# guanjq/targetdiff

Hardware: AMD Instinct MI355X
Metric: ligands/sec (1000-step sampling, 100 samples/pocket) at 1/2/4/8 MI355X (higher is better)
Workload: dtype f32

## Files before the change

targetdiff_amd/capi.py:

```python
from __future__ import annotations

import ctypes
import os
from ctypes import POINTER, c_char_p, c_float, c_int32, c_int64, c_size_t, c_void_p

import numpy as np
import torch

_HERE = os.path.dirname(os.path.abspath(__file__))
LIB_PATH = os.path.join(_HERE, 'lib', 'libtargetdiff_hip.so')

TD_OK = 0
HIDDEN = 128
KNN = 32


class TdConfig(ctypes.Structure):
    _fields_ = [('hidden_dim', c_int32), ('n_heads', c_int32), ('knn', c_int32), ('num_layers', c_int32),
                ('num_r_gaussian', c_int32), ('edge_feat_dim', c_int32), ('protein_feat_dim', c_int32),
                ('ligand_num_classes', c_int32), ('num_timesteps', c_int32), ('cutoff_mode', c_int32), ('radius', c_float),
                ('max_num_neighbors', c_int32), ('model_mean_type', c_int32), ('num_blocks', c_int32), ('ew_net_type', c_int32),
                ('x2h_out_fc', c_int32), ('sync_twoup', c_int32), ('num_x2h', c_int32), ('num_h2x', c_int32), ('reserved', c_int32 * 1)]


# ... 554 lines not shown
        io.d_step = _ptr(step_index, torch.int32, 'step_index').value
        io.d_t_all = _ptr(t_all, torch.int32, 't_all').value
        io.num_steps, io.pos_only = S, int(bool(pos_only))
        io.d_ligand_pos = _ptr(ligand_pos, torch.float32, 'ligand_pos').value
        io.d_ligand_v = _ptr(ligand_v, torch.int64, 'ligand_v').value
        io.d_noise = _ptr(noise, torch.float32, 'noise').value
        io.d_uniform = _ptr(uniform, torch.float32, 'uniform').value
        io.d_pos_traj = _ptr(pos_traj, torch.float32, 'pos_traj').value
        io.d_v_traj = _ptr(v_traj, torch.int64, 'v_traj').value
        io.d_v0_traj = _ptr(v0_traj, torch.float32, 'v0_traj').value if v0_traj is not None and v0_traj.numel() else None
        io.d_vt_traj = _ptr(vt_traj, torch.float32, 'vt_traj').value if vt_traj is not None and vt_traj.numel() else None
        gb = _graph_bias_ptr(ligand_graph_bias, int(t_all.shape[1]))
        io.d_ligand_graph_bias = gb.value if gb is not None else None
        fm, fp, fv = _fixed_ptrs(fixed_mask, fixed_pos, fixed_v, self.Nl)
        if fm is not None:
            io.d_fixed_mask, io.d_fixed_pos, io.d_fixed_v = fm.value, fp.value, fv.value
        return io

    def set_program(self, table, kinds):
        if table is None:
            self._prog_table = None
            with _on(self.device):
                _check(self.lib.td_session_set_program(self.handle, None, None, 0), 'td_session_set_program')
            return
        kinds = [int(k) for k in kinds]
        if table.dtype != torch.float32 or tuple(table.shape) != (len(kinds), PROG_ROW) or not table.is_contiguous():
            raise ValueError(f'the program table must be contiguous fp32 [{len(kinds)}, {PROG_ROW}]')
        arr = (c_int32 * len(kinds))(*kinds)
        self._prog_table = table
        with _on(self.device):
            _check(self.lib.td_session_set_program(self.handle, _ptr(table, torch.float32, 'table'), arr, len(kinds)),
                   'td_session_set_program')

    def step(self, io: StepIO, use_graph=True):
        with _on(self.device):
            _check(self.lib.td_session_step(self.handle, ctypes.byref(io), int(bool(use_graph)), _stream(self.device)),
                   'td_session_step')

    def last_step_was_graph(self) -> bool:
        return bool(self.lib.td_session_step_graph(self.handle))

    def row_counts(self):
        n = self._counts()
        return int(n[0]), int(n[1]), [int(v) for v in n[2:6] if v >= 0]

    def forward_reach_rows(self):
        v = int(self._counts()[6])
        return v if v >= 0 else None

    def shared_static_tables(self):
        n = self._counts()
        return (int(n[7]), int(n[8])) if n[7] >= 0 else None

    @_device_bound
    def _counts(self):
        n = (c_int32 * 10)()
        _check(self.lib.td_session_row_counts(self.handle, n, 10, _stream(self.device)), 'td_session_row_counts')
        return n

    def dirty_rows(self) -> int:
        return self.row_counts()[1]


EGNN_LAYER_KEYS = ('edge_mlp.net.0.weight', 'edge_mlp.net.0.bias', 'edge_mlp.net.2.weight', 'edge_mlp.net.2.bias',
                   'edge_inf.0.weight', 'edge_inf.0.bias', 'x_mlp.0.weight', 'x_mlp.0.bias', 'x_mlp.2.weight',
                   'node_mlp.net.0.weight', 'node_mlp.net.0.bias', 'node_mlp.net.2.weight', 'node_mlp.net.2.bias')


def egnn_flat_key_order(num_layers: int):
    return [f'net.{l}.{k}' for l in range(num_layers) for k in EGNN_LAYER_KEYS]


def graph_ptr(batch: torch.Tensor, B: int) -> torch.Tensor:
    lib = load_library()
    ptr = torch.empty(B + 1, dtype=torch.int32, device=batch.device)
    with _on(batch.device):
        _check(lib.td_graph_ptr(_ptr(batch, torch.int64, 'batch'), batch.numel(), B, _ptr(ptr), _stream(batch.device)),
               'td_graph_ptr')
    return ptr


def protein_centroids(protein_pos: torch.Tensor, protein_ptr: torch.Tensor) -> torch.Tensor:
    lib = load_library()
    B = protein_ptr.numel() - 1
    scratch = protein_pos.detach().clone().contiguous().float()
    offset = torch.empty(B, 3, dtype=torch.float32, device=protein_pos.device)
    with _on(protein_pos.device):
        _check(lib.td_center_pos(_ptr(scratch), _ptr(protein_ptr, torch.int32, 'protein_ptr'), None,
                                 _ptr(protein_ptr, torch.int32, 'protein_ptr'), B, _ptr(offset), 1, -1,
                                 _stream(protein_pos.device)), 'td_center_pos')
    return offset


class NativeEgnn:

    def __init__(self, num_layers: int, state_dict, hidden_dim=HIDDEN, edge_feat_dim=4, k=KNN, device=None, prefix=''):
        self.lib = load_library()
        self.device = _canonical_device(device)
        self.num_layers = int(num_layers)
        blob = np.ascontiguousarray(np.concatenate(
            [state_dict[prefix + key].detach().cpu().numpy().astype(np.float32).reshape(-1)
             for key in egnn_flat_key_order(self.num_layers)]))
        handle = c_void_p()
        with torch.cuda.device(self.device):
            _check(self.lib.td_egnn_create(self.num_layers, hidden_dim, edge_feat_dim, k, blob.ctypes.data_as(POINTER(c_float)),
                                           blob.size, ctypes.byref(handle)), 'td_egnn_create')
# ... 147 lines not shown
```

targetdiff_amd/csrc/edge16.hip:

```cpp
#include <type_traits>

#include "td_device.h"
#include "td_internal.h"

typedef float floatx4_t __attribute__((ext_vector_type(4)));

__device__ __forceinline__ floatx4_t td_mfma16(float a, float b, floatx4_t c) {
    return __builtin_amdgcn_mfma_f32_16x16x4f32(a, b, c, 0, 0, 0);
}

#ifndef TD_ZPLAIN_OFF
#define TD_ZPLAIN_OFF 0
#endif
#ifndef TD_ABL
#define TD_ABL 0
#endif
typedef _Float16 half8_16 __attribute__((ext_vector_type(8)));
__device__ __forceinline__ floatx4_t td_mfma16h(uint4 a, uint4 b, floatx4_t c) {
    return __builtin_amdgcn_mfma_f32_16x16x32_f16(__builtin_bit_cast(half8_16, a), __builtin_bit_cast(half8_16, b), c, 0, 0, 0);
}
__device__ __forceinline__ void td_split_h2(float x, float y, unsigned &h1, unsigned &h2) {
    h1 = __builtin_bit_cast(unsigned, __builtin_amdgcn_cvt_pkrtz(x, y));
    asm("v_fma_mixlo_f16 %0, %1, -1.0, %2 op_sel_hi:[1,0,0]\n\t"
        "v_fma_mixhi_f16 %0, %1, -1.0, %3 op_sel:[1,0,0] op_sel_hi:[1,0,0]"
// ... 41 lines not shown
#if TD_SPLIT_X4
#pragma unroll
    for (int m = 0; m < 4; ++m) h1[m] = __builtin_bit_cast(unsigned, __builtin_amdgcn_cvt_pkrtz(x[m], y[m]));
    asm("v_fma_mixlo_f16 %0, %4, -1.0, %8 op_sel_hi:[1,0,0]\n\t"
        "v_fma_mixlo_f16 %1, %5, -1.0, %9 op_sel_hi:[1,0,0]\n\t"
        "v_fma_mixlo_f16 %2, %6, -1.0, %10 op_sel_hi:[1,0,0]\n\t"
        "v_fma_mixlo_f16 %3, %7, -1.0, %11 op_sel_hi:[1,0,0]\n\t"
        "v_fma_mixhi_f16 %0, %4, -1.0, %12 op_sel:[1,0,0] op_sel_hi:[1,0,0]\n\t"
        "v_fma_mixhi_f16 %1, %5, -1.0, %13 op_sel:[1,0,0] op_sel_hi:[1,0,0]\n\t"
        "v_fma_mixhi_f16 %2, %6, -1.0, %14 op_sel:[1,0,0] op_sel_hi:[1,0,0]\n\t"
        "v_fma_mixhi_f16 %3, %7, -1.0, %15 op_sel:[1,0,0] op_sel_hi:[1,0,0]"
        : "=&v"(h2[0]), "=&v"(h2[1]), "=&v"(h2[2]), "=&v"(h2[3])
        : "v"(h1[0]), "v"(h1[1]), "v"(h1[2]), "v"(h1[3]), "v"(x[0]), "v"(x[1]), "v"(x[2]), "v"(x[3]), "v"(y[0]), "v"(y[1]), "v"(y[2]), "v"(y[3]));
#else
#pragma unroll
    for (int m = 0; m < 4; ++m) td_split_h2(x[m], y[m], h1[m], h2[m]);
#endif
}

constexpr float TD_ATT_SCALE_16 = 0.35355339059327373f;
constexpr float TD_LOG2E = 1.4426950408889634f;
constexpr float TD_FAR_CENTRE = 1.0e4f;
constexpr int E16_STEPS = TD_SLOTK / 4;
constexpr int E16_R_FLOATS = 2 * 2 * E16_STEPS * 64 * 8;
constexpr int E16_WQ_FLOATS = 8 * 4 * 2 * 64 * 4;

struct Args16 {
    const float4 *x4;
    const int32_t *nbr;
    const float *ew;
    const float *P;
    const float *q;
    const int32_t *rows;
    const int32_t *count_ptr;
    float *h;
    const float *gate_m;
    float *out;
    float *alpha;
    float4 *x4_out;
    int64_t count;
    TdEdgeMlp mlp;
    const float *offsets;
    float coeff;
    int p_off;
    const int32_t *chunk_node;
    const int32_t *cptr;
    const int32_t *lig_rows;
    int64_t lig_count;
    int cpn_p;
    int64_t lig_chunks;
    const int32_t *mixed_count;
    int deal;
    unsigned long long *trace;
};

__device__ __forceinline__ void td_trace_wave_end(unsigned long long *trace, int lane) {
    if (lane == 0) {
        const unsigned long long t = __builtin_amdgcn_s_memrealtime();
        atomicMin(trace + 8 * blockIdx.x + 2, t);
        atomicAdd(trace + 8 * blockIdx.x + 3, t);
    }
}

__device__ __forceinline__ void td_node_range16(int64_t count, const int32_t *count_ptr, int64_t &begin, int64_t &end, int G = gridDim.x,
                                                int b = blockIdx.x) {
    if (count_ptr) count = *count_ptr;
    const int x = b & 7, r = G & 7;
    const int chunk = x * (G >> 3) + (x < r ? x : r) + (b >> 3);
    const int64_t per = (count + G - 1) / G;
    begin = (int64_t)chunk * per;
    end = begin + per < count ? begin + per : count;
}

__device__ __forceinline__ void td_deal16(int64_t count, int U, int64_t &first, int64_t &end, int64_t &stride, int G = gridDim.x,
                                          int b = blockIdx.x) {
    const int x = b & 7, r = G & 7, w = b >> 3;
    const int c0 = x * (G >> 3) + (x < r ? x : r), nx = (G >> 3) + (x < r ? 1 : 0);
    const int64_t xb = count * c0 / G;
    end = count * (c0 + nx) / G;
    first = xb + (int64_t)w * U;
    stride = (int64_t)nx * U;
}

__device__ __forceinline__ float td_sum_groups(float v) { return td_sum_halves(td_sum_rows16(v)); }

__device__ __forceinline__ float td_sum16(float v) {
    v += td_dpp<DPP_QUAD_XOR1>(v);
    v += td_dpp<DPP_QUAD_XOR2>(v);
    v += td_dpp<DPP_ROW_HALF_MIRROR>(v);
    v += td_dpp<DPP_ROW_MIRROR>(v);
    return v;
}
__device__ __forceinline__ float td_max16(float v) {
    v = fmaxf(v, td_dpp<DPP_QUAD_XOR1>(v));
    v = fmaxf(v, td_dpp<DPP_QUAD_XOR2>(v));
    v = fmaxf(v, td_dpp<DPP_ROW_HALF_MIRROR>(v));
    v = fmaxf(v, td_dpp<DPP_ROW_MIRROR>(v));
    return v;
}

#define TD_DPP4(op, ctrl)                                            \
    op " %0, %0, %0 " ctrl " row_mask:0xf bank_mask:0xf\n\t"         \
    op " %1, %1, %1 " ctrl " row_mask:0xf bank_mask:0xf\n\t"         \
    op " %2, %2, %2 " ctrl " row_mask:0xf bank_mask:0xf\n\t"         \
    op " %3, %3, %3 " ctrl " row_mask:0xf bank_mask:0xf\n\t"
__device__ __forceinline__ void td_max16x4(float (&v)[4]) {
// ... 370 lines not shown
                for (int h2 = 0; h2 < 2; ++h2)
#pragma unroll
                    for (int eb = 0; eb < NEB; ++eb)
                        acc[eb][2 * hp + h2] = td_mfma16b(aq[h2], bq[eb][tb], acc[eb][2 * hp + h2]);
            }
        }
    }
}

template <int NEB>
__device__ __forceinline__ void td_h2_bquads(const float (&m)[NEB][5], const unsigned (&ct)[NEB], uint4 (&bq)[NEB][2]) {
    if constexpr (NEB == 2) {
        const float x[4] = {m[0][0], m[0][2], m[1][0], m[1][2]}, y[4] = {m[0][1], m[0][3], m[1][1], m[1][3]};
        unsigned a1[4], a2[4], u1, u2;
        td_split_h2_x4(x, y, a1, a2);
        td_split_h2(m[0][4], m[1][4], u1, u2);
        bq[0][0] = make_uint4(a1[0], a1[1], a1[0], a1[1]);
        bq[1][0] = make_uint4(a1[2], a1[3], a1[2], a1[3]);
        bq[0][1] = make_uint4(a2[0], a2[1], __builtin_amdgcn_perm(u2, u1, 0x05040100u), __builtin_amdgcn_perm(ct[0], u1, 0x07060100u));
        bq[1][1] = make_uint4(a2[2], a2[3], __builtin_amdgcn_perm(u2, u1, 0x07060302u), __builtin_amdgcn_perm(ct[1], u1, 0x07060302u));
    } else {
        unsigned a1[2], a2[2], u1, u2;
        td_split_h2(m[0][0], m[0][1], a1[0], a2[0]);
        td_split_h2(m[0][2], m[0][3], a1[1], a2[1]);
        td_split_h2(m[0][4], 0.f, u1, u2);
        bq[0][0] = make_uint4(a1[0], a1[1], a1[0], a1[1]);
        bq[0][1] = make_uint4(a2[0], a2[1], __builtin_amdgcn_perm(u2, u1, 0x05040100u), __builtin_amdgcn_perm(ct[0], u1, 0x07060100u));
    }
}
template <bool AHEAD, int NEB>
__device__ __forceinline__ void td_h2_tiles(const uint4 *__restrict__ Rs, const uint4 (&bq)[NEB][2], floatx4_t (&acc)[2][8]) {
    auto quad = [&](int st) -> uint4 { return Rs[((st & 1) ? 0 : 512) + (st >> 1) * 64]; };
    if constexpr (AHEAD) {
        uint4 cur = quad(0);
#pragma unroll
        for (int st = 0; st < 16; ++st) {
            uint4 nxt = cur;
            if (st + 1 < 16) nxt = quad(st + 1);
            __builtin_amdgcn_sched_barrier(0);
#pragma unroll
            for (int eb = 0; eb < NEB; ++eb) acc[eb][st >> 1] = td_mfma16h(cur, bq[eb][(st & 1) ? 0 : 1], acc[eb][st >> 1]);
            cur = nxt;
        }
    } else {
#pragma unroll
        for (int st = 0; st < 16; ++st) {
            const uint4 q = quad(st);
#pragma unroll
            for (int eb = 0; eb < NEB; ++eb) acc[eb][st >> 1] = td_mfma16h(q, bq[eb][(st & 1) ? 0 : 1], acc[eb][st >> 1]);
        }
    }
}

struct TdNoHook { __device__ __forceinline__ void operator()() const {} };
template <bool LOAD_EW, bool ONE_CLASS, bool PI_LATE, int NEB, bool LN_SKIP, int PK, int AH = 0, class Hook = TdNoHook, bool NO_LN = false>
__device__ __forceinline__ void td_first_layer_split16(const Args16 &a, const uint4 *__restrict__ Rp,
                                                       const float *__restrict__ KB,
                                                       const float (&offj)[8], const RowIn16 &r, int64_t i, int lane,
                                                       floatx4_t (&acc)[2][8], Edge2 &ed, Hook before_products = Hook()) {
    const int g = lane >> 4;
    const float4 xi = r.xi;
    ed.xi = xi;
    const int cls = xi.w > 0.5f ? 0 : 1;
    float4 pi[8];
    {
        const float *pp = a.P + (size_t)i * (4 * TD_H) + a.p_off + 4 * g;
#pragma unroll
        for (int hb = 0; hb < 8; ++hb) pi[hb] = *reinterpret_cast<const float4 *>(pp + 16 * hb);
    }
    auto add_pi = [&]() {
#pragma unroll
        for (int hb = 0; hb < 8; ++hb)
#pragma unroll
            for (int eb = 0; eb < NEB; ++eb) {
                acc[eb][hb][0] += pi[hb].x; acc[eb][hb][1] += pi[hb].y; acc[eb][hb][2] += pi[hb].z; acc[eb][hb][3] += pi[hb].w;
            }
    };
    if (!PI_LATE) add_pi();
    int slot[NEB];
    bool has[2][NEB];
    float gv[NEB][5];
    if (NEB == 1) {
        ed.valid[1] = false; ed.any[1] = false;
        ed.rel[1][0] = ed.rel[1][1] = ed.rel[1][2] = 0.f;
        if (LOAD_EW) ed.ew[1] = 0.f;
#pragma unroll
        for (int hb = 0; hb < 8; ++hb) acc[1][hb] = floatx4_t{0.f, 0.f, 0.f, 0.f};
    }
    const float c2 = a.coeff * TD_LOG2E;
#pragma unroll
    for (int eb = 0; eb < NEB; ++eb) {
        ed.valid[eb] = r.j[eb] >= 0;
        const float4 xj = r.xj[eb];
        if (LOAD_EW) ed.ew[eb] = r.ew[eb];
        const float rx = xi.x - xj.x, ry = xi.y - xj.y, rz = xi.z - xj.z;
        const float dist = td_sqrt_d2(rx * rx + ry * ry + rz * rz);
        ed.rel[eb][0] = rx; ed.rel[eb][1] = ry; ed.rel[eb][2] = rz;
        slot[eb] = xj.w > 0.5f ? 0 : 1;
        has[0][eb] = __ballot(ed.valid[eb] && slot[eb] == 0) != 0ull;
        has[1][eb] = __ballot(ed.valid[eb] && slot[eb] == 1) != 0ull;
        ed.any[eb] = has[0][eb] || has[1][eb];
#pragma unroll
        for (int j = 0; j < 5; ++j) {
            const float u = dist - offj[j];
            gv[eb][j] = __builtin_amdgcn_exp2f(c2 * (u * u));
        }
    }
    before_products();
    auto products4 = [&](int sl) {
        if constexpr (PK == 5) {
            float mm[NEB][5];
            unsigned ct[NEB];
            uint4 bh[NEB][2];
#pragma unroll
            for (int eb = 0; eb < NEB; ++eb) {
                const bool keep = !has[1 - sl][eb] || slot[eb] == sl;
#pragma unroll
                for (int j = 0; j < 5; ++j) mm[eb][j] = keep ? gv[eb][j] : 0.f;
                ct[eb] = keep ? 0x3c000000u : 0u;
            }
            td_h2_bquads<NEB>(mm, ct, bh);
            td_h2_tiles<AH != 0, NEB>(Rp + (size_t)((ONE_CLASS ? 0 : cls * 2) + sl) * e16q_cs_u4<5>() + lane, bh, acc);
            return;
        } else {
        uint4 bq[NEB][4];
        const unsigned ctype = td_pk4_ctype(g);
#pragma unroll
        for (int eb = 0; eb < NEB; ++eb) {
            const bool keep = !has[1 - sl][eb] || slot[eb] == sl;
            float m[5];
#pragma unroll
            for (int j = 0; j < 5; ++j) m[j] = keep ? gv[eb][j] : 0.f;
            td_pk4_bquads(m, keep ? ctype : 0u, bq[eb]);
        }
        if constexpr (PK == 3) {
            static_assert(PK != 3 || !ONE_CLASS, "PK = 3 holds both destination classes");
            if (cls) td_pk4_tiles<1, AH, NEB>(Rp + 2 * e16q_cs_u4<2>() + (size_t)sl * e16q_cs_u4<1>() + lane, lane, bq, acc);
            else td_pk4_tiles<2, AH, NEB>(Rp + (size_t)sl * e16q_cs_u4<2>() + lane, lane, bq, acc);
        } else if constexpr (PK == 4) {
            static_assert(PK != 4 || ONE_CLASS, "PK = 4 holds one destination class");
            if (sl) td_pk4_tiles<1, AH, NEB>(Rp + e16q_cs_u4<2>() + lane, lane, bq, acc);
            else td_pk4_tiles<2, AH, NEB>(Rp + lane, lane, bq, acc);
        } else
            td_pk4_tiles<PK, AH, NEB>(Rp + (size_t)((ONE_CLASS ? 0 : cls * 2) + sl) * e16q_cs_u4<PK>() + lane, lane, bq, acc);
        }
    };
#pragma unroll
    for (int sl = 0; sl < 2; ++sl) {
        bool any_sl = has[sl][0];
        if (NEB == 2) any_sl = any_sl || has[sl][NEB - 1];
        if (any_sl) products4(sl);
    }
    if (PI_LATE) add_pi();
    if constexpr (NO_LN) return;
    const TdLn ln{a.mlp.ln_c1, a.mlp.ln_c2};
    if (NEB == 2 && LN_SKIP) td_ln_relu16_skip(KB, g, acc, ln, ed.any);
    else td_ln_relu16<NEB>(KB, g, acc, ln);
}

template <bool LOAD_EW, bool SKIP_EMPTY = false>
__device__ __forceinline__ void td_first_layer16(const Args16 &a, const float4 *__restrict__ Rt,
                                                 const float *__restrict__ KB,
                                                 const float (&offk)[E16_STEPS], int64_t i, int lane,
                                                 floatx4_t (&acc)[2][8], Edge2 &ed, int64_t c = -1) {
    RowIn16 r;
    if (c < 0) c = i;
    td_row_index16(a, i, c, lane, r);
    td_row_gather16<LOAD_EW>(a, i, c, lane, r, acc);
    td_first_layer_compute16<LOAD_EW, SKIP_EMPTY>(a, Rt, KB, offk, r, lane, acc, ed);
}

constexpr int K16_WAVES = 16;
constexpr int XV16_WAVES = 8;
constexpr size_t K16_LDS_BYTES = (size_t)(E16_R_FLOATS + E16_WQ_FLOATS + TD_H + 4) * sizeof(float);
#ifndef TD_KEY_WAVES
#define TD_KEY_WAVES 12
#endif
#ifndef TD_KEY_WALK_F16
#define TD_KEY_WALK_F16 1
#endif
constexpr int K16S_WAVES = TD_KEY_WAVES;
#ifndef TD_KEY_PK
#define TD_KEY_PK 3
#endif
#ifndef TD_KEY_AH
#define TD_KEY_AH -1
#endif
constexpr size_t K16S_LDS_BYTES = (size_t)(e16q_u4<TD_KEY_PK>() * 4 + E16_WQ_FLOATS + TD_H + 4 + 32) * sizeof(float);
static_assert(K16S_LDS_BYTES <= 160 * 1024, "key pass: LDS");

template <bool XV, int WAVES, int STAGE, int GRAPH = 0, bool SPLIT = false, int L2 = 0, int FL = 0>
__global__ __launch_bounds__(WAVES * 64) void edge_key16_kernel(Args16 a) {
    constexpr bool ZPLAIN = L2 == 2;
    constexpr bool CHUNKED = GRAPH == 1;
    constexpr bool VIA = GRAPH == 2;
    constexpr bool L2H = L2 != 0;
    static_assert(L2 == 0 || (SPLIT && !XV && STAGE == 0), "f16 logits: x2h key pass, bf16 first layer");
    static_assert(FL == 0 || SPLIT, "f16 first layer: the 16-bit instantiations");
    constexpr int KPK = FL ? 5 : TD_KEY_PK;
    constexpr int RF = SPLIT ? e16q_u4<KPK>() * 4 : E16_R_FLOATS;
    constexpr int NOFF = SPLIT ? 8 : E16_STEPS;
    extern __shared__ __attribute__((aligned(16))) float lds[];
    const float4 *Rt = reinterpret_cast<const float4 *>(lds);
    const float4 *Wq = reinterpret_cast<const float4 *>(lds + RF);
    const float *KB = lds + RF + E16_WQ_FLOATS;
    const int tid = threadIdx.x, lane = tid & 63, wid = tid >> 6;
    const int lo = lane & 15, g = lane >> 4;
    if (a.trace && threadIdx.x == 0) a.trace[8 * blockIdx.x + 4] = __builtin_amdgcn_s_memrealtime();
    {
        if (SPLIT) {
            if constexpr (KPK == 5)
                td_stage_lds16(reinterpret_cast<const float4 *>(a.mlp.R16h), reinterpret_cast<float4 *>(lds), e16q_u4<5>(), tid, WAVES * 64);
            else if constexpr (TD_KEY_PK == 3) {
                td_stage_pk4<2>(a.mlp.R16q, lds, 2, tid, WAVES * 64);
                td_stage_pk4<1>(a.mlp.R16q + (size_t)2 * E16Q_GLOBAL_CS_U4 * 4, lds + 2 * e16q_cs_u4<2>() * 4, 2, tid, WAVES * 64);
            } else
                td_stage_pk4<TD_KEY_PK>(a.mlp.R16q, lds, 4, tid, WAVES * 64);
        }
        else td_stage_lds16(reinterpret_cast<const float4 *>(a.mlp.R16), reinterpret_cast<float4 *>(lds), RF / 4, tid, WAVES * 64);
        const int nw4 = XV ? 8 * 4 * 64 / 4 : E16_WQ_FLOATS / 4;
        td_stage_lds16(reinterpret_cast<const float4 *>(a.mlp.Walt16), reinterpret_cast<float4 *>(lds + RF), nw4, tid,
                       WAVES * 64);
        if (tid < TD_H) lds[RF + E16_WQ_FLOATS + tid] = a.mlp.beta[tid];
        else if (tid == TD_H) *reinterpret_cast<int *>(lds + RF + E16_WQ_FLOATS + TD_H) = 0;
        else if (SPLIT && tid >= TD_H + 32 && tid < TD_H + 64) {
            const int s8 = tid - (TD_H + 32);
            lds[RF + E16_WQ_FLOATS + TD_H + 4 + s8] = (s8 & 7) < 5 ? a.offsets[5 * (s8 >> 3) + (s8 & 7)] : TD_FAR_CENTRE;
        }
    }
    float offk[NOFF];
#pragma unroll
    for (int s = 0; s < NOFF; ++s) {
        const int k = SPLIT ? 5 * g + s : 4 * s + g;
        offk[s] = SPLIT ? (s < 5 ? a.offsets[k] : TD_FAR_CENTRE) : (k < TD_NG ? a.offsets[k] : 0.f);
    }
    __syncthreads();
    if (a.trace && tid == 0) a.trace[8 * blockIdx.x] = __builtin_amdgcn_s_memrealtime();
    int64_t begin, end, stride = WAVES;
    if (a.deal) td_deal16(a.count_ptr ? (int64_t)*a.count_ptr : a.count, a.deal == 2 ? 1 : WAVES, begin, end, stride);
    else td_node_range16(a.count, a.count_ptr, begin, end);
    int *row_ctr = reinterpret_cast<int *>(lds + RF + E16_WQ_FLOATS + TD_H);
    const bool dyn = a.deal == 2;
    auto grab = [&]() -> int {
        int n = 0;
        if (lane == 0) n = __hip_atomic_fetch_add(row_ctr, 1, __ATOMIC_RELAXED, __HIP_MEMORY_SCOPE_WORKGROUP);
        return n;
    };
    auto row_of = [&](int n) -> int64_t {
        return begin + (int64_t)__builtin_amdgcn_readfirstlane(n) * stride;
    };

    float4 qpre0, qpre1;
    auto first_layer = [&](int64_t i, int64_t c, floatx4_t (&acc)[2][8], Edge2 &ed) {
        constexpr bool EW = !XV && !CHUNKED;
        if constexpr (SPLIT) {
            RowIn16 rin;
            td_row_index16(a, i, c, lane, rin);
            td_row_gather16<EW>(a, i, c, lane, rin, acc);
            float offr[8];
            {
                int dep = 0;
                asm volatile("" : "+v"(dep));
                const float4 *op = reinterpret_cast<const float4 *>(lds + RF + E16_WQ_FLOATS + TD_H + 4 + 8 * g + dep);
                const float4 o0 = op[0], o1 = op[1];
                offr[0] = o0.x; offr[1] = o0.y; offr[2] = o0.z; offr[3] = o0.w; offr[4] = o1.x; offr[5] = o1.y; offr[6] = o1.z; offr[7] = o1.w;
            }
            auto fetch_q = [&]() {
                if constexpr (!XV && !CHUNKED) {
                    qpre0 = *reinterpret_cast<const float4 *>(a.q + (size_t)i * TD_H + 8 * lo);
                    qpre1 = *reinterpret_cast<const float4 *>(a.q + (size_t)i * TD_H + 8 * lo + 4);
                }
            };
            if (XV && CHUNKED && __ballot(rin.j[1] >= 0) == 0ull)
                td_first_layer_split16<EW, false, false, 1, false, KPK>(a, reinterpret_cast<const uint4 *>(lds), KB, offr, rin, i, lane, acc, ed, fetch_q);
            else
                td_first_layer_split16<EW, false, false, 2, CHUNKED, KPK, (CHUNKED || XV) ? 0 : TD_KEY_AH, decltype(fetch_q), L2H>(a, reinterpret_cast<const uint4 *>(lds), KB, offr, rin, i, lane, acc, ed, fetch_q);
        } else
            td_first_layer16<EW, CHUNKED>(a, Rt, KB, offk, i, lane, acc, ed, c);
    };

    for (int64_t it = dyn ? row_of(grab()) : begin + wid; it < end; it = dyn ? row_of(grab()) : it + stride) {
        const int64_t i = a.rows ? (int64_t)a.rows[it] : it;
        int64_t c0 = i;
        int nch = 1;
        if (CHUNKED) {
            c0 = __builtin_amdgcn_readfirstlane(a.cptr[i]);
            nch = __builtin_amdgcn_readfirstlane(a.cptr[i + 1]) - (int)c0;
        }
        if (VIA) {
            if (__builtin_amdgcn_readfirstlane(__float_as_int(a.x4[i].w)) > __float_as_int(0.5f)) continue;
            c0 = __builtin_amdgcn_readfirstlane(a.cptr[i]);
        }

        if (XV) {
            const float *Wx = lds + RF;
            const float b2 = a.mlp.b2[lo];
            float sx = 0.f, sy = 0.f, sz = 0.f;
            float4 xi_keep = a.x4[i];
            for (int64_t c = c0; c < c0 + nch; ++c) {
                floatx4_t acc[2][8];
                Edge2 ed;
                first_layer(i, c, acc, ed);
                floatx4_t xv[2];
#pragma unroll
                for (int eb = 0; eb < 2; ++eb) xv[eb] = floatx4_t{0.f, 0.f, 0.f, 0.f};
#pragma unroll
                for (int hb = 0; hb < 8; ++hb)
#pragma unroll
                    for (int r = 0; r < 4; ++r) {
                        const float u = Wx[(hb * 4 + r) * 64 + lane];
                        xv[0] = td_mfma16(u, acc[0][hb][r], xv[0]);
                        if (!CHUNKED || ed.any[1]) xv[1] = td_mfma16(u, acc[1][hb][r], xv[1]);
                    }
#pragma unroll
                for (int r = 0; r < 4; ++r) {
                    const float bias = __shfl(b2, 4 * g + r);
                    const float *ap = a.alpha + ((size_t)c * TD_HEADS + 4 * g + r) * TD_K + lo;
#pragma unroll
                    for (int eb = 0; eb < 2; ++eb) {
                        const float wgt = ed.valid[eb] ? ap[16 * eb] * (xv[eb][r] + bias) : 0.f;
                        sx = fmaf(wgt, ed.rel[eb][0], sx);
                        sy = fmaf(wgt, ed.rel[eb][1], sy);
                        sz = fmaf(wgt, ed.rel[eb][2], sz);
                    }
                }
// ... 920 lines not shown
#pragma unroll
            for (int s = 0; s < 8; ++s) zb[hb] = td_mfma16(bvb[hb & 1][s], al[s], zb[hb]);
        }

        }
        const int64_t icur = i;
        const float hcur0 = hres0, hcur1 = hres1;
        if (SPLIT && dyn && more) {
            inext = settle(inext, rnext, cnext);
            more = inext >= 0;
        }
        {
            const int64_t gsafe = more ? inext : 0;
            td_row_gather16<false>(a, gsafe, more ? cnext : chunk_of(0), lane, rnext, acc);
            load_side(gsafe, more ? cnext : chunk_of(0), al, hres0, hres1);
            rin = rnext;
        }
        i = inext;

        float o0, o1;
        td_value_out16(zb, Wt_lane, o0, o1);
        o0 = fmaf(B2[nout], ssum, o0 * out_scale);
        o1 = fmaf(B2[nout + 4], ssum, o1 * out_scale);
        if (a.out) {
            a.out[(size_t)icur * TD_H + nout] = o0;
            a.out[(size_t)icur * TD_H + nout + 4] = o1;
        } else {
            a.h[(size_t)icur * TD_H + nout] = hcur0 + o0;
            a.h[(size_t)icur * TD_H + nout + 4] = hcur1 + o1;
        }
    }
    trace_end();
}

constexpr int V16T_WAVES = 12;
#ifndef TD_VALUET_PK
#define TD_VALUET_PK 1
#endif
constexpr int V16T_PK = TD_VALUET_PK;
#ifndef TD_VALUET_AH
#define TD_VALUET_AH -1
#endif
constexpr int V16T_AH = TD_VALUET_AH;
constexpr int V16T_WAVE_FLOATS = V16_TILE_FLOATS;
constexpr size_t V16T_LDS_BYTES =
    (size_t)(e16q_half_u4<V16T_PK>() * 4 + V16_W_FLOATS + V16T_WAVES * V16T_WAVE_FLOATS + 2 * TD_H + 4 + 32) * sizeof(float);
static_assert(V16T_LDS_BYTES <= 160 * 1024, "value pass (12 waves): LDS");

template <int L2, bool VIA = false, int FL = 0>
__global__ __launch_bounds__(V16T_WAVES * 64) void edge_value16t_kernel(Args16 a) {
    constexpr bool ZPLAIN = L2 == 2;
    constexpr int WAVES = V16T_WAVES;
    constexpr int VPK = FL ? 5 : V16T_PK;
    constexpr int RF = e16q_half_u4<VPK>() * 4;
    extern __shared__ __attribute__((aligned(16))) float lds[];
    const int tid = threadIdx.x, lane = tid & 63, wid = tid >> 6;
    const int lo = lane & 15, g = lane >> 4;
    float *TB = lds + RF + V16_W_FLOATS + wid * V16T_WAVE_FLOATS;
    float *B2 = lds + RF + V16_W_FLOATS + WAVES * V16T_WAVE_FLOATS;
    const float *KB = B2 + TD_H;
    int my_cls = 1, GL = 0;
    const int64_t n_rows = a.count_ptr ? (int64_t)*a.count_ptr : a.count;
    {
        const int64_t G = gridDim.x, nl = a.lig_count, np = n_rows > nl ? n_rows - nl : 0;
        if (nl > 0) {
            int64_t nm = a.mixed_count ? (int64_t)*a.mixed_count - nl : (np * 3) / 10;
            nm = nm < 0 ? 0 : (nm > np ? np : nm);
            const int64_t wl = TD_ROW_COST_MIXED * nl, wp = TD_ROW_COST_PURE * (np - nm) + TD_ROW_COST_MIXED * nm;
            GL = (int)((wl * G + (wl + wp) / 2) / (wl + wp));
            const int cap = (int)G - (np > 0 ? 1 : 0);
            GL = GL < 1 ? 1 : (GL > cap ? cap : GL);
        }
        my_cls = (int)blockIdx.x >= (int)G - GL ? 0 : 1;
    }
    const int GP = gridDim.x - GL;
    if (a.trace && threadIdx.x == 0) a.trace[8 * blockIdx.x + 4] = __builtin_amdgcn_s_memrealtime();
    {
        if constexpr (VPK == 5)
            td_stage_lds16(reinterpret_cast<const float4 *>(a.mlp.R16h) + (size_t)my_cls * 2 * e16q_cs_u4<5>(), reinterpret_cast<float4 *>(lds), 2 * e16q_cs_u4<5>(), tid, WAVES * 64);
        else if constexpr (V16T_PK == 4) {
            td_stage_pk4<2>(a.mlp.R16q + (size_t)my_cls * 2 * E16Q_GLOBAL_CS_U4 * 4, lds, 1, tid, WAVES * 64);
            td_stage_pk4<1>(a.mlp.R16q + (size_t)(my_cls * 2 + 1) * E16Q_GLOBAL_CS_U4 * 4, lds + e16q_cs_u4<2>() * 4, 1, tid, WAVES * 64);
        } else
            td_stage_pk4<V16T_PK>(a.mlp.R16q + (size_t)my_cls * 2 * E16Q_GLOBAL_CS_U4 * 4, lds, 2, tid, WAVES * 64);
        td_stage_lds16(reinterpret_cast<const float4 *>(a.mlp.Walt), reinterpret_cast<float4 *>(lds + RF), V16_W_FLOATS / 4, tid, WAVES * 64);
        if (tid < TD_H) B2[tid] = a.mlp.b2[tid];
        else if (tid < 2 * TD_H) B2[tid] = a.mlp.beta[tid - TD_H];
        else if (tid == 2 * TD_H) *reinterpret_cast<int *>(B2 + 2 * TD_H) = 0;
        else if (tid >= 2 * TD_H + 32 && tid < 2 * TD_H + 64) {
            const int s8 = tid - (2 * TD_H + 32);
            B2[2 * TD_H + 4 + s8] = (s8 & 7) < 5 ? a.offsets[5 * (s8 >> 3) + (s8 & 7)] : TD_FAR_CENTRE;
        }
    }
    __syncthreads();
    if (a.trace && tid == 0) a.trace[8 * blockIdx.x] = __builtin_amdgcn_s_memrealtime();
    const int32_t *list = a.rows;
    int64_t first, end, stride = 1;
    if (my_cls) td_deal16(n_rows, 1, first, end, stride, GP, (int)blockIdx.x);
    else {
        list = a.lig_rows;
        const int64_t per = (a.lig_count + GL - 1) / GL;
        first = ((int)blockIdx.x - GP) * per;
        end = first + per < a.lig_count ? first + per : a.lig_count;
    }
    int *row_ctr = reinterpret_cast<int *>(B2 + 2 * TD_H);
    auto next_row = [&]() -> int64_t {
        int n = 0;
        if (lane == 0) n = __hip_atomic_fetch_add(row_ctr, 1, __ATOMIC_RELAXED, __HIP_MEMORY_SCOPE_WORKGROUP);
        n = __builtin_amdgcn_readfirstlane(n);
        const int64_t itx = first + (int64_t)n * stride;
        return itx < end ? (int64_t)__builtin_amdgcn_readfirstlane((int)(list ? (int64_t)list[itx] : itx)) : -1;
    };
    const int nout = td_value_out_index16(lo, g);
    int woff = RF + 4 * lane;
    asm volatile("" : "+v"(woff));
    const float *Wt_lane = lds + woff;
    for (int64_t i = next_row(); i >= 0; i = next_row()) {
        RowIn16 rin;
        const int64_t c = VIA ? (int64_t)__builtin_amdgcn_readfirstlane(a.cptr[i]) : i;
        td_row_index16(a, i, c, lane, rin);
        if (((__builtin_amdgcn_readfirstlane(__float_as_int(rin.xi.w)) > __float_as_int(0.5f)) ? 0 : 1) != my_cls) continue;
        floatx4_t acc[2][8];
        td_row_gather16<false>(a, i, c, lane, rin, acc);
        float al[8];
        if constexpr (L2 != 0) {
            const float *ap = a.alpha + ((size_t)c * TD_HEADS + lo) * TD_K + 4 * g;
            const float4 v0 = *reinterpret_cast<const float4 *>(ap), v1 = *reinterpret_cast<const float4 *>(ap + 16);
            al[0] = v0.x; al[1] = v1.x; al[2] = v0.y; al[3] = v1.y; al[4] = v0.z; al[5] = v1.z; al[6] = v0.w; al[7] = v1.w;
        } else {
            const float *ap = a.alpha + ((size_t)c * TD_HEADS + lo) * TD_K + 8 * g;
            const float4 v0 = *reinterpret_cast<const float4 *>(ap), v1 = *reinterpret_cast<const float4 *>(ap + 4);
            al[0] = v0.x; al[1] = v0.y; al[2] = v0.z; al[3] = v0.w; al[4] = v1.x; al[5] = v1.y; al[6] = v1.z; al[7] = v1.w;
        }
        const float hres0 = a.h[(size_t)i * TD_H + nout], hres1 = a.h[(size_t)i * TD_H + nout + 4];
        Edge2 ed;
        float offr[8];
        {
            int dep = 0;
            asm volatile("" : "+v"(dep));
            const float4 *op = reinterpret_cast<const float4 *>(B2 + 2 * TD_H + 4 + 8 * g + dep);
            const float4 o0 = op[0], o1 = op[1];
            offr[0] = o0.x; offr[1] = o0.y; offr[2] = o0.z; offr[3] = o0.w; offr[4] = o1.x; offr[5] = o1.y; offr[6] = o1.z; offr[7] = o1.w;
        }
        float ssum = ((al[0] + al[1]) + (al[2] + al[3])) + ((al[4] + al[5]) + (al[6] + al[7]));
        ssum = td_sum_groups(ssum);
        floatx4_t zb[8];
        constexpr float OUT_SCALE = L2 == 0 ? 1.0f : (ZPLAIN ? 1.0f / 1024.0f : 1.0f / (1024.0f * TD_Z_SCALE));
        if constexpr (L2 != 0) {
        td_first_layer_split16<false, true, false, 2, false, VPK, V16T_AH, TdNoHook, true>(a, reinterpret_cast<const uint4 *>(lds), KB, offr, rin, i, lane, acc, ed);
        uint4 z1[8], z2[8];
        td_ln_relu16_pairs_eb<!ZPLAIN>(KB, g, acc, TdLn{a.mlp.ln_c1, a.mlp.ln_c2}, z1, z2);
        uint4 aq1, aq2;
        {
            unsigned p1[4], p2[4];
            const float ax[4] = {al[0] * 1024.0f, al[2] * 1024.0f, al[4] * 1024.0f, al[6] * 1024.0f};
            const float ay[4] = {al[1] * 1024.0f, al[3] * 1024.0f, al[5] * 1024.0f, al[7] * 1024.0f};
            td_split_h2_x4(ax, ay, p1, p2);
            aq1 = make_uint4(p1[0], p1[1], p1[2], p1[3]);
            aq2 = make_uint4(p2[0], p2[1], p2[2], p2[3]);
        }
        unsigned *TW = reinterpret_cast<unsigned *>(TB);
        constexpr int TWS = 20, TWP = 16 * TWS;
        auto flip_store = [&](int hb) {
            *reinterpret_cast<uint4 *>(TW + lo * TWS + 4 * g) = z1[hb];
            *reinterpret_cast<uint4 *>(TW + TWP + lo * TWS + 4 * g) = z2[hb];
        };
        auto flip_load = [&](uint4 (&zq)[2]) {
            const unsigned *t = TW + 4 * g * TWS + lo;
            zq[0] = make_uint4(t[0], t[TWS], t[2 * TWS], t[3 * TWS]);
            zq[1] = make_uint4(t[TWP], t[TWP + TWS], t[TWP + 2 * TWS], t[TWP + 3 * TWS]);
        };
        uint4 zqb[2][2];
        flip_store(0);
        flip_load(zqb[0]);
#pragma unroll
        for (int hb = 0; hb < 8; ++hb) {
            if (hb + 1 < 8) {
                flip_store(hb + 1);
                flip_load(zqb[(hb + 1) & 1]);
            }
            __builtin_amdgcn_sched_barrier(0);
            zb[hb] = floatx4_t{0.f, 0.f, 0.f, 0.f};
            zb[hb] = td_mfma16h(zqb[hb & 1][1], aq1, zb[hb]);
            zb[hb] = td_mfma16h(zqb[hb & 1][0], aq2, zb[hb]);
            zb[hb] = td_mfma16h(zqb[hb & 1][0], aq1, zb[hb]);
        }
        } else {
        td_first_layer_split16<false, true, false, 2, false, VPK, V16T_AH>(a, reinterpret_cast<const uint4 *>(lds), KB, offr, rin, i, lane, acc, ed);
        auto flip_store = [&](int hb) {
#pragma unroll
            for (int eb = 0; eb < 2; ++eb)
                *reinterpret_cast<float4 *>(TB + td_tile_row16(16 * eb + lo) + 4 * g) =
                    make_float4(acc[eb][hb][0], acc[eb][hb][1], acc[eb][hb][2], acc[eb][hb][3]);
        };
        auto flip_load = [&](float (&bv)[8]) {
#pragma unroll
            for (int sx = 0; sx < 8; ++sx) bv[sx] = TB[td_tile_row16(8 * g + sx) + lo];
        };
        float bvb[2][8];
        flip_store(0);
        flip_load(bvb[0]);
#pragma unroll
        for (int hb = 0; hb < 8; ++hb) {
            if (hb + 1 < 8) {
                flip_store(hb + 1);
                flip_load(bvb[(hb + 1) & 1]);
            }
            __builtin_amdgcn_sched_barrier(0);
            zb[hb] = floatx4_t{0.f, 0.f, 0.f, 0.f};
#pragma unroll
            for (int sx = 0; sx < 8; ++sx) zb[hb] = td_mfma16(bvb[hb & 1][sx], al[sx], zb[hb]);
        }
        }
        float o0, o1;
        td_value_out16(zb, Wt_lane, o0, o1);
        o0 = fmaf(B2[nout], ssum, o0 * OUT_SCALE);
        o1 = fmaf(B2[nout + 4], ssum, o1 * OUT_SCALE);
        if (a.out) {
            a.out[(size_t)i * TD_H + nout] = o0;
            a.out[(size_t)i * TD_H + nout + 4] = o1;
        } else {
            a.h[(size_t)i * TD_H + nout] = hres0 + o0;
            a.h[(size_t)i * TD_H + nout + 4] = hres1 + o1;
        }
    }
    if (a.trace) {
        td_trace_wave_end(a.trace, lane);
        __syncthreads();
        if (tid == 0) a.trace[8 * blockIdx.x + 1] = __builtin_amdgcn_s_memrealtime();
    }
}

constexpr int TD_GATE_WGS = 1024;
constexpr int G16_WAVES = 4;
constexpr int G16Q_U4 = e16q_cs_u4<1>();
constexpr size_t G16_LDS_BYTES = (size_t)G16Q_U4 * 16 + (size_t)3 * TD_H * sizeof(float);

__global__ __launch_bounds__(G16_WAVES * 64) void edge_gate16_kernel(TdGate gt, const float4 *__restrict__ x4,
                                                                     const int32_t *__restrict__ nbr, int64_t N,
                                                                     const int32_t *__restrict__ rows,
                                                                     const int32_t *__restrict__ count_ptr,
// ... 41 lines not shown
                gv[j] = __builtin_amdgcn_exp2f(c2 * (u * u));
            }
            td_pk4_bquads(gv, 0u, bq[eb]);
#pragma unroll
            for (int hb = 0; hb < 8; ++hb) {
                const float4 b = *reinterpret_cast<const float4 *>(B0 + 16 * hb + 4 * g);
                acc[eb][hb][0] = b.x; acc[eb][hb][1] = b.y; acc[eb][hb][2] = b.z; acc[eb][hb][3] = b.w;
            }
        }
        td_pk4_tiles<1, 1, 2>(Rp + lane, lane, bq, acc);
        td_ln_relu16<2>(BET, g, acc, TdLn{gt.ln_c1, gt.ln_c2});
#pragma unroll
        for (int eb = 0; eb < 2; ++eb) {
            float part = 0.f;
#pragma unroll
            for (int hb = 0; hb < 8; ++hb) {
                const float4 w = *reinterpret_cast<const float4 *>(W3 + 16 * hb + 4 * g);
                part = fmaf(acc[eb][hb][0], w.x, part); part = fmaf(acc[eb][hb][1], w.y, part);
                part = fmaf(acc[eb][hb][2], w.z, part); part = fmaf(acc[eb][hb][3], w.w, part);
            }
            const float logit = td_sum_groups(part) + gt.b3;
            if (g == 0) ew[row * TD_K + 16 * eb + lo] = valid[eb] ? 1.0f / (1.0f + expf(-logit)) : 0.f;
        }
    }
}

#define TD_LDS_ONCE(fn, bytes) do { static TdLdsOnce once; int _rc = td_set_lds(once, reinterpret_cast<const void *>(fn), bytes); if (_rc != TD_OK) return _rc; } while (0)

static int grid16(int64_t count, int waves) {
    int64_t g = (count + waves - 1) / waves;
    if (g < 256) g = count < 256 ? count : 256;
    if (g > 256) g = 256;
    if (g >= 8) g = (g / 8) * 8;
    return (int)(g < 1 ? 1 : g);
}

static unsigned long long *g_wg_trace = nullptr;
static int g_wg_trace_slots = 0, g_wg_trace_launch[3] = {0, 0, 0};
int td_set_wg_trace(unsigned long long *buf, int slots) {
    g_wg_trace = slots > 0 ? buf : nullptr;
    g_wg_trace_slots = slots;
    g_wg_trace_launch[0] = g_wg_trace_launch[1] = g_wg_trace_launch[2] = 0;
    return TD_OK;
}
bool td_wg_trace_armed() { return g_wg_trace != nullptr; }
static unsigned long long *wg_trace_slot(int pass) {
    if (!g_wg_trace) return nullptr;
    const int n = g_wg_trace_launch[pass]++ % g_wg_trace_slots;
    return g_wg_trace + ((size_t)n * 3 + pass) * 256 * 8;
}

int td_launch_edge_key16(const TdEdgeMlp &mlp, const TdLayer &L, const float4 *x4, const int32_t *nbr, const float *ew,
                         const float *P, const float *q, const int32_t *rows, const int32_t *count_ptr, int64_t count,
                         float *alpha, hipStream_t s, bool h2x_stage, const int32_t *cptr, const int32_t *lig_rows, int64_t lig_count, int cpn_p) {
    if (count == 0) return TD_OK;
    Args16 a = {};
    a.x4 = x4; a.nbr = nbr; a.ew = ew; a.P = P; a.q = q; a.rows = rows; a.count_ptr = count_ptr; a.h = nullptr;
    a.alpha = alpha; a.x4_out = nullptr; a.count = count; a.mlp = mlp; a.offsets = L.offsets; a.coeff = L.coeff; a.p_off = 0;
    a.cptr = cptr;
    const bool h2x = h2x_stage;
    if (!h2x) a.trace = wg_trace_slot(0);
    a.deal = h2x ? 0 : mlp.deal_rows;
#define TD_KEY_LAUNCH(WAVES, STAGE, CH, SP, BYTES)                                                            \
    do {                                                                                                      \
        TD_LDS_ONCE((edge_key16_kernel<false, WAVES, STAGE, CH, SP>), BYTES);                                 \
        edge_key16_kernel<false, WAVES, STAGE, CH, SP><<<dim3(grid16(a.count, WAVES)), dim3(WAVES * 64), BYTES, s>>>(a); \
    } while (0)
#define TD_KEY_LAUNCH_X2H(GR, L2V)                                                                                            \
    do {                                                                                                                  \
        if (mlp.l1_f16) {                                                                                                 \
            TD_LDS_ONCE((edge_key16_kernel<false, K16S_WAVES, 0, GR, true, L2V, 1>), K16S_LDS_BYTES);                      \
            edge_key16_kernel<false, K16S_WAVES, 0, GR, true, L2V, 1><<<dim3(grid16(a.count, K16S_WAVES)), dim3(K16S_WAVES * 64), K16S_LDS_BYTES, s>>>(a); \
        } else {                                                                                                          \
            TD_LDS_ONCE((edge_key16_kernel<false, K16S_WAVES, 0, GR, true, L2V, 0>), K16S_LDS_BYTES);                      \
            edge_key16_kernel<false, K16S_WAVES, 0, GR, true, L2V, 0><<<dim3(grid16(a.count, K16S_WAVES)), dim3(K16S_WAVES * 64), K16S_LDS_BYTES, s>>>(a); \
        }                                                                                                                 \
    } while (0)
#define TD_KEY_LAUNCH_WALK_L2(L2V) TD_KEY_LAUNCH_X2H(1, L2V)
#if TD_KEY_WALK_F16
#define TD_KEY_LAUNCH_WALK_F16(L2V)                                                                                           \
    do {                                                                                                                  \
        TD_LDS_ONCE((edge_key16_kernel<false, K16S_WAVES, 0, 1, true, L2V, 1>), K16S_LDS_BYTES);                          \
        edge_key16_kernel<false, K16S_WAVES, 0, 1, true, L2V, 1><<<dim3(grid16(a.count, K16S_WAVES)), dim3(K16S_WAVES * 64), K16S_LDS_BYTES, s>>>(a); \
    } while (0)
#define TD_KEY_LAUNCH_WALK()                                                        \
    do {                                                                            \
        if (!mlp.l2_f16 || !mlp.l1_f16) TD_KEY_LAUNCH_WALK_L2(0);                   \
        else if (mlp.z_plain && !TD_ZPLAIN_OFF) TD_KEY_LAUNCH_WALK_F16(2);          \
        else TD_KEY_LAUNCH_WALK_F16(1);                                             \
    } while (0)
#else
#define TD_KEY_LAUNCH_WALK() TD_KEY_LAUNCH_WALK_L2(0)
#endif
#define TD_KEY_LAUNCH_H2X(GR)                                                                                                 \
    do {                                                                                                                  \
        if (mlp.l1_f16) {                                                                                                 \
            TD_LDS_ONCE((edge_key16_kernel<false, K16S_WAVES, 1, GR, true, 0, 1>), K16S_LDS_BYTES);                        \
            edge_key16_kernel<false, K16S_WAVES, 1, GR, true, 0, 1><<<dim3(grid16(a.count, K16S_WAVES)), dim3(K16S_WAVES * 64), K16S_LDS_BYTES, s>>>(a); \
        } else TD_KEY_LAUNCH(K16S_WAVES, 1, GR, true, K16S_LDS_BYTES);                                                     \
    } while (0)
    if (mlp.use_split) {
        if (cptr && !h2x && cpn_p == 1) {
#define TD_KEY_LAUNCH_VIA(L2V) TD_KEY_LAUNCH_X2H(2, L2V)
            if (!mlp.l2_f16) TD_KEY_LAUNCH_VIA(0);
            else if (mlp.z_plain && !TD_ZPLAIN_OFF) TD_KEY_LAUNCH_VIA(2);
            else TD_KEY_LAUNCH_VIA(1);
#undef TD_KEY_LAUNCH_VIA
            if (lig_rows && lig_count > 0) {
                a.rows = lig_rows; a.count_ptr = nullptr; a.count = lig_count; a.trace = nullptr;
// ... 2 lines not shown
        } else if (cptr) { if (h2x) TD_KEY_LAUNCH_H2X(1); else TD_KEY_LAUNCH_WALK(); }
        else if (h2x) TD_KEY_LAUNCH_H2X(0);
        else {
#define TD_KEY_LAUNCH_L2(L2V) TD_KEY_LAUNCH_X2H(0, L2V)
            if (!mlp.l2_f16) TD_KEY_LAUNCH_L2(0);
            else if (mlp.z_plain && !TD_ZPLAIN_OFF) TD_KEY_LAUNCH_L2(2);
            else TD_KEY_LAUNCH_L2(1);
#undef TD_KEY_LAUNCH_L2
        }
    } else {
        if (cptr) { if (h2x) TD_KEY_LAUNCH(K16_WAVES, 1, 1, false, K16_LDS_BYTES); else TD_KEY_LAUNCH(K16_WAVES, 0, 1, false, K16_LDS_BYTES); }
        else { if (h2x) TD_KEY_LAUNCH(K16_WAVES, 1, 0, false, K16_LDS_BYTES); else TD_KEY_LAUNCH(K16_WAVES, 0, 0, false, K16_LDS_BYTES); }
    }
#undef TD_KEY_LAUNCH
#undef TD_KEY_LAUNCH_WALK
#undef TD_KEY_LAUNCH_WALK_L2
#undef TD_KEY_LAUNCH_X2H
#undef TD_KEY_LAUNCH_H2X
    TD_CHECK_HIP(hipGetLastError());
    return TD_OK;
}

int td_launch_edge_xv16(const TdEdgeMlp &mlp, const TdLayer &L, const float4 *x4_in, float4 *x4_out, const int32_t *nbr,
                        const float *P, const int32_t *rows, int64_t count, const float *alpha, hipStream_t s,
                        const int32_t *cptr) {
    if (count == 0) return TD_OK;
    Args16 a = {};
    a.x4 = x4_in; a.nbr = nbr; a.ew = nullptr; a.P = P; a.q = nullptr; a.rows = rows; a.count_ptr = nullptr; a.h = nullptr;
    a.alpha = const_cast<float *>(alpha); a.x4_out = x4_out; a.count = count; a.mlp = mlp; a.offsets = L.offsets;
    a.coeff = L.coeff; a.p_off = 2 * TD_H; a.cptr = cptr;
    const dim3 grid(grid16(count, XV16_WAVES)), block(XV16_WAVES * 64);
#define TD_XV_LAUNCH(CH, SP, BYTES)                                                            \
    do {                                                                                       \
        TD_LDS_ONCE((edge_key16_kernel<true, XV16_WAVES, 1, CH, SP>), BYTES);                  \
        edge_key16_kernel<true, XV16_WAVES, 1, CH, SP><<<grid, block, BYTES, s>>>(a);          \
    } while (0)
#define TD_XV_LAUNCH_F16(CH)                                                                   \
    do {                                                                                       \
        TD_LDS_ONCE((edge_key16_kernel<true, XV16_WAVES, 1, CH, true, 0, 1>), K16S_LDS_BYTES); \
        edge_key16_kernel<true, XV16_WAVES, 1, CH, true, 0, 1><<<grid, block, K16S_LDS_BYTES, s>>>(a); \
    } while (0)
    if (mlp.use_split && mlp.l1_f16) { if (cptr) TD_XV_LAUNCH_F16(1); else TD_XV_LAUNCH_F16(0); }
    else if (mlp.use_split) { if (cptr) TD_XV_LAUNCH(1, true, K16S_LDS_BYTES); else TD_XV_LAUNCH(0, true, K16S_LDS_BYTES); }
    else { if (cptr) TD_XV_LAUNCH(1, false, K16_LDS_BYTES); else TD_XV_LAUNCH(0, false, K16_LDS_BYTES); }
#undef TD_XV_LAUNCH
#undef TD_XV_LAUNCH_F16
    TD_CHECK_HIP(hipGetLastError());
    return TD_OK;
}

int td_launch_edge_value16(const TdEdgeMlp &mlp, const TdLayer &L, const float4 *x4, const int32_t *nbr, const float *P,
                           const int32_t *rows, const int32_t *count_ptr, int64_t count, float *h, const float *alpha,
                           const int32_t *lig_rows, int64_t lig_count, hipStream_t s, const int32_t *cptr, int cpn_p,
                           int64_t lig_chunks, const int32_t *mixed_count, float *out, const float *gate_m) {
    if (count == 0) return TD_OK;
    Args16 a = {};
    a.x4 = x4; a.nbr = nbr; a.ew = nullptr; a.P = P; a.q = nullptr; a.rows = rows; a.count_ptr = count_ptr; a.h = h;
    a.alpha = const_cast<float *>(alpha); a.x4_out = nullptr; a.count = count; a.mlp = mlp; a.offsets = L.offsets;
    a.coeff = L.coeff; a.p_off = 2 * TD_H; a.cptr = cptr; a.cpn_p = cpn_p > 0 ? cpn_p : 1; a.lig_chunks = lig_chunks;
    a.mixed_count = mixed_count;
    a.out = out;
    a.gate_m = cptr ? nullptr : gate_m;
    int G = grid16(count, V16_WAVES);
    const dim3 block(V16_WAVES * 64);
    a.trace = wg_trace_slot(1);
    a.deal = mlp.deal_rows;
#define TD_V16_LAUNCH(CH, GM, L2V)                                                                            \
    do {                                                                                                     \
        if (mlp.l1_f16) {                                                                                    \
            TD_LDS_ONCE((edge_value16_kernel<true, CH, GM, L2V, 1>), V16S_LDS_BYTES);                        \
            edge_value16_kernel<true, CH, GM, L2V, 1><<<dim3(G), block, V16S_LDS_BYTES, s>>>(a);             \
        } else {                                                                                             \
            TD_LDS_ONCE((edge_value16_kernel<true, CH, GM, L2V, 0>), V16S_LDS_BYTES);                        \
            edge_value16_kernel<true, CH, GM, L2V, 0><<<dim3(G), block, V16S_LDS_BYTES, s>>>(a);             \
        }                                                                                                    \
    } while (0)
#define TD_V16T_LAUNCH_ANY(L2V, VIAV)                                                                         \
    do {                                                                                                     \
        if (mlp.l1_f16) {                                                                                    \
            TD_LDS_ONCE((edge_value16t_kernel<L2V, VIAV, 1>), V16T_LDS_BYTES);                               \
            edge_value16t_kernel<L2V, VIAV, 1><<<dim3(Gt), dim3(V16T_WAVES * 64), V16T_LDS_BYTES, s>>>(a);   \
        } else {                                                                                             \
            TD_LDS_ONCE((edge_value16t_kernel<L2V, VIAV, 0>), V16T_LDS_BYTES);                               \
            edge_value16t_kernel<L2V, VIAV, 0><<<dim3(Gt), dim3(V16T_WAVES * 64), V16T_LDS_BYTES, s>>>(a);   \
        }                                                                                                    \
    } while (0)
#define TD_V16_LAUNCH_WALK_L2(L2V) TD_V16_LAUNCH(true, false, L2V)
#define TD_V16_LAUNCH_WALK()                                                        \
    do {                                                                            \
        if (!mlp.l2_f16) TD_V16_LAUNCH_WALK_L2(0);                                  \
        else if (mlp.z_plain && !TD_ZPLAIN_OFF) TD_V16_LAUNCH_WALK_L2(2);           \
        else TD_V16_LAUNCH_WALK_L2(1);                                              \
    } while (0)
    if (mlp.use_split) {
        a.lig_rows = lig_rows; a.lig_count = lig_rows ? lig_count : 0;
        if (G < 2 && a.lig_count > 0) G = 2;
        if (cptr && a.cpn_p == 1) {
            int Gt = grid16(count, V16T_WAVES);
            a.lig_rows = nullptr; a.lig_count = 0;
#define TD_V16T_LAUNCH_VIA(L2V) TD_V16T_LAUNCH_ANY(L2V, true)
            if (!mlp.l2_f16) TD_V16T_LAUNCH_VIA(0);
            else if (mlp.z_plain && !TD_ZPLAIN_OFF) TD_V16T_LAUNCH_VIA(2);
            else TD_V16T_LAUNCH_VIA(1);
#undef TD_V16T_LAUNCH_VIA
            if (lig_rows && lig_count > 0) {
                a.rows = lig_rows; a.count_ptr = nullptr; a.count = lig_count; a.lig_rows = lig_rows; a.lig_count = lig_count;
                a.mixed_count = nullptr; a.trace = nullptr;
                G = grid16(lig_count, V16_WAVES);
                TD_V16_LAUNCH_WALK();
// ... 18 lines not shown
            TD_V16_LAUNCH(false, false, 0);
        }
    } else if (cptr) {
        TD_LDS_ONCE((edge_value16_kernel<false, true>), V16_LDS_BYTES);
        edge_value16_kernel<false, true><<<dim3(G), block, V16_LDS_BYTES, s>>>(a);
    } else if (gate_m) {
        TD_LDS_ONCE((edge_value16_kernel<false, false, true>), V16_LDS_BYTES);
        edge_value16_kernel<false, false, true><<<dim3(G), block, V16_LDS_BYTES, s>>>(a);
    } else {
        TD_LDS_ONCE((edge_value16_kernel<false, false>), V16_LDS_BYTES);
        edge_value16_kernel<false, false><<<dim3(G), block, V16_LDS_BYTES, s>>>(a);
    }
#undef TD_V16_LAUNCH_WALK
#undef TD_V16_LAUNCH_WALK_L2
#undef TD_V16T_LAUNCH_ANY
#undef TD_V16_LAUNCH
    TD_CHECK_HIP(hipGetLastError());
    return TD_OK;
}

int td_launch_edge_h2x16(const TdEdgeMlp &mlp_k, const TdEdgeMlp &mlp_v, const TdLayer &L, const float4 *x4_in, float4 *x4_out,
                         const int32_t *nbr, const float *ew, const float *P, const float *q, const int32_t *rows,
                         int64_t count, hipStream_t s, const int32_t *cptr, float *alpha) {
    if (count == 0) return TD_OK;
    ArgsH2x ar = {};
    Args16 &a = ar.a;
    a.x4 = x4_in; a.nbr = nbr; a.ew = ew; a.P = P; a.q = q; a.rows = rows; a.count_ptr = nullptr; a.h = nullptr;
    a.alpha = alpha; a.x4_out = x4_out; a.count = count; a.mlp = mlp_k; a.offsets = L.offsets; a.coeff = L.coeff; a.p_off = 0;
    a.cptr = cptr;
    ar.mlp_v = mlp_v;
    a.trace = cptr ? nullptr : wg_trace_slot(2);
    const dim3 grid(grid16(count, H2X16_WAVES)), block(H2X16_WAVES * 64);
    const bool f16_first = mlp_k.l1_f16 && mlp_v.l1_f16;
    if (cptr && f16_first) {
        TD_LDS_ONCE((edge_h2x16_chunked_kernel<1>), h2x16_lds_bytes<true>());
        edge_h2x16_chunked_kernel<1><<<grid, block, h2x16_lds_bytes<true>(), s>>>(ar);
    } else if (cptr) {
        TD_LDS_ONCE((edge_h2x16_chunked_kernel<0>), h2x16_lds_bytes<true>());
        edge_h2x16_chunked_kernel<0><<<grid, block, h2x16_lds_bytes<true>(), s>>>(ar);
    } else if (mlp_k.use_split && mlp_v.use_split && f16_first) {
        TD_LDS_ONCE((edge_h2x16_kernel<true, 1>), h2x16_lds_bytes<true>());
        edge_h2x16_kernel<true, 1><<<grid, block, h2x16_lds_bytes<true>(), s>>>(ar);
    } else if (mlp_k.use_split && mlp_v.use_split) {
        TD_LDS_ONCE((edge_h2x16_kernel<true>), h2x16_lds_bytes<true>());
        edge_h2x16_kernel<true><<<grid, block, h2x16_lds_bytes<true>(), s>>>(ar);
    } else {
        TD_LDS_ONCE((edge_h2x16_kernel<false>), h2x16_lds_bytes<false>());
        edge_h2x16_kernel<false><<<grid, block, h2x16_lds_bytes<false>(), s>>>(ar);
    }
    TD_CHECK_HIP(hipGetLastError());
    return TD_OK;
}

int td_launch_gate16(const TdGate &g, const float4 *x4, const int32_t *nbr, int64_t N, const int32_t *rows,
                     const int32_t *count_ptr, float *ew, hipStream_t s, const int32_t *chunk_node) {
    if (N == 0) return TD_OK;
    TD_LDS_ONCE((edge_gate16_kernel), G16_LDS_BYTES);
    int64_t G = (N + G16_WAVES - 1) / G16_WAVES;
    if (G > TD_GATE_WGS) G = TD_GATE_WGS;
    edge_gate16_kernel<<<dim3((unsigned)G), dim3(G16_WAVES * 64), G16_LDS_BYTES, s>>>(g, x4, nbr, N, rows, count_ptr, chunk_node, ew);
    TD_CHECK_HIP(hipGetLastError());
    return TD_OK;
}
```

targetdiff_amd/csrc/graph.hip:

```cpp
#include "td_device.h"
#include "td_internal.h"

__global__ void graph_ptr_kernel(const int64_t *__restrict__ batch, int64_t N, int64_t B, int32_t *__restrict__ ptr) {
    int64_t i = (int64_t)blockIdx.x * blockDim.x + threadIdx.x;
    if (N == 0) {
        if (i <= B) ptr[i] = 0;
        return;
    }
    if (i >= N) return;
    int64_t b = batch[i];
    int64_t prev = (i == 0) ? -1 : batch[i - 1];
    for (int64_t g = prev + 1; g <= b && g <= B; ++g) ptr[g] = (int32_t)i;
    if (i == N - 1)
        for (int64_t g = b + 1; g <= B; ++g) ptr[g] = (int32_t)N;
}

int td_launch_graph_ptr(const int64_t *batch, int64_t N, int64_t B, int32_t *ptr, hipStream_t s) {
    int64_t n = N > B + 1 ? N : B + 1;
    graph_ptr_kernel<<<dim3((unsigned)((n + 255) / 256)), dim3(256), 0, s>>>(batch, N, B, ptr);
    TD_CHECK_HIP(hipGetLastError());
    return TD_OK;
}

__device__ __forceinline__ int td_find_graph(const int32_t *__restrict__ ptr, int B, int i) {
// ... 118 lines not shown
        }
        best = out;
    }
    if (lane < TD_K) {
        nbr[i * TD_K + lane] = (best == TD_KEY_MAX || lane >= k) ? -1 : (int32_t)(unsigned)(best & 0xffffffffull);
        if (STATIC) skeys[i * TD_K + lane] = best;
    }
}
template <int CH, bool STATIC>
__global__ __launch_bounds__(256) void knn_kernel(const float4 *__restrict__ x4, const int32_t *__restrict__ ptr,
                                                  const int32_t *__restrict__ gid, const int32_t *__restrict__ rows,
                                                  int64_t N, int k, int32_t *__restrict__ nbr,
                                                  unsigned long long *__restrict__ skeys) {
    knn_body<CH, STATIC>(blockIdx.x, x4, ptr, gid, rows, N, k, nbr, skeys);
}

template <bool STATIC>
static int launch_knn_t(const float4 *x4, const int32_t *node_ptr, const int32_t *gid, const int32_t *rows, int64_t N,
                        int max_graph_nodes, int k, int32_t *nbr, unsigned long long *skeys, hipStream_t s) {
    if (N == 0) return TD_OK;
    dim3 grid((unsigned)((N + 3) / 4)), block(256);
    if (max_graph_nodes > 0 && max_graph_nodes <= 256)
        knn_kernel<4, STATIC><<<grid, block, 0, s>>>(x4, node_ptr, gid, rows, N, k, nbr, skeys);
    else if (max_graph_nodes > 0 && max_graph_nodes <= 384)
        knn_kernel<6, STATIC><<<grid, block, 0, s>>>(x4, node_ptr, gid, rows, N, k, nbr, skeys);
    else if (max_graph_nodes <= 704)
        knn_kernel<11, STATIC><<<grid, block, 0, s>>>(x4, node_ptr, gid, rows, N, k, nbr, skeys);
    else
        knn_kernel<17, STATIC><<<grid, block, 0, s>>>(x4, node_ptr, gid, rows, N, k, nbr, skeys);
    TD_CHECK_HIP(hipGetLastError());
    return TD_OK;
}

int td_launch_knn(const float4 *x4, const int32_t *node_ptr, const int32_t *gid, int64_t N, int max_graph_nodes,
                  int32_t *nbr, hipStream_t s, int k) {
    return launch_knn_t<false>(x4, node_ptr, gid, nullptr, N, max_graph_nodes, k, nbr, nullptr, s);
}

int td_launch_knn_rows(const float4 *x4, const int32_t *node_ptr, const int32_t *gid, const int32_t *rows, int64_t count,
                       int max_graph_nodes, int32_t *nbr, hipStream_t s, int k) {
    return launch_knn_t<false>(x4, node_ptr, gid, rows, count, max_graph_nodes, k, nbr, nullptr, s);
}

int td_launch_knn_static(const float4 *x4, const int32_t *node_ptr, const int32_t *gid, const int32_t *rows, int64_t count,
                         int max_graph_nodes, int32_t *nbr, unsigned long long *skeys, hipStream_t s, int k) {
    return launch_knn_t<true>(x4, node_ptr, gid, rows, count, max_graph_nodes, k, nbr, skeys, s);
}

struct TdMergeArgs {
    const float4 *x4; const int32_t *ptr, *pptr, *gid, *prot_rows; int64_t Np;
    const unsigned long long *skeys; const int32_t *snbr; const float *h0, *h1s, *ews; int32_t *nbr; float *h, *ew;
    uint8_t *clean, *flags2; int k;
    const int32_t *cgraph, *cbase;
};
__device__ __forceinline__ void knn_merge_body(unsigned bid, const TdMergeArgs &ma) {
    const float4 *__restrict__ x4 = ma.x4;
    const int32_t *__restrict__ ptr = ma.ptr, *__restrict__ pptr = ma.pptr, *__restrict__ gid = ma.gid, *__restrict__ prot_rows = ma.prot_rows;
    const int64_t Np = ma.Np;
    const unsigned long long *__restrict__ skeys = ma.skeys;
    const int32_t *__restrict__ snbr = ma.snbr;
    const float *__restrict__ h0 = ma.h0, *__restrict__ h1s = ma.h1s, *__restrict__ ews = ma.ews;
    int32_t *__restrict__ nbr = ma.nbr;
    float *__restrict__ h = ma.h, *__restrict__ ew = ma.ew;
    uint8_t *__restrict__ clean = ma.clean, *__restrict__ flags2 = ma.flags2;
    const int k = ma.k;
    const int lane = threadIdx.x & 63;
    const int64_t qi = (int64_t)bid * 4 + (threadIdx.x >> 6);
    if (qi >= Np) return;
    const int64_t i = prot_rows[qi];
    const int g = gid[i];
    const int lbeg = ptr[g] + (pptr[g + 1] - pptr[g]), lend = ptr[g + 1];
    const float4 xi = x4[i];
    int64_t c = i;
    int rebase = 0;
    if (ma.cgraph) {
        rebase = ptr[g] - ptr[ma.cgraph[g]];
        c = (int64_t)ma.cbase[g] + (i - ptr[g]);
    }
    unsigned long long ks = lane < TD_K ? skeys[c * TD_K + lane] : TD_KEY_MAX;
    if (ks != TD_KEY_MAX) ks += (unsigned long long)(unsigned)rebase;
    const unsigned long long thr = __shfl(ks, k - 1);
    unsigned long long kl[2] = {TD_KEY_MAX, TD_KEY_MAX};
    bool closer = false;
    bool overflow = lend - lbeg > 128;
#pragma unroll
    for (int u = 0; u < 2; ++u) {
        const int j = lbeg + lane + 64 * u;
        if (j < lend) {
            const float4 xj = x4[j];
            const float d2 = td_dist2(xj.x - xi.x, xj.y - xi.y, xj.z - xi.z);
            kl[u] = ((unsigned long long)__float_as_uint(d2) << 32) | (unsigned)j;
            closer |= kl[u] < thr;
        }
    }
    bool is_clean = !overflow && __ballot(closer) == 0ull;
    if (!is_clean && !overflow) {
        const bool c0 = kl[0] < thr, c1 = kl[1] < thr;
        const unsigned long long m0 = __ballot(c0), m1 = __ballot(c1);
        const int n_static = __popcll(__ballot(lane < TD_K && ks != TD_KEY_MAX));
        int shift = 0;
        bool lig_in = false;
#pragma unroll
        for (int u = 0; u < 2; ++u) {
            unsigned long long mm = u ? m1 : m0;
            while (mm) {
                const int src = __builtin_amdgcn_readfirstlane(__ffsll((long long)mm) - 1);
                mm &= mm - 1;
                const unsigned clo = __builtin_amdgcn_readlane((int)(unsigned)kl[u], src);
                const unsigned chi = __builtin_amdgcn_readlane((int)(unsigned)(kl[u] >> 32), src);
                const unsigned long long ck = ((unsigned long long)chi << 32) | clo;
                if (lane < TD_K && ck < ks) ++shift;
                const int rank = __popcll(__ballot(lane < TD_K && ks < ck)) + __popcll(__ballot(c0 && kl[0] < ck)) +
                                 __popcll(__ballot(c1 && kl[1] < ck));
                if (rank < k) {
                    lig_in = true;
                    if (lane == 0) nbr[i * TD_K + rank] = (int32_t)clo;
                }
            }
        }
        const int total = n_static + __popcll(m0) + __popcll(m1);
        if (lane < TD_K) {
            const int pos = lane + shift;
            if (ks != TD_KEY_MAX && pos < k) nbr[i * TD_K + pos] = (int32_t)(unsigned)(ks & 0xffffffffull);
            if (lane >= (total < k ? total : k)) nbr[i * TD_K + lane] = -1;
        }
        is_clean = !lig_in;
    } else if (!is_clean) {
        unsigned long long best = ks;
        for (int base = lbeg; base < lend; base += 128) {
            if (base != lbeg) {
#pragma unroll
                for (int u = 0; u < 2; ++u) {
                    const int j = base + lane + 64 * u;
                    kl[u] = TD_KEY_MAX;
                    if (j < lend) {
                        const float4 xj = x4[j];
                        const float d2 = td_dist2(xj.x - xi.x, xj.y - xi.y, xj.z - xi.z);
                        kl[u] = ((unsigned long long)__float_as_uint(d2) << 32) | (unsigned)j;
                    }
                }
            }
            unsigned long long carry = best, out = TD_KEY_MAX;
            for (int r = 0; r < k; ++r) {
                unsigned long long lmin = carry;
                lmin = kl[0] < lmin ? kl[0] : lmin;
                lmin = kl[1] < lmin ? kl[1] : lmin;
                const unsigned long long wmin = td_wave_min_u64(lmin);
                if (wmin != TD_KEY_MAX) {
                    if (carry == wmin) carry = TD_KEY_MAX;
                    if (kl[0] == wmin) kl[0] = TD_KEY_MAX;
                    if (kl[1] == wmin) kl[1] = TD_KEY_MAX;
                }
                if (lane == r) out = wmin;
            }
            best = out;
        }
        if (lane < TD_K) nbr[i * TD_K + lane] = (best == TD_KEY_MAX || lane >= k) ? -1 : (int32_t)(unsigned)(best & 0xffffffffull);
        const bool lig_in = lane < k && best != TD_KEY_MAX && (int)(unsigned)(best & 0xffffffffull) >= lbeg;
        is_clean = __ballot(lig_in) == 0ull;
    } else if (lane < TD_K) {
        const int32_t sj = snbr[c * TD_K + lane];
        nbr[i * TD_K + lane] = sj >= 0 ? sj + rebase : -1;
    }
    const float2 hv = *reinterpret_cast<const float2 *>((is_clean ? h1s : h0) + c * TD_H + 2 * lane);
    *reinterpret_cast<float2 *>(h + i * TD_H + 2 * lane) = hv;
    if (is_clean && lane < TD_K) ew[i * TD_K + lane] = ews[c * TD_K + lane];
    if (lane == 0) {
        clean[i] = is_clean ? 1 : 0;
        if (flags2) flags2[i] = 0;
    }
}

__global__ __launch_bounds__(256) void knn_merge_kernel(TdMergeArgs ma) { knn_merge_body(blockIdx.x, ma); }

template <int CH>
__global__ __launch_bounds__(256) void knn_step_kernel(TdMergeArgs ma, unsigned GB, const int32_t *__restrict__ lig_rows, int64_t Nl,
                                                       int32_t *__restrict__ nbr) {
    if (blockIdx.x < GB) knn_body<CH, false>(blockIdx.x, ma.x4, ma.ptr, ma.gid, lig_rows, Nl, ma.k, nbr, nullptr);
    else knn_merge_body(blockIdx.x - GB, ma);
}

int td_launch_knn_merge(const float4 *x4, const int32_t *node_ptr, const int32_t *pptr, const int32_t *gid,
                        const int32_t *prot_rows, int64_t Np, const unsigned long long *skeys, const int32_t *snbr,
                        const float *h0, const float *h1s, const float *ews, int32_t *nbr, float *h, float *ew,
                        uint8_t *clean, uint8_t *flags2, hipStream_t s, int k, const int32_t *lig_rows, int64_t Nl,
                        int max_graph_nodes, const int32_t *cgraph, const int32_t *cbase) {
    const TdMergeArgs ma{x4, node_ptr, pptr, gid, prot_rows, Np, skeys, snbr, h0, h1s, ews, nbr, h, ew, clean, flags2, k, cgraph, cbase};
    const unsigned GA = (unsigned)((Np + 3) / 4), GB = lig_rows ? (unsigned)((Nl + 3) / 4) : 0u;
    if (GA + GB == 0) return TD_OK;
    if (GB == 0) {
        knn_merge_kernel<<<dim3(GA), dim3(256), 0, s>>>(ma);
    } else {
        const dim3 grid(GA + GB), block(256);
        if (max_graph_nodes > 0 && max_graph_nodes <= 256) knn_step_kernel<4><<<grid, block, 0, s>>>(ma, GB, lig_rows, Nl, nbr);
        else if (max_graph_nodes > 0 && max_graph_nodes <= 384) knn_step_kernel<6><<<grid, block, 0, s>>>(ma, GB, lig_rows, Nl, nbr);
        else if (max_graph_nodes <= 704) knn_step_kernel<11><<<grid, block, 0, s>>>(ma, GB, lig_rows, Nl, nbr);
        else knn_step_kernel<17><<<grid, block, 0, s>>>(ma, GB, lig_rows, Nl, nbr);
    }
    TD_CHECK_HIP(hipGetLastError());
    return TD_OK;
}

__global__ __launch_bounds__(256) void knn_merge_general_kernel(
    const float4 *__restrict__ x4, const int32_t *__restrict__ ptr, const int32_t *__restrict__ pptr,
    const int32_t *__restrict__ gid, const int32_t *__restrict__ prot_rows, int64_t Np,
    const unsigned long long *__restrict__ skeys, const int32_t *__restrict__ snbr, const float *__restrict__ h0,
    const float *__restrict__ h1s, const float *__restrict__ ews, const int32_t *__restrict__ cptr, int cpn,
    int32_t *__restrict__ nbr, float *__restrict__ h, float *__restrict__ ew, uint8_t *__restrict__ clean,
    uint8_t *__restrict__ flags2, int k) {
    const int lane = threadIdx.x & 63;
    const int64_t qi = (int64_t)blockIdx.x * 4 + (threadIdx.x >> 6);
    if (qi >= Np) return;
    const int64_t i = prot_rows[qi];
    const int g = gid[i];
    const int lbeg = ptr[g] + (pptr[g + 1] - pptr[g]), lend = ptr[g + 1];
    const float4 xi = x4[i];
    const int64_t c0 = cptr[i];
    const unsigned long long ks = skeys[i * 64 + lane];
    const unsigned long long thr = __shfl(ks, k - 1);
    bool closer = false;
    for (int base = lbeg; base < lend; base += 64) {
        const int j = base + lane;
        if (j < lend) {
            const float4 xj = x4[j];
            const float d2 = td_dist2(xj.x - xi.x, xj.y - xi.y, xj.z - xi.z);
            closer |= (((unsigned long long)__float_as_uint(d2) << 32) | (unsigned)j) < thr;
        }
    }
    bool is_clean = __ballot(closer) == 0ull;
    if (!is_clean) {
        unsigned long long best = ks;
        for (int base = lbeg; base < lend; base += 128) {
            unsigned long long kl[2];
#pragma unroll
            for (int u = 0; u < 2; ++u) {
                const int j = base + lane + 64 * u;
                kl[u] = TD_KEY_MAX;
                if (j < lend) {
                    const float4 xj = x4[j];
                    const float d2 = td_dist2(xj.x - xi.x, xj.y - xi.y, xj.z - xi.z);
// ... 738 lines not shown
```

targetdiff_amd/csrc/pack.cpp:

```cpp
#include <algorithm>
#include <atomic>
#include <cmath>
#include <cstdarg>
#include <cstdio>
#include <cstdlib>
#include <cstring>
#include <mutex>
#include <new>
#include <vector>

#include "td_device.h"
#include "td_internal.h"
#include "td_api.h"

using namespace tdapi;

namespace tdapi {



struct FoldedMlp {
    std::vector<float> w0, b0, g, b, w3, b3v;
    const float *b3;
    float ln_c1 = 1.f / 128.f, ln_c2 = 1e-5f;
// ... 411 lines not shown
        return TD_EINVAL;
    }
    if (c.model_mean_type != 0 && c.model_mean_type != 1) {
        td_set_error("td_model_create: model_mean_type must be 0 ('C0') or 1 ('noise'), got %d", c.model_mean_type);
        return TD_EINVAL;
    }
    if (c.model_mean_type == 1 && !has_rc) {
        td_set_error("td_model_create: model_mean_type 'noise' needs the 10 schedule arrays (sqrt_recip_alphas_cumprod, sqrt_recipm1_alphas_cumprod)");
        return TD_EINVAL;
    }
    const int H = TD_H, E = H - 1, F = c.protein_feat_dim, C = c.ligand_num_classes, KV = kv_in(c), L = c.num_layers;
    Cursor cur{host_weights, num_weights};
    const float *Wp = cur.take((size_t)E * F), *bp = cur.take(E);
    const float *Wl = cur.take((size_t)E * C), *bl = cur.take(E);
    const float *goff = cur.take(TD_NG);
    static const std::vector<float> zero_mlp(mlp_floats(TD_NG, TD_H, 1), 0.f);
    Cursor zc{zero_mlp.data(), zero_mlp.size()};
    MlpSrc gate = c.ew_net_type == 0 ? cur.mlp(TD_NG, H, 1) : zc.mlp(TD_NG, H, 1);
    const FoldedMlp fgate(gate, TD_NG, H, 1);
    gate = fgate.src();
    bool fold_overflow = fgate.overflow_risk;
    int fold_dead = fgate.dead_units;

    Packer pk;
    size_t oWpT = pk.alloc((size_t)F * H), obp = pk.alloc(H), oWlT = pk.alloc((size_t)C * H), obl = pk.alloc(H);
    for (int cc = 0; cc < F; ++cc)
        for (int n = 0; n < E; ++n) pk.data[oWpT + (size_t)cc * H + n] = Wp[(size_t)n * F + cc];
    for (int cc = 0; cc < C; ++cc)
        for (int n = 0; n < E; ++n) pk.data[oWlT + (size_t)cc * H + n] = Wl[(size_t)n * C + cc];
    for (int n = 0; n < E; ++n) { pk.data[obp + n] = bp[n]; pk.data[obl + n] = bl[n]; }
    pk.data[obp + E] = 0.f;
    pk.data[obl + E] = 1.f;
    size_t oGR = pk.alloc((size_t)TD_SLOT_STEPS * 64 * 4);
    for (int s = 0; s < TD_SLOT_STEPS; ++s)
        for (int lane = 0; lane < 64; ++lane)
            for (int t = 0; t < 4; ++t) {
                const int kk = td_kmap(s, lane >> 5), n = 32 * t + (lane & 31);
                pk.data[oGR + ((size_t)s * 64 + lane) * 4 + t] = kk < TD_NG ? gate.w0[(size_t)n * TD_NG + kk] : 0.f;
            }
    size_t oGb0 = pack_vec(pk, gate.b0, H), oGg = pack_vec(pk, gate.g, H), oGb = pack_vec(pk, gate.b, H),
           oGw3 = pack_vec(pk, gate.w3, H), oGoff = pack_vec(pk, goff, TD_NG);
    const float gate_b3 = gate.b3[0], gate_coeff = gaussian_coeff(goff);
    const size_t oGRp = pk.alloc(PK4_WORDS);
    pack_pk4_table(reinterpret_cast<uint32_t *>(pk.data.data() + oGRp), [&](int n, int k) { return k < TD_NG ? gate.w0[(size_t)n * TD_NG + k] : 0.f; });
    struct LayerOff { NodeOff nx, nh; EdgeOff hk, hv, xk, xv; size_t off; float coeff; size_t ew_x2h = 0, ew_h2x = 0, gate_m = 0, noB = 0, nob1 = 0, nog = 0, nobeta = 0, nob2 = 0;
                      bool has_x = false, has_h = false; };
    const int NX = num_x2h(c), NH = num_h2x(c), M = stage_rows(c);
    std::vector<LayerOff> lo((size_t)L * M);
    auto gate_rows = [&](size_t &dst, const float *src) {
        dst = pk.alloc(4 * TD_NG + 1);
        if (src) memcpy(pk.data.data() + dst, src, (4 * TD_NG + 1) * sizeof(float));
        else pk.data[dst + 4 * TD_NG] = 40.f;
    };
    for (int l = 0; l < L && cur.ok; ++l) {
        const float *off = cur.take(TD_NG);
        if (!cur.ok) break;
        const size_t ooff = pack_vec(pk, off, TD_NG);
        for (int i = 0; i < M; ++i) { lo[(size_t)l * M + i].off = ooff; lo[(size_t)l * M + i].coeff = gaussian_coeff(off); }
        for (int i = 0; i < NX; ++i) {
            LayerOff &o = lo[(size_t)l * M + i];
            MlpSrc hk = cur.mlp(KV, H, H), hv = cur.mlp(KV, H, H), hq = cur.mlp(H, H, H);
            MlpSrc nout{};
            if (c.x2h_out_fc) nout = cur.mlp(2 * H, H, H);
            const float *ewx = c.ew_net_type == 1 ? cur.take(4 * TD_NG + 1) : nullptr;
            const float *ewm = c.ew_net_type == 3 ? cur.take(H + 1) : nullptr;
            if (!cur.ok) break;
            const FoldedMlp fhk(hk, KV, H, H, true), fhv(hv, KV, H, H, true);
            hk = fhk.src(); hv = fhv.src();
            fold_overflow = fold_overflow || fhk.overflow_risk || fhv.overflow_risk;
            fold_dead += fhk.dead_units + fhv.dead_units;
            if (c.ew_net_type != 0) gate_rows(o.ew_x2h, ewx);
            if (ewm) {
                o.gate_m = pk.alloc(TD_H + 1);
                double cc = ewm[H];
                for (int oo = 0; oo < H; ++oo) cc += (double)ewm[oo] * (double)fhv.b3[oo];
                for (int n = 0; n < H; ++n) {
                    double u = 0.0;
                    for (int oo = 0; oo < H; ++oo) u += (double)ewm[oo] * (double)fhv.w3[(size_t)oo * H + n];
                    pk.data[o.gate_m + n] = (float)u;
                }
                pk.data[o.gate_m + H] = (float)cc;
            }
            if (c.x2h_out_fc) {
                o.noB = pack_B128(pk, nout.w0, 2 * TD_H, 0);
                pack_B128(pk, nout.w0, 2 * TD_H, TD_H);
                pack_B128(pk, nout.w3, TD_H, 0);
                o.nob1 = pack_vec(pk, nout.b0, TD_H);
                o.nog = pack_vec(pk, nout.g, TD_H);
                o.nobeta = pack_vec(pk, nout.b, TD_H);
                o.nob2 = pack_vec(pk, nout.b3, TD_H);
            }
            o.nx = pack_node_stage(pk, hk, hv, hq, KV);
            o.hk = pack_edge_mlp(pk, fhk, KV, H, 1);
            o.hv = pack_edge_mlp(pk, fhv, KV, H, 2);
            o.has_x = true;
        }
        for (int j = 0; j < NH && cur.ok; ++j) {
            LayerOff &o = lo[(size_t)l * M + j];
            MlpSrc xk = cur.mlp(KV, H, H), xv = cur.mlp(KV, H, c.n_heads), xq = cur.mlp(H, H, H);
            const float *ewh = c.ew_net_type == 1 ? cur.take(4 * TD_NG + 1) : nullptr;
            if (!cur.ok) break;
            const FoldedMlp fxk(xk, KV, H, H, true), fxv(xv, KV, H, c.n_heads, true);
            xk = fxk.src(); xv = fxv.src();
            fold_overflow = fold_overflow || fxk.overflow_risk || fxv.overflow_risk;
            fold_dead += fxk.dead_units + fxv.dead_units;
            if (c.ew_net_type != 0) gate_rows(o.ew_h2x, ewh);
            o.nh = pack_node_stage(pk, xk, xv, xq, KV);
            o.xk = pack_edge_mlp(pk, fxk, KV, H, 1);
            o.xv = pack_edge_mlp(pk, fxv, KV, c.n_heads, 0);
            o.has_h = true;
        }
    }
    const float *V0 = cur.take((size_t)H * H), *vb0 = cur.take(H), *V2 = cur.take((size_t)C * H), *vb2 = cur.take(C);
    if (!cur.ok || cur.left != 0) { td_set_error("td_model_create: weight blob layout mismatch"); return TD_EINVAL; }
    if (fold_overflow) {
        td_set_error("td_model_create: an edge MLP's LayerNorm has bias / |weight| beyond 1e15 on a unit that is not negligible "
                     "(sqrt(hidden) |weight| max |second-Linear column| above 2^-30 of the MLP's largest): the folded form would overflow fp32");
        return TD_EINVAL;
    }
    size_t oW0T = pk.alloc((size_t)H * H), ohb0 = pack_vec(pk, vb0, H), oW2T = pk.alloc((size_t)H * TD_MAXC),
           ohb2 = pack_vec(pk, vb2, C, TD_MAXC);
    for (int k = 0; k < H; ++k) {
        for (int n = 0; n < H; ++n) pk.data[oW0T + (size_t)k * H + n] = V0[(size_t)n * H + k];
        for (int cc = 0; cc < C; ++cc) pk.data[oW2T + (size_t)k * TD_MAXC + cc] = V2[(size_t)cc * H + k];
    }
    const int T = c.num_timesteps;
    size_t oS = pk.alloc((size_t)10 * T);
    if (host_schedules) memcpy(pk.data.data() + oS, host_schedules, (size_t)(has_rc ? 10 : (has_abar ? 8 : 7)) * T * sizeof(float));

    td_model *m = new (std::nothrow) td_model();
    if (!m) { td_set_error("td_model_create: out of host memory"); return TD_ENOMEM; }
    m->cfg = c;
    m->blob_floats = pk.data.size();
    m->fold_dead_units = fold_dead;
    m->layers = new (std::nothrow) TdLayer[(size_t)L * stage_rows(c)]();
    hipError_t e = hipMalloc(reinterpret_cast<void **>(&m->blob), m->blob_floats * sizeof(float));
    if (e == hipSuccess) e = hipMemcpy(m->blob, pk.data.data(), m->blob_floats * sizeof(float), hipMemcpyHostToDevice);
    if (e != hipSuccess || !m->layers) {
        td_set_error("td_model_create: device upload failed: %s", hipGetErrorString(e));
        if (m->blob) (void)hipFree(m->blob);
        delete[] m->layers;
        delete m;
        return e != hipSuccess ? TD_EHIP : TD_ENOMEM;
    }
    const float *D = m->blob;
    m->emb = TdEmbed{D + oWpT, D + obp, D + oWlT, D + obl};
    m->gate = TdGate{D + oGR, D + oGb0, D + oGg, D + oGb, D + oGw3, gate_b3, D + oGoff, gate_coeff, D + oGRp, fgate.ln_c1, fgate.ln_c2, m->opt.edge_key_split != 0};
    auto edge = [&](const EdgeOff &o, bool split = false) {
        return TdEdgeMlp{D + o.R, D + o.gamma, D + o.beta, D + o.W2, D + o.b2, D + o.R16, D + o.Walt16, D + o.Walt,
                         D + o.R16q, o.R16h ? D + o.R16h : nullptr, o.ln_c1, o.ln_c2, o.w2_bound, m->opt.edge_second_layer_f16 != 0 && o.f16_safe,
                         m->opt.edge_first_layer_f16 != 0 && o.R16h != 0 && o.f16_safe, o.z_plain, split && m->opt.edge_key_split != 0,
                         m->opt.edge_row_dealing, o.f16_safe};
    };
    auto node = [&](const NodeOff &o) {
        return TdNodeStage{D + o.projB, D + o.projBias, D + o.qGamma, D + o.qBeta, D + o.q3B, D + o.q3Bias, D + o.projB3, D + o.q3B3,
                           m->opt.node_proj_split != 0, m->opt.node_proj_bpipe != 0, m->opt.node_proj_async != 0};
    };
    for (size_t l = 0; l < lo.size(); ++l) {
        TdLayer &Ly = m->layers[l];
        Ly = TdLayer{};
        Ly.offsets = D + lo[l].off; Ly.coeff = lo[l].coeff;
        if (lo[l].has_x) {
            Ly.nodeX2h = node(lo[l].nx);
            Ly.hk = edge(lo[l].hk, true); Ly.hv = edge(lo[l].hv, true);
            m->fold_fp32_mlps += !lo[l].hk.f16_safe + !lo[l].hv.f16_safe;
            Ly.ew_x2h = c.ew_net_type != 0 ? D + lo[l].ew_x2h : nullptr;
            Ly.gate_m = c.ew_net_type == 3 ? D + lo[l].gate_m : nullptr;
            if (c.x2h_out_fc) Ly.nodeOut = TdNodeOut{D + lo[l].noB, D + lo[l].nob1, D + lo[l].nog, D + lo[l].nobeta, D + lo[l].nob2};
        }
        if (lo[l].has_h) {
            Ly.nodeH2x = node(lo[l].nh);
            Ly.xk = edge(lo[l].xk, true); Ly.xv = edge(lo[l].xv, true);
            m->fold_fp32_mlps += !lo[l].xk.f16_safe + !lo[l].xv.f16_safe;
            Ly.ew_h2x = c.ew_net_type != 0 ? D + lo[l].ew_h2x : nullptr;
        }
    }
    m->head = TdHead{D + oW0T, D + ohb0, D + oW2T, D + ohb2};
    const float *S = D + oS;
    m->sched = TdSchedules{S, S + T, S + 2 * T, S + 3 * T, S + 4 * T, S + 5 * T, S + 6 * T, has_abar ? S + 7 * T : nullptr,
                           has_rc ? S + 8 * T : nullptr, has_rc ? S + 9 * T : nullptr};
    *out = m;
    return TD_OK;
}

extern "C" void td_model_destroy(td_model *m) {
    if (!m) return;
    if (m->blob) (void)hipFree(m->blob);
    delete[] m->layers;
    delete m;
}

extern "C" int td_model_set_option(td_model *m, const char *name, int32_t value) {
    if (!m || !name) { td_set_error("td_model_set_option: null argument"); return TD_EINVAL; }
    if (strcmp(name, "h2x_fused") == 0) m->opt.h2x_fused = value != 0;
    else if (strcmp(name, "node_proj_split") == 0) {
        m->opt.node_proj_split = value != 0;
        for (int l = 0; l < m->cfg.num_layers * stage_rows(m->cfg); ++l) m->layers[l].nodeX2h.use_split = m->layers[l].nodeH2x.use_split = value != 0;
    } else if (strcmp(name, "edge_row_dealing") == 0) {
        m->opt.edge_row_dealing = value < 0 ? 0 : (value > 2 ? 2 : value);
        for (int l = 0; l < m->cfg.num_layers * stage_rows(m->cfg); ++l)
            m->layers[l].hk.deal_rows = m->layers[l].hv.deal_rows = m->layers[l].xk.deal_rows = m->layers[l].xv.deal_rows = m->opt.edge_row_dealing;
    } else if (strcmp(name, "node_proj_bpipe") == 0) {
        m->opt.node_proj_bpipe = value != 0;
        for (int l = 0; l < m->cfg.num_layers * stage_rows(m->cfg); ++l) m->layers[l].nodeX2h.bpipe = m->layers[l].nodeH2x.bpipe = value != 0;
    } else if (strcmp(name, "node_proj_async") == 0) {
        m->opt.node_proj_async = value != 0;
        for (int l = 0; l < m->cfg.num_layers * stage_rows(m->cfg); ++l) m->layers[l].nodeX2h.async_copy = m->layers[l].nodeH2x.async_copy = value != 0;
    } else if (strcmp(name, "edge_key_split") == 0) {
        m->opt.edge_key_split = value != 0;
        m->gate.use_split = value != 0;
        for (int l = 0; l < m->cfg.num_layers * stage_rows(m->cfg); ++l) {
            m->layers[l].hk.use_split = m->layers[l].hk.R16q && value != 0;
            m->layers[l].hv.use_split = m->layers[l].hv.R16q && value != 0;
            m->layers[l].xk.use_split = m->layers[l].xk.R16q && value != 0;
            m->layers[l].xv.use_split = m->layers[l].xv.R16q && value != 0;
        }
    } else if (strcmp(name, "edge_first_layer_f16") == 0) {
        m->opt.edge_first_layer_f16 = value != 0;
        for (int l = 0; l < m->cfg.num_layers * stage_rows(m->cfg); ++l)
            for (TdEdgeMlp *e : {&m->layers[l].hk, &m->layers[l].hv, &m->layers[l].xk, &m->layers[l].xv}) e->l1_f16 = e->R16h && e->f16_safe && value != 0;
    } else if (strcmp(name, "edge_second_layer_f16") == 0) {
        m->opt.edge_second_layer_f16 = value != 0;
        for (int l = 0; l < m->cfg.num_layers * stage_rows(m->cfg); ++l)
            for (TdEdgeMlp *e : {&m->layers[l].hk, &m->layers[l].hv, &m->layers[l].xk, &m->layers[l].xv}) e->l2_f16 = e->f16_safe && value != 0;
    } else if (strcmp(name, "session_hop_levels") == 0) {
        if (value < 1 || value > TD_HOP_LEVELS) { td_set_error("td_model_set_option: session_hop_levels must be 1..%d", TD_HOP_LEVELS); return TD_EINVAL; }
        m->opt.session_hop_levels = value;
    } else if (strcmp(name, "session_forward_reach") == 0) m->opt.session_forward_reach = value != 0;
    else if (strcmp(name, "session_step_lists") == 0) m->opt.session_step_lists = value != 0;
    else if (strcmp(name, "session_share_pockets") == 0) m->opt.session_share_pockets = value != 0;
    else if (strcmp(name, "fold_dead_units") == 0 || strcmp(name, "fold_fp32_mlps") == 0) {
        td_set_error("td_model_set_option: '%s' is read-only (a decision of the LayerNorm fold at td_model_create)", name);
        return TD_EINVAL;
    } else { td_set_error("td_model_set_option: unknown option '%s'", name); return TD_EINVAL; }
    ++m->option_epoch;
    return TD_OK;
}

extern "C" int td_model_get_option(const td_model *m, const char *name, int32_t *value) {
    if (!m || !name || !value) { td_set_error("td_model_get_option: null argument"); return TD_EINVAL; }
    if (strcmp(name, "h2x_fused") == 0) *value = m->opt.h2x_fused;
    else if (strcmp(name, "node_proj_split") == 0) *value = m->opt.node_proj_split;
    else if (strcmp(name, "node_proj_async") == 0) *value = m->opt.node_proj_async;
    else if (strcmp(name, "node_proj_bpipe") == 0) *value = m->opt.node_proj_bpipe;
    else if (strcmp(name, "edge_row_dealing") == 0) *value = m->opt.edge_row_dealing;
    else if (strcmp(name, "edge_key_split") == 0) *value = m->opt.edge_key_split;
    else if (strcmp(name, "edge_second_layer_f16") == 0) *value = m->opt.edge_second_layer_f16;
    else if (strcmp(name, "edge_first_layer_f16") == 0) *value = m->opt.edge_first_layer_f16;
    else if (strcmp(name, "session_hop_levels") == 0) *value = m->opt.session_hop_levels;
    else if (strcmp(name, "session_forward_reach") == 0) *value = m->opt.session_forward_reach;
    else if (strcmp(name, "session_step_lists") == 0) *value = m->opt.session_step_lists;
    else if (strcmp(name, "session_share_pockets") == 0) *value = m->opt.session_share_pockets;
    else if (strcmp(name, "fold_dead_units") == 0) *value = m->fold_dead_units;
    else if (strcmp(name, "fold_fp32_mlps") == 0) *value = m->fold_fp32_mlps;
    else { td_set_error("td_model_get_option: unknown option '%s'", name); return TD_EINVAL; }
    return TD_OK;
}
```

targetdiff_amd/csrc/plan.cpp:

```cpp
#include <atomic>
#include <cmath>
#include <cstdarg>
#include <cstdio>
#include <cstdlib>
#include <cstring>
#include <mutex>
#include <new>
#include <vector>

#include "td_device.h"
#include "td_internal.h"
#include "td_api.h"

using namespace tdapi;

namespace tdapi {

Workspace carve(char *base, int64_t N, int64_t B, int64_t Nl) {
    Workspace w;
    size_t off = 0;
    auto take = [&](size_t n) { char *p = base ? base + off : nullptr; off += align_up(n); return p; };
    const size_t n = (size_t)(N > 0 ? N : 1), nl = (size_t)(Nl > 0 ? Nl : n);
    w.x4a = reinterpret_cast<float4 *>(take(n * sizeof(float4)));
    w.x4b = reinterpret_cast<float4 *>(take(n * sizeof(float4)));
    w.gid = reinterpret_cast<int32_t *>(take(n * sizeof(int32_t)));
    w.nbr = reinterpret_cast<int32_t *>(take(n * TD_K * sizeof(int32_t)));
    w.lig_node = reinterpret_cast<int32_t *>(take((nl + 1) * sizeof(int32_t)));
    w.node_ptr = reinterpret_cast<int32_t *>(take((size_t)(B + 1) * sizeof(int32_t)));
    w.ew = reinterpret_cast<float *>(take(n * TD_K * sizeof(float)));
    w.P = reinterpret_cast<float *>(take(n * 4 * TD_H * sizeof(float)));
    w.q = reinterpret_cast<float *>(take(n * TD_H * sizeof(float)));
    w.h = reinterpret_cast<float *>(take(n * TD_H * sizeof(float)));
    w.alpha = reinterpret_cast<float *>(take(n * TD_HEADS * TD_K * sizeof(float)));
    w.Px = reinterpret_cast<float *>(take(n * 4 * TD_H * sizeof(float)));
    w.qx = reinterpret_cast<float *>(take(n * TD_H * sizeof(float)));
    w.bytes = off;
    return w;
}


int key_pass(const TdEdgeMlp &mlp, const TdLayer &L, const float4 *x4, const GraphTab &gt, const float *ew, const int32_t *nbr,
             const float *P, const float *q, const int32_t *rows, const int32_t *count_ptr, int64_t count, float *alpha, hipStream_t s,
             const int32_t *lig, int64_t Nl, bool h2x_stage) {
    return td_launch_edge_key16(mlp, L, x4, nbr, ew, P, q, rows, count_ptr, count, alpha, s, h2x_stage, gt.cptr, lig, Nl, gt.cpn_p);
}
int value_pass(const TdEdgeMlp &mlp, const TdLayer &L, const float4 *x4, const GraphTab &gt, const int32_t *nbr, const float *P,
               const int32_t *rows, const int32_t *count_ptr, int64_t count, float *h, const float *alpha, const int32_t *lig,
               int64_t Nl, hipStream_t s, float *out) {
    return td_launch_edge_value16(mlp, L, x4, nbr, P, rows, count_ptr, count, h, alpha, lig, Nl, s, gt.cptr, gt.cpn_p,
                                  lig ? gt.NCl : 0, gt.mixed, out, L.gate_m);
}

int h2x_project(const TdLayer &L, Workspace &w, float *h, int64_t N, int64_t Nl, float *P, float *q,
                const int32_t *hop_rows, const int32_t *hop_count, hipStream_t s) {
    ProfScope ps(PC_NODE, s);
    if (hop_rows) return td_launch_node_proj(L.nodeH2x, h, N, hop_rows, 0x0a, P, q, s, hop_count, w.lig_node, Nl, 0x15);
    return td_launch_node_proj(L.nodeH2x, h, N, nullptr, 0x0a, P, q, s, nullptr, w.lig_node, Nl, 0x15);
}

int h2x_attend(const td_model *m, const TdLayer &L, Workspace &w, const GraphTab &gt, int64_t Nl, float4 *xc, float4 *xn, float *P,
               float *q, hipStream_t s) {
    int rc;
    if (m->opt.h2x_fused && (!gt.cptr || (L.xk.use_split && L.xv.use_split))) {
        ProfScope ps(PC_H2X_K, s);
        return td_launch_edge_h2x16(L.xk, L.xv, L, xc, xn, gt.nbr, gt.ew, P, q, w.lig_node, Nl, s, gt.cptr, gt.alpha);
    }
    {
        ProfScope ps(PC_H2X_K, s);
        if ((rc = key_pass(L.xk, L, xc, gt, gt.ew, gt.nbr, P, q, w.lig_node, nullptr, Nl, gt.alpha, s, nullptr, 0, true)) != TD_OK) return rc;
    }
    ProfScope ps(PC_H2X_V, s);
    return td_launch_edge_xv16(L.xv, L, xc, xn, gt.nbr, P, w.lig_node, Nl, gt.alpha, s, gt.cptr);
}


int run_backbone_stages(const td_model *m, Workspace &w, const GraphTab &gt, float *h, int64_t N, int64_t Nl, int fix_x,
                        float4 **x_final, hipStream_t s, bool init_xn);

int run_backbone(const td_model *m, Workspace &w, const GraphTab &gt, float *h, int64_t N, int64_t Nl, int fix_x,
                 float4 **x_final, hipStream_t s, bool init_xn, bool layer0_x2h_done,
                 const int32_t *hop_rows, const int32_t *hop_count, int hop_levels, const FwdReach *fwd) {
    int rc;
    if (stage_rows(m->cfg) > 1 || m->cfg.num_x2h > 1 || m->cfg.num_h2x > 1) return run_backbone_stages(m, w, gt, h, N, Nl, fix_x, x_final, s, init_xn);
    const int Lc = m->cfg.num_layers;
    auto level_rows = [&](int k) -> const int32_t * { return (hop_rows && k <= hop_levels) ? hop_rows + (size_t)(k - 1) * N : nullptr; };
    auto level_count = [&](int k) -> const int32_t * { return (hop_rows && k <= hop_levels) ? hop_count + (k - 1) : nullptr; };
    float4 *xc = w.x4a, *xn = w.x4b;
    const bool do_h2x = !fix_x && Nl > 0;
    if (do_h2x && init_xn) TD_CHECK_HIP(hipMemcpyAsync(xn, xc, (size_t)N * sizeof(float4), hipMemcpyDeviceToDevice, s));
    auto proj_rows = [&](int l) -> const int32_t * { return l > 0 ? level_rows(Lc - 1 - l + 2) : nullptr; };
    auto proj_count = [&](int l) -> const int32_t * { return l > 0 ? level_count(Lc - 1 - l + 2) : nullptr; };
    bool proj_done = false;
    const bool sync = m->cfg.sync_twoup != 0;
    for (int l = 0; l < Lc; ++l) {
        const TdLayer &L = m->layers[l];
        if (!(l == 0 && layer0_x2h_done)) {
            const int e = Lc - 1 - l;
            const int32_t *rws = l > 0 ? level_rows(e + 1) : nullptr, *cnt = l > 0 ? level_count(e + 1) : nullptr;
            const bool use_fwd = fwd && l == 1 && !rws;
            if (use_fwd) { rws = fwd->rows; cnt = fwd->counts; }
            if (sync && do_h2x) {
                ProfScope ps(PC_NODE, s);
                if ((rc = td_launch_node_proj_pair(L.nodeH2x, level_rows(1), level_count(1), w.lig_node, Nl, w.Px, w.qx, L.nodeX2h,
// ... 216 lines not shown
```

targetdiff_amd/csrc/session.cpp:

```cpp
#include <atomic>
#include <cmath>
#include <cstdarg>
#include <cstdio>
#include <cstdlib>
#include <cstring>
#include <map>
#include <mutex>
#include <new>
#include <vector>

#include "td_device.h"
#include "td_internal.h"
#include "td_api.h"

using namespace tdapi;

struct td_session {
    const td_model *m;
    int64_t N, Np, Nl, B;
    int max_graph_nodes;
    char *block;
    hipStream_t last_stream;
    Workspace w;
    int32_t *prot_node, *pptr, *lptr, *snbr, *dirty_rows, *dirty_count, *hop_rows, *hop_count, *dirty_chunks;
    int hop_levels;
    unsigned long long *skeys;
    float *ews, *h0, *h1s, *h2s, *P0, *q0;
    uint8_t *flags2;
    int32_t *fwd_rows, *fwd_rest, *fwd_counts;
    bool use_fwd;
    uint8_t *clean;
    int graph_nodes_max;
    int32_t *cgraph = nullptr, *cbase = nullptr;
    int64_t static_rows = 0;
    int pocket_groups = 0;
    bool caching;
    bool chunked;
    GraphPlan plan;
    float *pred_pos, *pred_v;
    hipGraph_t graph;
    hipGraphExec_t graph_exec;
    td_step_io graph_io;
    unsigned graph_epoch = 0;
    int eager_steps;
    bool graph_failed, last_step_graph;
    const float *prog_table = nullptr;
    std::vector<int32_t> prog_kinds;
    size_t prog_next = 0;
};

namespace tdapi {
constexpr int TD_STEP_LISTS_MAX_NODES = 12288;

GraphTab session_tab(td_session *S) {
    GraphTab gt = S->chunked ? plan_tab(S->plan) : default_tab(S->w);
    if (S->caching) gt.mixed = S->dirty_count;
    return gt;
}

void free_async_or_sync(void *p, hipStream_t s) {
    if (!p) return;
    if (hipFreeAsync(p, s) == hipSuccess) return;
    (void)hipGetLastError();
    (void)hipDeviceSynchronize();
    (void)hipFree(p);
}

void session_drop_graph(td_session *S) {
    if (S->graph_exec) (void)hipStreamSynchronize(S->last_stream);
    if (S->graph_exec) (void)hipGraphExecDestroy(S->graph_exec);
    if (S->graph) (void)hipGraphDestroy(S->graph);
    S->graph_exec = nullptr;
    S->graph = nullptr;
}

void session_free(td_session *S, hipStream_t s) {
    if (!S) return;
    session_drop_graph(S);
    if (S->chunked) plan_destroy(S->plan, s);
    free_async_or_sync(S->block, s);
    delete S;
}
}

extern "C" int td_session_create(const td_model *m, const float *d_protein_pos, const float *d_protein_v,
                                 const int32_t *d_protein_ptr, int64_t N_p, const int32_t *d_ligand_ptr, int64_t N_l,
                                 int64_t B, int32_t max_graph_nodes, void *stream, td_session **out) {
    if (!m || !out || N_p <= 0 || N_l <= 0 || B <= 0 || !d_protein_pos || !d_protein_v || !d_protein_ptr || !d_ligand_ptr) {
        td_set_error("td_session_create: bad argument");
        return TD_EINVAL;
    }
    hipStream_t s = static_cast<hipStream_t>(stream);
    const int64_t N = N_p + N_l;
    td_session *S = new (std::nothrow) td_session();
    if (!S) { td_set_error("td_session_create: out of host memory"); return TD_ENOMEM; }
    S->m = m; S->N = N; S->Np = N_p; S->Nl = N_l; S->B = B; S->max_graph_nodes = max_graph_nodes; S->last_stream = s;
    S->chunked = !default_graph(m->cfg);
    int rc;
    std::vector<int32_t> hp, hl;
    if ((rc = fetch_ptrs(d_protein_ptr, d_ligand_ptr, B, hp, hl, s)) != TD_OK) { delete S; return rc; }
    int gmax = 0;
    for (int64_t g = 0; g < B; ++g) gmax = std::max(gmax, (hp[g + 1] - hp[g]) + (hl[g + 1] - hl[g]));
    S->graph_nodes_max = gmax;
    const bool knn_like = m->cfg.cutoff_mode == TD_CUTOFF_KNN || m->cfg.cutoff_mode == TD_CUTOFF_HYBRID;
    S->caching = knn_like && (!S->chunked || gmax <= TD_STEP_LISTS_MAX_NODES) && num_blocks(m->cfg) == 1 && m->cfg.ew_net_type == 0 &&
                 !m->cfg.x2h_out_fc && !m->cfg.sync_twoup && stage_rows(m->cfg) == 1;
    if (S->chunked && (rc = plan_create(m->cfg, hp.data(), hl.data(), B, s, &S->plan)) != TD_OK) { delete S; return rc; }
    const int64_t NC = S->chunked ? S->plan.NC : N;
    const int KS = S->chunked ? 64 : TD_K;
// ... 12 lines not shown
        std::vector<int32_t> flag((size_t)B, 0);
        cgraph_h.assign((size_t)B, 0); cbase_h.assign((size_t)B, 0);
        auto bail = [&](int r) { free_async_or_sync(tg, s); delete S; return r; };
        if ((rc = td_launch_pocket_hash(d_protein_pos, d_protein_v, d_protein_ptr, B, F, d_hash, s)) != TD_OK) return bail(rc);
        if (hipMemcpyAsync(hash.data(), d_hash, (size_t)B * 8, hipMemcpyDeviceToHost, s) != hipSuccess || hipStreamSynchronize(s) != hipSuccess) {
            td_set_error("td_session_create: reading the pocket hashes failed"); return bail(TD_EHIP);
        }
        {
            std::map<std::pair<int32_t, unsigned long long>, int32_t> first;
            for (int64_t g = 0; g < B; ++g)
                cgraph_h[(size_t)g] = first.emplace(std::make_pair(hp[g + 1] - hp[g], hash[(size_t)g]), (int32_t)g).first->second;
        }
        hipError_t e2 = hipMemcpyAsync(d_cand, cgraph_h.data(), (size_t)B * 4, hipMemcpyHostToDevice, s);
        if (e2 == hipSuccess) e2 = hipMemsetAsync(d_flag, 0, (size_t)B * 4, s);
        if (e2 != hipSuccess) { td_set_error("td_session_create: pocket grouping failed: %s", hipGetErrorString(e2)); return bail(TD_EHIP); }
        if ((rc = td_launch_pocket_verify(d_protein_pos, d_protein_v, d_protein_ptr, B, F, d_cand, d_flag, s)) != TD_OK) return bail(rc);
        if (hipMemcpyAsync(flag.data(), d_flag, (size_t)B * 4, hipMemcpyDeviceToHost, s) != hipSuccess || hipStreamSynchronize(s) != hipSuccess) {
            td_set_error("td_session_create: reading the pocket comparison failed"); return bail(TD_EHIP);
        }
        free_async_or_sync(tg, s);
        Nc = 0;
        for (int64_t g = 0; g < B; ++g) {
            if (flag[(size_t)g]) cgraph_h[(size_t)g] = (int32_t)g;
            const int32_t c = cgraph_h[(size_t)g];
            if (c == (int32_t)g) {
                cbase_h[(size_t)g] = (int32_t)Nc;
                const int32_t n0 = hp[g] + hl[g], np = hp[g + 1] - hp[g];
                for (int32_t a = 0; a < np; ++a) canon_rows_h.push_back(n0 + a);
                Nc += np;
                ++S->pocket_groups;
            } else {
                cbase_h[(size_t)g] = cbase_h[(size_t)c];
            }
        }
        S->static_rows = Nc;
    }

    const size_t ws_bytes = carve(nullptr, N, B, N_l).bytes;
    size_t off = ws_bytes;
    auto reserve = [&](size_t n) { size_t o = off; off += align_up(n ? n : 4); return o; };
    const size_t n = (size_t)N, nc = (size_t)NC;
    const bool C = S->caching;
    const size_t ns = share ? (size_t)Nc : n, ncs = share ? (size_t)Nc : nc;
    const size_t o_prot = reserve((size_t)N_p * 4), o_pptr = reserve((size_t)(B + 1) * 4), o_lptr = reserve((size_t)(B + 1) * 4),
                 o_h0 = reserve(ns * TD_H * 4), o_tmp_lpos = reserve((size_t)N_l * 12), o_tmp_lv = reserve((size_t)N_l * 8),
                 o_snbr = reserve(C ? ncs * TD_K * 4 : 0), o_skeys = reserve(C ? ns * KS * 8 : 0), o_ews = reserve(C ? ncs * TD_K * 4 : 0),
                 o_h1s = reserve(C ? ns * TD_H * 4 : 0), o_h2s = reserve(C ? ns * TD_H * 4 : 0), o_f2 = reserve(C ? n : 0),
                 o_frows = reserve(C ? n * 4 : 0), o_frest = reserve(C ? n * 4 : 0), o_fcnt = reserve(256),
                 o_P0 = reserve(C ? n * 4 * TD_H * 4 : 0), o_q0 = reserve(C ? n * TD_H * 4 : 0), o_clean = reserve(C ? n : 0),
                 o_dirty = reserve(C ? n * 4 : 0), o_dcnt = reserve(256), o_hop = reserve(C ? n * 4 * TD_HOP_LEVELS : 0),
                 o_hcnt = reserve(256), o_dchunks = reserve(C && S->chunked ? nc * 4 : 0),
                 o_ppos = reserve((size_t)N_l * 3 * 4), o_pv = reserve((size_t)N_l * TD_MAXC * 4),
                 o_cg = reserve(share ? (size_t)B * 4 : 0), o_cb = reserve(share ? (size_t)B * 4 : 0), o_crows = reserve(share ? (size_t)Nc * 4 : 0);
    hipError_t e = td_malloc_async(reinterpret_cast<void **>(&S->block), off, s);
    if (e != hipSuccess) {
        td_set_error("td_session_create: hipMallocAsync(%zu) failed: %s", off, hipGetErrorString(e));
        S->block = nullptr;
        session_free(S, s);
        return TD_ENOMEM;
    }
    char *b = S->block;
    S->w = carve(b, N, B, N_l);
    S->prot_node = reinterpret_cast<int32_t *>(b + o_prot);
    S->pptr = reinterpret_cast<int32_t *>(b + o_pptr);
    S->lptr = reinterpret_cast<int32_t *>(b + o_lptr);
    S->snbr = reinterpret_cast<int32_t *>(b + o_snbr);
    S->skeys = reinterpret_cast<unsigned long long *>(b + o_skeys);
    S->ews = reinterpret_cast<float *>(b + o_ews);
    S->h0 = reinterpret_cast<float *>(b + o_h0);
    S->h1s = reinterpret_cast<float *>(b + o_h1s);
    S->h2s = reinterpret_cast<float *>(b + o_h2s);
    S->flags2 = reinterpret_cast<uint8_t *>(b + o_f2);
    S->fwd_rows = reinterpret_cast<int32_t *>(b + o_frows);
    S->fwd_rest = reinterpret_cast<int32_t *>(b + o_frest);
    S->fwd_counts = reinterpret_cast<int32_t *>(b + o_fcnt);
    S->use_fwd = C && m->opt.session_forward_reach && m->cfg.num_layers >= 2;
    S->P0 = reinterpret_cast<float *>(b + o_P0);
    S->q0 = reinterpret_cast<float *>(b + o_q0);
    S->clean = reinterpret_cast<uint8_t *>(b + o_clean);
    S->dirty_rows = reinterpret_cast<int32_t *>(b + o_dirty);
    S->dirty_count = reinterpret_cast<int32_t *>(b + o_dcnt);
    S->hop_rows = reinterpret_cast<int32_t *>(b + o_hop);
    S->hop_count = reinterpret_cast<int32_t *>(b + o_hcnt);
    S->dirty_chunks = reinterpret_cast<int32_t *>(b + o_dchunks);
    S->pred_pos = reinterpret_cast<float *>(b + o_ppos);
    S->pred_v = reinterpret_cast<float *>(b + o_pv);
    int32_t *canon_rows = nullptr;
    if (share) {
        S->cgraph = reinterpret_cast<int32_t *>(b + o_cg);
        S->cbase = reinterpret_cast<int32_t *>(b + o_cb);
        canon_rows = reinterpret_cast<int32_t *>(b + o_crows);
    }
    {
        int lv = m->opt.session_hop_levels;
        if (lv < 1) lv = 1;
        if (lv > TD_HOP_LEVELS) lv = TD_HOP_LEVELS;
        if (lv > m->cfg.num_layers) lv = m->cfg.num_layers;
        S->hop_levels = lv;
    }
    float *tmp_lpos = reinterpret_cast<float *>(b + o_tmp_lpos);
    int64_t *tmp_lv = reinterpret_cast<int64_t *>(b + o_tmp_lv);
    Workspace &w = S->w;
    auto fail = [&](int r) { session_free(S, s); return r; };
#define TD_TRY(expr) do { if ((rc = (expr)) != TD_OK) return fail(rc); } while (0)
#define TD_TRY_HIP(expr) do { hipError_t _e = (expr); if (_e != hipSuccess) { td_set_error("%s failed: %s", #expr, hipGetErrorString(_e)); return fail(TD_EHIP); } } while (0)
    TD_TRY_HIP(hipMemcpyAsync(S->pptr, d_protein_ptr, (size_t)(B + 1) * 4, hipMemcpyDeviceToDevice, s));
    TD_TRY_HIP(hipMemcpyAsync(S->lptr, d_ligand_ptr, (size_t)(B + 1) * 4, hipMemcpyDeviceToDevice, s));
    TD_TRY_HIP(hipMemsetAsync(tmp_lpos, 0, (size_t)N_l * 12, s));
    TD_TRY_HIP(hipMemsetAsync(tmp_lv, 0, (size_t)N_l * 8, s));
    char *scratch = nullptr;
    float *h0_f = S->h0, *h1_f = S->h1s, *h2_f = S->h2s, *ews_f = S->ews;
    int32_t *snbr_f = S->snbr;
    unsigned long long *skeys_f = S->skeys;
    const int32_t *set_rows = S->prot_node;
    int64_t set_count = N_p;
    auto fail2 = [&](int r) { free_async_or_sync(scratch, s); return fail(r); };
    if (share) {
        const size_t b_keys = align_up(n * TD_K * 8), b_nbr = align_up(n * TD_K * 4), b_h = align_up(n * TD_H * 4);
        const size_t sb = b_keys + 2 * b_nbr + 3 * b_h;
        hipError_t se = td_malloc_async(reinterpret_cast<void **>(&scratch), sb, s);
        if (se != hipSuccess) { td_set_error("td_session_create: hipMallocAsync(%zu) failed: %s", sb, hipGetErrorString(se)); scratch = nullptr; return fail(TD_ENOMEM); }
        skeys_f = reinterpret_cast<unsigned long long *>(scratch);
        snbr_f = reinterpret_cast<int32_t *>(scratch + b_keys);
        ews_f = reinterpret_cast<float *>(scratch + b_keys + b_nbr);
        h0_f = reinterpret_cast<float *>(scratch + b_keys + 2 * b_nbr);
        h1_f = reinterpret_cast<float *>(scratch + b_keys + 2 * b_nbr + b_h);
        h2_f = reinterpret_cast<float *>(scratch + b_keys + 2 * b_nbr + 2 * b_h);
        hipError_t ue = hipMemcpyAsync(S->cgraph, cgraph_h.data(), (size_t)B * 4, hipMemcpyHostToDevice, s);
        if (ue == hipSuccess) ue = hipMemcpyAsync(S->cbase, cbase_h.data(), (size_t)B * 4, hipMemcpyHostToDevice, s);
        if (ue == hipSuccess) ue = hipMemcpyAsync(canon_rows, canon_rows_h.data(), (size_t)Nc * 4, hipMemcpyHostToDevice, s);
        if (ue == hipSuccess) ue = hipStreamSynchronize(s);
        if (ue != hipSuccess) { td_set_error("td_session_create: uploading the pocket groups failed: %s", hipGetErrorString(ue)); return fail2(TD_EHIP); }
    }
#undef TD_TRY
#undef TD_TRY_HIP
#define TD_TRY(expr) do { if ((rc = (expr)) != TD_OK) return fail2(rc); } while (0)
#define TD_TRY_HIP(expr) do { hipError_t _e = (expr); if (_e != hipSuccess) { td_set_error("%s failed: %s", #expr, hipGetErrorString(_e)); return fail2(TD_EHIP); } } while (0)
    int32_t *prot_out = S->chunked ? S->plan.prot_node : S->prot_node;
    TD_TRY(td_launch_compose(m, d_protein_pos, d_protein_v, S->pptr, N_p, tmp_lpos, tmp_lv, S->lptr, N_l, B, h0_f, w.x4a,
                             w.node_ptr, w.gid, w.lig_node, prot_out, s));
    if (S->chunked) {
        S->prot_node = S->plan.prot_node;
        TD_TRY(plan_layout(S->plan, w.node_ptr, w.gid, s));
    }
    set_rows = share ? canon_rows : S->prot_node;
    set_count = share ? Nc : N_p;
    TD_TRY_HIP(hipMemcpyAsync(w.x4b, w.x4a, n * sizeof(float4), hipMemcpyDeviceToDevice, s));
    if (!S->caching) {
        *out = S;
        return TD_OK;
    }
    GraphTab gt = session_tab(S);
    GraphTab st = gt;
    st.nbr = snbr_f; st.ew = ews_f;
    TD_TRY_HIP(hipMemsetAsync(snbr_f, 0xff, nc * TD_K * 4, s));
    if (S->chunked) {
        TD_TRY(td_launch_knn_general_static(w.x4a, w.node_ptr, S->pptr, w.gid, S->prot_node, N_p, m->cfg.knn, gmax, S->plan.cptr,
                                            S->snbr, S->skeys, s));
        TD_TRY(td_launch_gate(m->gate, w.x4a, S->snbr, NC, nullptr, nullptr, S->ews, s, S->plan.chunk_node));
        TD_TRY_HIP(hipMemsetAsync(S->plan.cnbr, 0xff, nc * TD_K * 4, s));
        TD_TRY_HIP(hipMemsetAsync(S->plan.ew, 0, nc * TD_K * 4, s));
        if (m->cfg.cutoff_mode == TD_CUTOFF_HYBRID)
            TD_TRY(td_launch_hybrid_ligand_half(w.node_ptr, S->pptr, w.gid, w.lig_node, N_l, S->plan.cptr, S->plan.cnbr, s));
    } else {
        TD_TRY(td_launch_knn_static(w.x4a, w.node_ptr, w.gid, set_rows, set_count, max_graph_nodes, snbr_f, skeys_f, s, m->cfg.knn));
        TD_TRY(td_launch_gate(m->gate, w.x4a, snbr_f, set_count, set_rows, nullptr, ews_f, s));
    }
    const TdLayer &L0 = m->layers[0];
    TD_TRY(td_launch_node_proj(L0.nodeX2h, h0_f, N, nullptr, 0x1f, S->P0, S->q0, s));
    TD_TRY(key_pass(L0.hk, L0, w.x4a, st, st.ew, st.nbr, S->P0, S->q0, set_rows, nullptr, set_count, gt.alpha, s));
    TD_TRY_HIP(hipMemcpyAsync(h1_f, h0_f, n * TD_H * 4, hipMemcpyDeviceToDevice, s));
    TD_TRY(value_pass(L0.hv, L0, w.x4a, st, st.nbr, S->P0, set_rows, nullptr, set_count, h1_f, gt.alpha, nullptr, 0, s));
    if (S->use_fwd) {
        const TdLayer &L1 = m->layers[1];
        TD_TRY(td_launch_node_proj(L1.nodeX2h, h1_f, N, nullptr, 0x1f, w.P, w.q, s));
        TD_TRY(key_pass(L1.hk, L1, w.x4a, st, st.ew, st.nbr, w.P, w.q, set_rows, nullptr, set_count, gt.alpha, s));
        TD_TRY_HIP(hipMemcpyAsync(h2_f, h1_f, n * TD_H * 4, hipMemcpyDeviceToDevice, s));
        TD_TRY(value_pass(L1.hv, L1, w.x4a, st, st.nbr, w.P, set_rows, nullptr, set_count, h2_f, gt.alpha, nullptr, 0, s));
    }
    if (share) {
        TD_TRY(td_launch_compact_rows(skeys_f, canon_rows, Nc, TD_K * 8, S->skeys, s));
        TD_TRY(td_launch_compact_rows(snbr_f, canon_rows, Nc, TD_K * 4, S->snbr, s));
        TD_TRY(td_launch_compact_rows(ews_f, canon_rows, Nc, TD_K * 4, S->ews, s));
        TD_TRY(td_launch_compact_rows(h0_f, canon_rows, Nc, TD_H * 4, S->h0, s));
        TD_TRY(td_launch_compact_rows(h1_f, canon_rows, Nc, TD_H * 4, S->h1s, s));
        if (S->use_fwd) TD_TRY(td_launch_compact_rows(h2_f, canon_rows, Nc, TD_H * 4, S->h2s, s));
        free_async_or_sync(scratch, s);
        scratch = nullptr;
    }
#undef TD_TRY
#undef TD_TRY_HIP
    *out = S;
    return TD_OK;
}

extern "C" void td_session_destroy(td_session *S) {
    if (!S) return;
    session_free(S, S->last_stream);
}

extern "C" int td_session_forward(td_session *S, const float *d_ligand_pos, const int64_t *d_ligand_v,
                                  float *d_pred_ligand_pos, float *d_pred_ligand_v, float *d_final_ligand_h,
                                  const float *d_ligand_graph_bias, void *stream) {
    if (!S || !d_ligand_pos || !d_ligand_v || !d_pred_ligand_pos || !d_pred_ligand_v) {
        td_set_error("td_session_forward: null pointer");
        return TD_EINVAL;
    }
    hipStream_t s = static_cast<hipStream_t>(stream);
    S->last_stream = s;
    const td_model *m = S->m;
    Workspace &w = S->w;
    const int64_t N = S->N, Nl = S->Nl, Np = S->Np;
    const GraphTab gt = session_tab(S);
    int rc;
    if (!S->caching) {
        {
            ProfScope ps(PC_COMPOSE, s);
            TD_CHECK_HIP(hipMemcpyAsync(w.h, S->h0, (size_t)N * TD_H * sizeof(float), hipMemcpyDeviceToDevice, s));
            if ((rc = td_launch_ligand_update(m, d_ligand_pos, d_ligand_v, w.lig_node, Nl, w.h, w.x4a, s, nullptr, d_ligand_graph_bias, w.gid)) != TD_OK) return rc;
        }
        float4 *xg = nullptr;
        Workspace wb = w;
        rc = TD_OK;
        for (int blk = 0; rc == TD_OK && blk < num_blocks(m->cfg); ++blk) {
            if (S->chunked) rc = build_general_graph(m, S->plan, wb, N, Nl, S->max_graph_nodes, s);
            else rc = build_default_graph(m, wb, N, S->max_graph_nodes, s);
            if (rc == TD_OK) rc = run_backbone(m, wb, gt, wb.h, N, Nl, 0, &xg, s, true);
            if (rc == TD_OK && xg == wb.x4b) std::swap(wb.x4a, wb.x4b);
        }
        if (rc != TD_OK) return rc;
        ProfScope ps(PC_HEAD, s);
        return td_launch_head(m->head, w.h, xg, w.lig_node, Nl, m->cfg.ligand_num_classes, d_pred_ligand_pos, d_pred_ligand_v,
                              d_final_ligand_h, s);
    }
    {
        ProfScope ps(PC_COMPOSE, s);
        TdStepReset rs;
        rs.c0 = S->dirty_count; rs.n0 = 2;
        rs.c1 = S->fwd_counts; rs.n1 = 2;
        rs.c2 = S->hop_count; rs.n2 = TD_HOP_LEVELS;
        rs.flags2 = S->use_fwd ? S->flags2 : nullptr;
        if ((rc = td_launch_ligand_update(m, d_ligand_pos, d_ligand_v, w.lig_node, Nl, w.h, w.x4a, s, &rs, d_ligand_graph_bias, w.gid)) != TD_OK) return rc;
    }
    bool lists_done = false;
    {
        ProfScope ps(PC_KNN, s);
        const TdStepLists lists{S->dirty_rows, S->dirty_count, S->use_fwd ? S->fwd_rows : nullptr, S->fwd_rest, S->fwd_counts,
                                S->hop_rows, S->hop_count, S->hop_levels, S->chunked ? S->dirty_chunks : nullptr,
                                S->chunked ? S->dirty_count + 1 : nullptr};
        if (S->chunked) {
            const GraphPlan &p = S->plan;
            if ((rc = td_launch_knn_merge_general(w.x4a, w.node_ptr, S->pptr, w.gid, S->prot_node, Np, S->skeys, S->snbr, S->h0,
                                                  S->h1s, S->ews, p.cptr, p.cpn_p, p.cnbr, w.h, p.ew, S->clean,
                                                  S->use_fwd ? S->flags2 : nullptr, s, m->cfg.knn)) != TD_OK) return rc;
            if ((rc = td_launch_ligand_rows_general(p.mode, w.x4a, w.node_ptr, S->pptr, w.gid, w.lig_node, Nl, p.k, S->graph_nodes_max,
                                                    p.cptr, p.cnbr, s)) != TD_OK) return rc;
            if ((rc = td_launch_step_lists(S->clean, w.x4a, p.cnbr, w.node_ptr, N, S->B, S->graph_nodes_max, lists, s, p.cptr,
                                           p.chunk_node)) != TD_OK) {
                if (rc == TD_EINVAL) td_set_error("td_session_forward: a graph of %d nodes does not fit the row-list kernel", S->graph_nodes_max);
                return rc;
            }
            lists_done = true;
        } else {
            if ((rc = td_launch_knn_merge(w.x4a, w.node_ptr, S->pptr, w.gid, S->prot_node, Np, S->skeys, S->snbr, S->h0,
                                          S->h1s, S->ews, w.nbr, w.h, w.ew, S->clean, S->use_fwd ? S->flags2 : nullptr, s, m->cfg.knn,
                                          w.lig_node, Nl, S->max_graph_nodes, S->cgraph, S->cbase)) != TD_OK) return rc;
            rc = (m->opt.session_step_lists && S->graph_nodes_max > 0) ? td_launch_step_lists(S->clean, w.x4a, w.nbr, w.node_ptr, N, S->B, S->graph_nodes_max, lists, s)
                                        : TD_EINVAL;
            lists_done = rc == TD_OK;
            if (rc != TD_OK && rc != TD_EINVAL) return rc;
            if (!lists_done) {
                if ((rc = td_launch_compact_dirty(S->clean, w.x4a, N, S->dirty_rows, S->dirty_count, s)) != TD_OK) return rc;
                if (S->use_fwd) {
                    if ((rc = td_launch_forward_reach(S->clean, w.x4a, w.nbr, N, S->flags2, S->fwd_rows, S->fwd_rest, S->fwd_counts,
                                                      S->clean, s)) != TD_OK) return rc;
                } else {
                    TD_CHECK_HIP(hipMemsetAsync(S->clean, 0, (size_t)N, s));
                }
            }
        }
    }
    {
        ProfScope ps(PC_GATE, s);
        if (S->chunked)
            rc = td_launch_gate(m->gate, w.x4a, gt.nbr, S->plan.NC, S->dirty_chunks, S->dirty_count + 1, gt.ew, s, S->plan.chunk_node);
        else
            rc = td_launch_gate(m->gate, w.x4a, gt.nbr, N, S->dirty_rows, S->dirty_count, gt.ew, s);
        if (rc != TD_OK) return rc;
    }
    const TdLayer &L0 = m->layers[0];
    {
        { ProfScope ps(PC_NODE, s); if ((rc = td_launch_node_proj(L0.nodeX2h, w.h, Nl, w.lig_node, 0x1f, S->P0, S->q0, s)) != TD_OK) return rc; }
        { ProfScope ps(PC_X2H_K, s); if ((rc = key_pass(L0.hk, L0, w.x4a, gt, gt.ew, gt.nbr, S->P0, S->q0, S->dirty_rows, S->dirty_count, N, gt.alpha, s, w.lig_node, Nl)) != TD_OK) return rc; }
        { ProfScope ps(PC_X2H_V, s); if ((rc = value_pass(L0.hv, L0, w.x4a, gt, gt.nbr, S->P0, S->dirty_rows, S->dirty_count, N, w.h, gt.alpha, w.lig_node, Nl, s)) != TD_OK) return rc; }
    }
    if (!lists_done && (rc = td_launch_hop_levels(w.lig_node, Nl, w.nbr, N, S->clean, S->hop_rows, S->hop_count, S->hop_levels, s, true)) != TD_OK) return rc;
    float4 *xf = nullptr;
    const FwdReach fwd{S->fwd_rows, S->fwd_rest, S->fwd_counts, S->h2s, S->cbase};
    if ((rc = run_backbone(m, w, gt, w.h, N, Nl, 0, &xf, s, false, true, S->hop_rows, S->hop_count, S->hop_levels,
                           S->use_fwd ? &fwd : nullptr)) != TD_OK) return rc;
    ProfScope ps(PC_HEAD, s);
    return td_launch_head(m->head, w.h, xf, w.lig_node, Nl, m->cfg.ligand_num_classes, d_pred_ligand_pos,
                          d_pred_ligand_v, d_final_ligand_h, s);
}

namespace tdapi {
int session_step_issue(td_session *S, const td_step_io &io, hipStream_t s) {
    const td_model *m = S->m;
    int rc = td_session_forward(S, io.d_ligand_pos, io.d_ligand_v, S->pred_pos, S->pred_v, nullptr, io.d_ligand_graph_bias, s);
    if (rc != TD_OK) return rc;
    ProfScope ps(PC_POST, s);
    return td_launch_posterior_step(m->sched, m->cfg.num_timesteps, io.d_step, io.d_t_all, io.num_steps, S->lptr, S->Nl, S->B,
                                    m->cfg.ligand_num_classes, io.d_ligand_pos, io.d_ligand_v, S->pred_pos, S->pred_v, io.d_noise,
                                    io.d_uniform, io.d_pos_traj, io.d_v_traj, io.d_v0_traj, io.d_vt_traj, io.pos_only, s,
                                    m->cfg.model_mean_type, io.d_fixed_mask, io.d_fixed_mask ? io.d_fixed_pos : nullptr,
                                    io.d_fixed_mask ? io.d_fixed_v : nullptr, S->prog_table);
}
}

// ... 45 lines not shown
    }
    const bool graph_ok = use_graph && !S->graph_failed && g_prof.mask == 0 && !td_wg_trace_armed();
    if (graph_ok && S->graph_exec && (memcmp(&S->graph_io, io, sizeof(td_step_io)) != 0 || S->graph_epoch != S->m->option_epoch)) session_drop_graph(S);
    if (graph_ok && !S->graph_exec && S->eager_steps > 0) {
        hipError_t e = hipStreamBeginCapture(s, hipStreamCaptureModeRelaxed);
        if (e == hipSuccess) {
            const int rc = session_step_issue(S, *io, s);
            hipGraph_t g = nullptr;
            e = hipStreamEndCapture(s, &g);
            if (rc == TD_OK && e == hipSuccess && g) {
                e = hipGraphInstantiate(&S->graph_exec, g, nullptr, nullptr, 0);
                if (e == hipSuccess) { S->graph = g; S->graph_io = *io; S->graph_epoch = S->m->option_epoch; }
                else { (void)hipGraphDestroy(g); S->graph_exec = nullptr; }
            } else if (g) {
                (void)hipGraphDestroy(g);
            }
        }
        if (!S->graph_exec) {
            (void)hipGetLastError();
            S->graph_failed = true;
        }
    }
    if (graph_ok && S->graph_exec) {
        S->last_stream = s;
        TD_CHECK_HIP(hipGraphLaunch(S->graph_exec, s));
        S->last_step_graph = true;
        return TD_OK;
    }
    const int rc = session_step_issue(S, *io, s);
    if (rc == TD_OK) ++S->eager_steps;
    return rc;
}

extern "C" int td_session_step_graph(const td_session *S) { return S && S->last_step_graph ? 1 : 0; }

extern "C" int td_session_row_counts(td_session *S, int32_t *host_counts, int32_t n_counts, void *stream) {
    if (!S || !host_counts || n_counts < 2) { td_set_error("td_session_row_counts: bad argument"); return TD_EINVAL; }
    hipStream_t s = static_cast<hipStream_t>(stream);
    host_counts[0] = (int32_t)S->N;
    if (!S->caching) {
        host_counts[1] = (int32_t)S->N;
        for (int k = 2; k < n_counts; ++k) host_counts[k] = -1;
        return TD_OK;
    }
    TD_CHECK_HIP(hipMemcpyAsync(host_counts + 1, S->dirty_count, sizeof(int32_t), hipMemcpyDeviceToHost, s));
    for (int k = 2; k < n_counts; ++k) host_counts[k] = -1;
    const int room = n_counts - 2 < TD_HOP_LEVELS ? n_counts - 2 : TD_HOP_LEVELS;
    const int lv = S->hop_levels < room ? S->hop_levels : room;
    if (lv > 0) TD_CHECK_HIP(hipMemcpyAsync(host_counts + 2, S->hop_count, sizeof(int32_t) * (size_t)lv, hipMemcpyDeviceToHost, s));
    if (n_counts > 2 + TD_HOP_LEVELS && S->use_fwd)
        TD_CHECK_HIP(hipMemcpyAsync(host_counts + 2 + TD_HOP_LEVELS, S->fwd_counts, sizeof(int32_t), hipMemcpyDeviceToHost, s));
    if (n_counts > 3 + TD_HOP_LEVELS) host_counts[3 + TD_HOP_LEVELS] = S->cgraph ? (int32_t)S->static_rows : -1;
    if (n_counts > 4 + TD_HOP_LEVELS) host_counts[4 + TD_HOP_LEVELS] = S->cgraph ? (int32_t)S->pocket_groups : -1;
    TD_CHECK_HIP(hipStreamSynchronize(s));
    return TD_OK;
}
```

targetdiff_amd/csrc/td_api.h:

```cpp
#pragma once

#include <atomic>
#include <mutex>
#include <vector>

#include "td_internal.h"

void td_set_error(const char *fmt, ...);

namespace tdapi {

enum { PC_KNN = 0, PC_GATE, PC_NODE, PC_X2H_K, PC_X2H_V, PC_H2X_K, PC_H2X_V, PC_COMPOSE, PC_HEAD, PC_POST, PC_COUNT };
struct Profiler {
    std::atomic<unsigned> mask{0};
    std::mutex mu;
    std::vector<hipEvent_t> ev[PC_COUNT];
    std::vector<hipEvent_t> pool;
    hipEvent_t get() {
        {
            std::lock_guard<std::mutex> lk(mu);
            if (!pool.empty()) { hipEvent_t e = pool.back(); pool.pop_back(); return e; }
        }
        hipEvent_t e = nullptr;
        (void)hipEventCreate(&e);
// ... 43 lines not shown

inline int num_x2h(const td_config &c) { return c.num_x2h > 0 ? c.num_x2h : 1; }
inline int num_h2x(const td_config &c) { return c.num_h2x > 0 ? c.num_h2x : 1; }
inline int stage_rows(const td_config &c) { return num_x2h(c) > num_h2x(c) ? num_x2h(c) : num_h2x(c); }

inline int kv_in(const td_config &c) { return 2 * c.hidden_dim + c.edge_feat_dim + 4 * c.num_r_gaussian; }

inline bool config_supported(const td_config &c) {
    const bool graph_ok = (c.cutoff_mode == TD_CUTOFF_KNN && c.knn >= 1 && c.knn <= TD_MAX_FANIN) ||
                          (c.cutoff_mode == TD_CUTOFF_HYBRID && c.knn >= 1 && c.knn <= TD_MAX_FANIN) ||
                          (c.cutoff_mode == TD_CUTOFF_RADIUS && c.radius > 0.f && c.max_num_neighbors >= 1 &&
                           c.max_num_neighbors <= TD_MAX_FANIN);
    return c.hidden_dim == TD_H && c.n_heads == TD_HEADS && graph_ok && c.num_r_gaussian == TD_NG &&
           c.edge_feat_dim == 4 && c.num_layers >= 1 && c.protein_feat_dim >= 1 && c.protein_feat_dim <= 32 &&
           c.ligand_num_classes >= 1 && c.ligand_num_classes <= TD_MAXC && c.num_timesteps >= 1;
}

inline bool caching_graph(const td_config &c) { return c.cutoff_mode == TD_CUTOFF_KNN && c.knn <= TD_K; }
inline bool default_graph(const td_config &c) {
    return caching_graph(c) || (c.cutoff_mode == TD_CUTOFF_RADIUS && c.max_num_neighbors <= TD_K);
}


struct Packer {
    std::vector<float> data;
    size_t alloc(size_t n) {
        size_t off = (data.size() + 63) & ~size_t(63);
        data.resize(off + n, 0.f);
        return off;
    }
};

size_t pack_B128(Packer &pk, const float *W, int ld, int col0);
size_t pack_B128_split(Packer &pk, const float *W, int ld, int col0);
size_t pack_vec(Packer &pk, const float *v, size_t n, size_t padded = 0);
float gaussian_coeff(const float *off);
inline size_t align_up(size_t v, size_t a = 256) { return (v + a - 1) / a * a; }

struct Workspace {
    float4 *x4a, *x4b;
    int32_t *gid, *nbr, *lig_node, *node_ptr;
    float *ew, *P, *q, *h, *alpha;
    float *Px, *qx;
    size_t bytes;
};

struct GraphTab {
    const int32_t *cptr;
    int32_t *nbr;
    float *ew, *alpha;
    int cpn_p;
    int64_t NCl;
    const int32_t *mixed;
};

struct FwdReach {
    const int32_t *rows, *rest, *counts;
    const float *hs;
    const int32_t *cbase = nullptr;
};

struct GraphPlan {
    int mode = 0, k = 0, cpn_p = 1;
    float radius = 0.f;
    int64_t N = 0, Np = 0, Nl = 0, B = 0, NC = 0, NCl = 0;
    char *block = nullptr;
    int32_t *cptr = nullptr, *chunk_node = nullptr, *lig_chunks = nullptr, *cnbr = nullptr, *prot_node = nullptr, *pptr = nullptr, *meta = nullptr;
    float *ew = nullptr, *alpha = nullptr;
};

Workspace carve(char *base, int64_t N, int64_t B, int64_t Nl);
inline GraphTab default_tab(Workspace &w) { return GraphTab{nullptr, w.nbr, w.ew, w.alpha, 1, 0, nullptr}; }
inline GraphTab plan_tab(const GraphPlan &p) { return GraphTab{p.cptr, p.cnbr, p.ew, p.alpha, p.cpn_p, p.NCl, nullptr}; }
inline int num_blocks(const td_config &c) { return c.num_blocks > 1 ? c.num_blocks : 1; }
int key_pass(const TdEdgeMlp &mlp, const TdLayer &L, const float4 *x4, const GraphTab &gt, const float *ew, const int32_t *nbr,
             const float *P, const float *q, const int32_t *rows, const int32_t *count_ptr, int64_t count, float *alpha, hipStream_t s,
             const int32_t *lig = nullptr, int64_t Nl = 0, bool h2x_stage = false);
int value_pass(const TdEdgeMlp &mlp, const TdLayer &L, const float4 *x4, const GraphTab &gt, const int32_t *nbr, const float *P,
               const int32_t *rows, const int32_t *count_ptr, int64_t count, float *h, const float *alpha, const int32_t *lig,
               int64_t Nl, hipStream_t s, float *out = nullptr);
int h2x_project(const TdLayer &L, Workspace &w, float *h, int64_t N, int64_t Nl, float *P, float *q,
                const int32_t *hop_rows, const int32_t *hop_count, hipStream_t s);
int h2x_attend(const td_model *m, const TdLayer &L, Workspace &w, const GraphTab &gt, int64_t Nl, float4 *xc, float4 *xn, float *P,
               float *q, hipStream_t s);
int run_backbone(const td_model *m, Workspace &w, const GraphTab &gt, float *h, int64_t N, int64_t Nl, int fix_x,
                 float4 **x_final, hipStream_t s, bool init_xn, bool layer0_x2h_done = false,
                 const int32_t *hop_rows = nullptr, const int32_t *hop_count = nullptr, int hop_levels = 0,
                 const FwdReach *fwd = nullptr);
int build_default_graph(const td_model *m, Workspace &w, int64_t N, int max_graph_nodes, hipStream_t s);
extern std::atomic<int> g_fail_alloc;
hipError_t td_malloc_async(void **p, size_t bytes, hipStream_t s);
void free_async_or_sync(void *p, hipStream_t s);
void plan_destroy(GraphPlan &p, hipStream_t s);
int plan_create(const td_config &c, const int32_t *host_pptr, const int32_t *host_lptr, int64_t B, hipStream_t s, GraphPlan *out);
int plan_layout(GraphPlan &p, const int32_t *node_ptr, const int32_t *gid, hipStream_t s);
int build_general_graph(const td_model *m, GraphPlan &p, Workspace &w, int64_t N, int64_t Nl, int max_graph_nodes, hipStream_t s);
int plan_from_mask(const td_config &c, const uint8_t *d_mask, const int32_t *d_node_ptr, int64_t N, int64_t B, hipStream_t s,
                   GraphPlan *out, int64_t *nl_out);
int fetch_ptrs(const int32_t *d_a, const int32_t *d_b, int64_t B, std::vector<int32_t> &a, std::vector<int32_t> &b, hipStream_t s);
struct AsyncScratch {
    hipStream_t s;
    std::vector<void *> blocks;
    explicit AsyncScratch(hipStream_t st) : s(st) {}
    AsyncScratch(const AsyncScratch &) = delete;
    AsyncScratch &operator=(const AsyncScratch &) = delete;
    ~AsyncScratch() { for (void *b : blocks) free_async_or_sync(b, s); }
// ... 17 lines not shown
```

targetdiff_amd/csrc/td_internal.h:

```cpp
#pragma once

#include <hip/hip_runtime.h>
#include <stddef.h>
#include <stdint.h>

#include <atomic>

#include "../../include/targetdiff_hip.h"

constexpr int TD_H = 128;
constexpr int TD_HEADS = 16;
constexpr int TD_DH = 8;
constexpr int TD_K = 32;
constexpr int TD_NG = 20;
constexpr int TD_SLOTK = 24;
constexpr int TD_SLOT_STEPS = TD_SLOTK / 2;
constexpr int TD_KSTEPS = TD_H / 2;
constexpr int TD_MAXC = 16;
constexpr int TD_SMALL_BATCH_ROWS = 16384;

void td_set_error(const char *fmt, ...);
#define TD_CHECK_HIP(expr)                                                                       \
    do {                                                                                         \
        hipError_t _e = (expr);                                                                  \
// ... 81 lines not shown
    const float *bp;
    const float *WlT;
    const float *bl;
};

struct TdHead {
    const float *W0T;
    const float *b0;
    const float *W2T;
    const float *b2;
};

struct TdEgnnLayer {
    TdNodeStage proj;
    const float *W2f;
    const float *Wxf;
    const float *vec;
    const float *nodeB;
    const float *nb1, *nb2;
};

constexpr int TD_PROP_H = 256;
constexpr int TD_PROP_G = 64;
constexpr int TD_PROP_ACT_NONE = 0, TD_PROP_ACT_RELU = 1, TD_PROP_ACT_SSP = 2;
constexpr int TD_PROP_EPI_NONE = 0, TD_PROP_EPI_RELU_MASK = 1, TD_PROP_EPI_SSP_DERIV = 2;
constexpr int TD_PROP_XTY_CHUNKS = 64;
struct TdPropLayer {
    const float *projW, *projB;
    const float *W1f;
    const float *W2f;
    const float *b2, *winf, *binf;
    const float *offset;
    const float *n1W, *n1b, *n2W, *n2b;
};

struct TdSchedules {
    const float *c0, *ct, *logvar, *log_a, *log_1ma, *log_ca, *log_1mca;
    const float *abar;
    const float *rc, *rm1;
};

struct TdOptions {
    int h2x_fused = 1;
    int node_proj_split = 1;
    int edge_key_split = 1;
    int edge_first_layer_f16 = 1;
    int edge_second_layer_f16 = 1;
    int session_hop_levels = 4;
    int session_forward_reach = 1;
    int edge_row_dealing = 2;
    int node_proj_bpipe = 0;
    int node_proj_async = 1;
    int session_share_pockets = 1;
    int session_step_lists = 1;
};

struct td_model {
    td_config cfg;
    TdOptions opt;
    float *blob;
    size_t blob_floats;
    TdEmbed emb;
    TdGate gate;
    TdLayer *layers;
    TdHead head;
    TdSchedules sched;
    unsigned option_epoch = 0;
    int fold_dead_units = 0;
    int fold_fp32_mlps = 0;
};

int td_launch_graph_ptr(const int64_t *batch, int64_t N, int64_t B, int32_t *ptr, hipStream_t s);
int td_launch_node_gid(const int32_t *node_ptr, int64_t N, int64_t B, int32_t *gid, hipStream_t s);
int td_launch_pack_x(const float *x3, const uint8_t *mask, int64_t N, float4 *x4, hipStream_t s);
int td_launch_unpack_x(const float4 *x4, int64_t N, float *x3, hipStream_t s);
int td_launch_knn(const float4 *x4, const int32_t *node_ptr, const int32_t *gid, int64_t N, int max_graph_nodes,
                  int32_t *nbr, hipStream_t s, int k = TD_K);
int td_launch_compose(const td_model *m, const float *ppos, const float *pv, const int32_t *pptr, int64_t Np,
                      const float *lpos, const int64_t *lv, const int32_t *lptr, int64_t Nl, int64_t B,
                      float *h, float4 *x4, int32_t *node_ptr, int32_t *gid, int32_t *lig_node, int32_t *prot_node,
                      hipStream_t s, const float *gbias = nullptr);
int td_launch_knn_rows(const float4 *x4, const int32_t *node_ptr, const int32_t *gid, const int32_t *rows, int64_t count,
                       int max_graph_nodes, int32_t *nbr, hipStream_t s, int k = TD_K);
int td_launch_knn_static(const float4 *x4, const int32_t *node_ptr, const int32_t *gid, const int32_t *rows, int64_t count,
                         int max_graph_nodes, int32_t *nbr, unsigned long long *skeys, hipStream_t s, int k = TD_K);
int td_launch_knn_merge(const float4 *x4, const int32_t *node_ptr, const int32_t *pptr, const int32_t *gid,
                        const int32_t *prot_rows, int64_t Np, const unsigned long long *skeys, const int32_t *snbr,
                        const float *h0, const float *h1s, const float *ews, int32_t *nbr, float *h, float *ew,
                        uint8_t *clean, uint8_t *flags2, hipStream_t s, int k = TD_K, const int32_t *lig_rows = nullptr, int64_t Nl = 0,
                        int max_graph_nodes = 0, const int32_t *cgraph = nullptr, const int32_t *cbase = nullptr);
int td_launch_pocket_hash(const float *ppos, const float *pv, const int32_t *pptr, int64_t B, int F, unsigned long long *out, hipStream_t s);
int td_launch_pocket_verify(const float *ppos, const float *pv, const int32_t *pptr, int64_t B, int F, const int32_t *cand, int32_t *flags,
                            hipStream_t s);
int td_launch_compact_rows(const void *src, const int32_t *rows, int64_t n_rows, int row_bytes, void *dst, hipStream_t s);
int td_launch_compact_dirty(const uint8_t *clean, const float4 *x4, int64_t N, int32_t *rows, int32_t *count,
                            hipStream_t s);
int td_launch_forward_reach(const uint8_t *clean, const float4 *x4, const int32_t *nbr, int64_t N, uint8_t *flags2,
                            int32_t *rows_on, int32_t *rows_off, int32_t *counts2, uint8_t *clean_to_zero, hipStream_t s);
int td_launch_restore_rows(const int32_t *rows, const int32_t *count_ptr, int64_t max_rows, const float *hs, float *h,
                           hipStream_t s, const int32_t *gid = nullptr, const int32_t *node_ptr = nullptr, const int32_t *cbase = nullptr);
constexpr int TD_HOP_LEVELS = 4;
int td_launch_hop_levels(const int32_t *lig_node, int64_t Nl, const int32_t *nbr, int64_t N, uint8_t *flags,
                         int32_t *rows, int32_t *counts, int levels, hipStream_t s, bool zeroed = false);
int td_launch_gate16(const TdGate &g, const float4 *x4, const int32_t *nbr, int64_t N, const int32_t *rows,
                     const int32_t *count_ptr, float *ew, hipStream_t s, const int32_t *chunk_node);
struct TdStepLists {
    int32_t *dirty_rows, *dirty_count;
    int32_t *reach_rows, *rest_rows, *reach_counts;
    int32_t *level_rows, *level_counts;
    int levels;
    int32_t *dirty_chunks = nullptr, *dirty_chunk_count = nullptr;
};
int td_launch_step_lists(const uint8_t *clean, const float4 *x4, const int32_t *nbr, const int32_t *node_ptr, int64_t N,
                         int64_t B, int max_nodes, const TdStepLists &out, hipStream_t s, const int32_t *cptr = nullptr,
                         const int32_t *chunk_node = nullptr);
struct TdStepReset {
    int32_t *c0 = nullptr, *c1 = nullptr, *c2 = nullptr;
    int n0 = 0, n1 = 0, n2 = 0;
    uint8_t *flags2 = nullptr;
};
int td_launch_ligand_update(const td_model *m, const float *lpos, const int64_t *lv, const int32_t *lig_node, int64_t Nl,
                            float *h, float4 *x4, hipStream_t s, const TdStepReset *reset = nullptr, const float *gbias = nullptr,
                            const int32_t *gid = nullptr);
int td_launch_ligand_list(const uint8_t *mask, int64_t N, int32_t *lig_node, int32_t *count, hipStream_t s);
int td_launch_node_proj(const TdNodeStage &st, const float *h, int64_t N, const int32_t *rows, unsigned mat_mask,
                        float *P, float *q, hipStream_t s, const int32_t *count_ptr = nullptr,
                        const int32_t *rows2 = nullptr, int64_t N2 = 0, unsigned mask2 = 0);
int td_launch_node_proj_pair(const TdNodeStage &hx, const int32_t *hop_rows, const int32_t *hop_count,
                             const int32_t *lig_rows, int64_t Nl, float *Px, float *qx, const TdNodeStage &nx,
                             const int32_t *rows, const int32_t *count_ptr, float *P, float *q, const float *h, int64_t N,
                             hipStream_t s);
int td_launch_node_output(const TdNodeOut &no, const float *out, float *h, int64_t N, hipStream_t s);
int td_launch_layer_gate(const float *w, const float *offsets, float coeff, const float4 *x4, const int32_t *nbr, int64_t N, float *ew,
                         hipStream_t s);
int td_launch_gate(const TdGate &g, const float4 *x4, const int32_t *nbr, int64_t N, const int32_t *rows,
                   const int32_t *count_ptr, float *ew, hipStream_t s, const int32_t *chunk_node = nullptr);
int td_launch_edge_key16(const TdEdgeMlp &mlp, const TdLayer &L, const float4 *x4, const int32_t *nbr, const float *ew,
                         const float *P, const float *q, const int32_t *rows, const int32_t *count_ptr, int64_t count,
                         float *alpha, hipStream_t s, bool h2x_stage, const int32_t *cptr = nullptr, const int32_t *lig_rows = nullptr,
                         int64_t lig_count = 0, int cpn_p = 0);
int td_launch_edge_h2x16(const TdEdgeMlp &mlp_k, const TdEdgeMlp &mlp_v, const TdLayer &L, const float4 *x4_in, float4 *x4_out,
                         const int32_t *nbr, const float *ew, const float *P, const float *q, const int32_t *rows,
                         int64_t count, hipStream_t s, const int32_t *cptr = nullptr, float *alpha = nullptr);
int td_launch_edge_xv16(const TdEdgeMlp &mlp, const TdLayer &L, const float4 *x4_in, float4 *x4_out, const int32_t *nbr,
                        const float *P, const int32_t *rows, int64_t count, const float *alpha, hipStream_t s,
                        const int32_t *cptr = nullptr);
int td_launch_edge_value16(const TdEdgeMlp &mlp, const TdLayer &L, const float4 *x4, const int32_t *nbr, const float *P,
                           const int32_t *rows, const int32_t *count_ptr, int64_t count, float *h, const float *alpha, const int32_t *lig_rows, int64_t lig_count,
                           hipStream_t s, const int32_t *cptr = nullptr, int cpn_p = 1, int64_t lig_chunks = 0,
                           const int32_t *mixed_count = nullptr, float *out = nullptr, const float *gate_m = nullptr);
int td_set_wg_trace(unsigned long long *buf, int slots);
bool td_wg_trace_armed();
int td_launch_layout(const int32_t *node_ptr, const int32_t *pptr, const int32_t *gid, const int32_t *g_cbase,
                     const int32_t *g_cl, const int32_t *g_lbase, int cpn_p, int64_t N, int32_t *cptr, int32_t *chunk_node,
                     int32_t *lig_chunks, int32_t total_chunks, hipStream_t s);
int td_launch_graph_general(int mode, const float4 *x4, const int32_t *node_ptr, const int32_t *pptr, const int32_t *gid,
                            const int32_t *prot_node, int64_t Np, const int32_t *lig_node, int64_t Nl, int64_t N, int k,
                            float radius, int max_graph_nodes, const int32_t *cptr, int32_t *cnbr, int64_t NC, hipStream_t s);
int td_launch_knn_general_static(const float4 *x4, const int32_t *node_ptr, const int32_t *pptr, const int32_t *gid,
                                 const int32_t *prot_rows, int64_t Np, int k, int max_graph_nodes, const int32_t *cptr,
                                 int32_t *snbr, unsigned long long *skeys, hipStream_t s);
int td_launch_ligand_rows_general(int mode, const float4 *x4, const int32_t *node_ptr, const int32_t *pptr, const int32_t *gid,
                                  const int32_t *lig_node, int64_t Nl, int k, int max_graph_nodes, const int32_t *cptr,
                                  int32_t *cnbr, hipStream_t s);
int td_launch_hybrid_ligand_half(const int32_t *node_ptr, const int32_t *pptr, const int32_t *gid, const int32_t *lig_node,
                                 int64_t Nl, const int32_t *cptr, int32_t *cnbr, hipStream_t s);
int td_launch_knn_merge_general(const float4 *x4, const int32_t *node_ptr, const int32_t *pptr, const int32_t *gid,
                                const int32_t *prot_rows, int64_t Np, const unsigned long long *skeys, const int32_t *snbr,
                                const float *h0, const float *h1s, const float *ews, const int32_t *cptr, int cpn, int32_t *nbr,
                                float *h, float *ew, uint8_t *clean, uint8_t *flags2, hipStream_t s, int k);
int td_launch_radius32(const float4 *x4, const int32_t *node_ptr, const int32_t *gid, int64_t N, float radius, int cap,
                       int32_t *nbr, hipStream_t s);
int td_launch_slots_to_dense(const int32_t *cptr, const int32_t *cnbr, int64_t N, int width, int32_t *out, hipStream_t s);
int td_launch_head(const TdHead &hd, const float *h, const float4 *x4, const int32_t *lig_node, int64_t Nl,
                   int classes, float *pred_pos, float *pred_v, float *lig_h, hipStream_t s);
int td_launch_posterior(const TdSchedules &sc, int T, const int32_t *t, const int32_t *lptr, int64_t Nl, int64_t B,
                        int classes, const float *pos, const int64_t *v, const float *pred_pos,
                        const float *pred_v, const float *noise, const float *uni, float *pos_next,
                        int64_t *v_next, float *log_v0, float *log_post, hipStream_t s, int mean_type = 0,
                        const uint8_t *fixed_mask = nullptr, const float *fixed_pos = nullptr, const int64_t *fixed_v = nullptr,
                        const float *prow = nullptr);
int td_launch_posterior_step(const TdSchedules &sc, int T, int32_t *step, const int32_t *t_all, int num_steps, const int32_t *lptr,
                             int64_t Nl, int64_t B, int classes, float *pos, int64_t *v, const float *pred_pos, const float *pred_v,
                             const float *noise, const float *uni, float *pos_traj, int64_t *v_traj, float *v0_traj, float *vt_traj,
                             int pos_only, hipStream_t s, int mean_type = 0, const uint8_t *fixed_mask = nullptr,
                             const float *fixed_pos = nullptr, const int64_t *fixed_v = nullptr, const float *prog_table = nullptr);
int td_launch_renoise(const float *prow, int64_t Nl, int classes, const float *pos, const int64_t *v, const float *noise,
                      const float *uni, float *pos_next, int64_t *v_next, float *log_v0, float *log_q, hipStream_t s);
int td_launch_renoise_step(const float *prog_table, int32_t *step, int num_steps, int64_t Nl, int classes, float *pos, int64_t *v,
                           const float *noise, const float *uni, float *pos_traj, int64_t *v_traj, float *v0_traj, float *vt_traj,
                           int pos_only, hipStream_t s);
int td_launch_egnn_edge(const TdEgnnLayer &L, const float4 *x4, float4 *x4_out, const int32_t *nbr, const float *P, float *mi,
                        int64_t N, hipStream_t s);
int td_launch_egnn_node(const TdEgnnLayer &L, const float *mi, float *h, int64_t N, hipStream_t s);
int td_launch_prop_linear(const float *X1, int K1, const float *X2, int K2, const float *W, const float *bias, const float *R, float *Y,
                          int64_t N, int O, int act, hipStream_t s);
int td_launch_prop_compose(const float *hp, const float *hl, const float *pp, const float *pl, const int32_t *protein_ptr,
                           const int32_t *ligand_ptr, float *h, float *x, int32_t *node_ptr, int64_t B, hipStream_t s);
int td_launch_prop_edge(const TdPropLayer &L, const float *x, const int32_t *nbr, int k, const float *P, float *mi, int64_t N,
                        float coeff, hipStream_t s);
int td_launch_prop_segment_sum(const float *h, const int32_t *node_ptr, const float *enc_graph, int Eg, float *pre_out, int64_t B,
                               hipStream_t s);
int td_launch_prop_select(const float *y, const int64_t *kind, int O, float *out, int64_t B, hipStream_t s);
// ... 29 lines not shown
```

Before: 26.65.

## Precompute static protein-row edge Gaussian operands once per session and reuse them

Protein rows whose neighbour lists never change across sampling steps get their first-layer f16 Gaussian-distance operand quads precomputed once at session creation into a per-row table. The key and value edge kernels check a row-to-table index and, for static rows, load the stored quads instead of recomputing distances and exp2. Elsewhere the row uses the original computation. This saves per-step ALU work on protein edges, at the cost of up to 64 MB of extra memory, an extra table read per row, and more branching and register pressure in the hot kernels.

After: 26.18. -1.8%, worse.

```diff
diff --git a/targetdiff_amd/capi.py b/targetdiff_amd/capi.py
--- a/targetdiff_amd/capi.py
+++ b/targetdiff_amd/capi.py
@@ -630,6 +630,10 @@
         n = self._counts()
         return (int(n[7]), int(n[8])) if n[7] >= 0 else None
 
+    def static_operand_rows(self):
+        v = int(self._counts()[9])
+        return v if v >= 0 else None
+
     @_device_bound
     def _counts(self):
         n = (c_int32 * 10)()
diff --git a/targetdiff_amd/csrc/edge16.hip b/targetdiff_amd/csrc/edge16.hip
--- a/targetdiff_amd/csrc/edge16.hip
+++ b/targetdiff_amd/csrc/edge16.hip
@@ -117,6 +117,8 @@
     const int32_t *mixed_count;
     int deal;
     unsigned long long *trace;
+    const int32_t *srow;
+    const uint4 *otab;
 };
 
 __device__ __forceinline__ void td_trace_wave_end(unsigned long long *trace, int lane) {
@@ -593,6 +595,29 @@
     }
 }
 
+__device__ __forceinline__ void td_edge_gauss5(const float4 xi, const float4 xj, const float (&offj)[8], float c2, float (&rel)[3],
+                                               float (&gv)[5]) {
+#pragma clang fp contract(off)
+    const float rx = xi.x - xj.x, ry = xi.y - xj.y, rz = xi.z - xj.z;
+    const float dist = td_sqrt_d2(__builtin_fmaf(rz, rz, __builtin_fmaf(rx, rx, ry * ry)));
+    rel[0] = rx; rel[1] = ry; rel[2] = rz;
+#pragma unroll
+    for (int j = 0; j < 5; ++j) {
+        const float u = dist - offj[j];
+        gv[j] = __builtin_amdgcn_exp2f(c2 * (u * u));
+    }
+}
+
+constexpr int TD_OTAB_ROW_U4 = 4 * 64;
+static_assert((size_t)TD_OTAB_ROW_U4 * sizeof(uint4) == TD_OTAB_ROW_BYTES, "operand table row");
+__device__ __forceinline__ void td_static_bquads16(const float4 xi, const float4 (&xj)[2], const float (&offj)[8], float c2, uint4 (&bq)[2][2]) {
+    float gv[2][5], rel[3];
+#pragma unroll
+    for (int eb = 0; eb < 2; ++eb) td_edge_gauss5(xi, xj[eb], offj, c2, rel, gv[eb]);
+    const unsigned ct[2] = {0x3c000000u, 0x3c000000u};
+    td_h2_bquads<2>(gv, ct, bq);
+}
+
 struct TdNoHook { __device__ __forceinline__ void operator()() const {} };
 template <bool LOAD_EW, bool ONE_CLASS, bool PI_LATE, int NEB, bool LN_SKIP, int PK, int AH = 0, class Hook = TdNoHook, bool NO_LN = false>
 __device__ __forceinline__ void td_first_layer_split16(const Args16 &a, const uint4 *__restrict__ Rp,
@@ -634,18 +659,11 @@
         ed.valid[eb] = r.j[eb] >= 0;
         const float4 xj = r.xj[eb];
         if (LOAD_EW) ed.ew[eb] = r.ew[eb];
-        const float rx = xi.x - xj.x, ry = xi.y - xj.y, rz = xi.z - xj.z;
-        const float dist = td_sqrt_d2(rx * rx + ry * ry + rz * rz);
-        ed.rel[eb][0] = rx; ed.rel[eb][1] = ry; ed.rel[eb][2] = rz;
+        td_edge_gauss5(xi, xj, offj, c2, ed.rel[eb], gv[eb]);
         slot[eb] = xj.w > 0.5f ? 0 : 1;
         has[0][eb] = __ballot(ed.valid[eb] && slot[eb] == 0) != 0ull;
         has[1][eb] = __ballot(ed.valid[eb] && slot[eb] == 1) != 0ull;
         ed.any[eb] = has[0][eb] || has[1][eb];
-#pragma unroll
-        for (int j = 0; j < 5; ++j) {
-            const float u = dist - offj[j];
-            gv[eb][j] = __builtin_amdgcn_exp2f(c2 * (u * u));
-        }
     }
     before_products();
     auto products4 = [&](int sl) {
@@ -697,6 +715,54 @@
     const TdLn ln{a.mlp.ln_c1, a.mlp.ln_c2};
     if (NEB == 2 && LN_SKIP) td_ln_relu16_skip(KB, g, acc, ln, ed.any);
     else td_ln_relu16<NEB>(KB, g, acc, ln);
+}
+
+template <bool LOAD_EW>
+__device__ __forceinline__ void td_row_gather_static16(const Args16 &a, int64_t i, int64_t c, int sr, int lane, RowIn16 &r,
+                                                       floatx4_t (&acc)[2][8], uint4 (&tq)[2][2]) {
+    const int lo = lane & 15, g = lane >> 4;
+    const uint4 *tp = a.otab + (size_t)sr * TD_OTAB_ROW_U4 + lane;
+    tq[0][0] = tp[0]; tq[1][0] = tp[64]; tq[0][1] = tp[128]; tq[1][1] = tp[192];
+#pragma unroll
+    for (int eb = 0; eb < 2; ++eb) {
+        const int jj = r.j[eb] >= 0 ? r.j[eb] : (int)i;
+        if (LOAD_EW) r.ew[eb] = a.ew[c * TD_K + 16 * eb + lo];
+        const float *pj = a.P + (size_t)jj * (4 * TD_H) + a.p_off + TD_H + 4 * g;
+#pragma unroll
+        for (int hb = 0; hb < 8; ++hb) {
+            const float4 v = *reinterpret_cast<const float4 *>(pj + 16 * hb);
+            acc[eb][hb][0] = v.x; acc[eb][hb][1] = v.y; acc[eb][hb][2] = v.z; acc[eb][hb][3] = v.w;
+        }
+    }
+}
+template <bool LOAD_EW, bool AHEAD, class Hook = TdNoHook, bool NO_LN = false>
+__device__ __forceinline__ void td_first_layer_static16(const Args16 &a, const uint4 *__restrict__ Rs, const float *__restrict__ KB,
+                                                        const RowIn16 &r, const uint4 (&tq)[2][2], int64_t i, int lane,
+                                                        floatx4_t (&acc)[2][8], Edge2 &ed, Hook before_products = Hook()) {
+    const int g = lane >> 4;
+    ed.xi = r.xi;
+    {
+        const float *pp = a.P + (size_t)i * (4 * TD_H) + a.p_off + 4 * g;
+#pragma unroll
+        for (int hb = 0; hb < 8; ++hb) {
+            const float4 pi = *reinterpret_cast<const float4 *>(pp + 16 * hb);
+#pragma unroll
+            for (int eb = 0; eb < 2; ++eb) {
+                acc[eb][hb][0] += pi.x; acc[eb][hb][1] += pi.y; acc[eb][hb][2] += pi.z; acc[eb][hb][3] += pi.w;
+            }
+        }
+    }
+#pragma unroll
+    for (int eb = 0; eb < 2; ++eb) {
+        ed.valid[eb] = r.j[eb] >= 0;
+        ed.any[eb] = true;
+        if (LOAD_EW) ed.ew[eb] = r.ew[eb];
+        ed.rel[eb][0] = ed.rel[eb][1] = ed.rel[eb][2] = 0.f;
+    }
+    before_products();
+    td_h2_tiles<AHEAD, 2>(Rs, tq, acc);
+    if constexpr (NO_LN) return;
+    td_ln_relu16<2>(KB, g, acc, TdLn{a.mlp.ln_c1, a.mlp.ln_c2});
 }
 
 template <bool LOAD_EW, bool SKIP_EMPTY = false>
@@ -739,6 +805,7 @@
     static_assert(L2 == 0 || (SPLIT && !XV && STAGE == 0), "f16 logits: x2h key pass, bf16 first layer");
     static_assert(FL == 0 || SPLIT, "f16 first layer: the 16-bit instantiations");
     constexpr int KPK = FL ? 5 : TD_KEY_PK;
+    constexpr bool SOPS = !XV && STAGE == 0 && GRAPH == 0 && SPLIT && FL == 1 && L2 != 0;
     constexpr int RF = SPLIT ? e16q_u4<KPK>() * 4 : E16_R_FLOATS;
     constexpr int NOFF = SPLIT ? 8 : E16_STEPS;
     extern __shared__ __attribute__((aligned(16))) float lds[];
@@ -797,6 +864,22 @@
         if constexpr (SPLIT) {
             RowIn16 rin;
             td_row_index16(a, i, c, lane, rin);
+            auto fetch_q = [&]() {
+                if constexpr (!XV && !CHUNKED) {
+                    qpre0 = *reinterpret_cast<const float4 *>(a.q + (size_t)i * TD_H + 8 * lo);
+                    qpre1 = *reinterpret_cast<const float4 *>(a.q + (size_t)i * TD_H + 8 * lo + 4);
+                }
+            };
+            if constexpr (SOPS) {
+                const int sr = a.otab ? __builtin_amdgcn_readfirstlane(a.srow[i]) : -1;
+                if (sr >= 0) {
+                    uint4 tq[2][2];
+                    td_row_gather_static16<EW>(a, i, c, sr, lane, rin, acc, tq);
+                    td_first_layer_static16<EW, TD_KEY_AH != 0, decltype(fetch_q), L2H>(
+                        a, reinterpret_cast<const uint4 *>(lds) + (size_t)3 * e16q_cs_u4<5>() + lane, KB, rin, tq, i, lane, acc, ed, fetch_q);
+                    return;
+                }
+            }
             td_row_gather16<EW>(a, i, c, lane, rin, acc);
             float offr[8];
             {
@@ -806,12 +889,6 @@
                 const float4 o0 = op[0], o1 = op[1];
                 offr[0] = o0.x; offr[1] = o0.y; offr[2] = o0.z; offr[3] = o0.w; offr[4] = o1.x; offr[5] = o1.y; offr[6] = o1.z; offr[7] = o1.w;
             }
-            auto fetch_q = [&]() {
-                if constexpr (!XV && !CHUNKED) {
-                    qpre0 = *reinterpret_cast<const float4 *>(a.q + (size_t)i * TD_H + 8 * lo);
-                    qpre1 = *reinterpret_cast<const float4 *>(a.q + (size_t)i * TD_H + 8 * lo + 4);
-                }
-            };
             if (XV && CHUNKED && __ballot(rin.j[1] >= 0) == 0ull)
                 td_first_layer_split16<EW, false, false, 1, false, KPK>(a, reinterpret_cast<const uint4 *>(lds), KB, offr, rin, i, lane, acc, ed, fetch_q);
             else
@@ -1838,6 +1915,7 @@
     constexpr bool ZPLAIN = L2 == 2;
     constexpr int WAVES = V16T_WAVES;
     constexpr int VPK = FL ? 5 : V16T_PK;
+    constexpr bool SOPS = !VIA && FL == 1;
     constexpr int RF = e16q_half_u4<VPK>() * 4;
     extern __shared__ __attribute__((aligned(16))) float lds[];
     const int tid = threadIdx.x, lane = tid & 63, wid = tid >> 6;
@@ -1907,33 +1985,51 @@
         td_row_index16(a, i, c, lane, rin);
         if (((__builtin_amdgcn_readfirstlane(__float_as_int(rin.xi.w)) > __float_as_int(0.5f)) ? 0 : 1) != my_cls) continue;
         floatx4_t acc[2][8];
-        td_row_gather16<false>(a, i, c, lane, rin, acc);
-        float al[8];
-        if constexpr (L2 != 0) {
-            const float *ap = a.alpha + ((size_t)c * TD_HEADS + lo) * TD_K + 4 * g;
-            const float4 v0 = *reinterpret_cast<const float4 *>(ap), v1 = *reinterpret_cast<const float4 *>(ap + 16);
-            al[0] = v0.x; al[1] = v1.x; al[2] = v0.y; al[3] = v1.y; al[4] = v0.z; al[5] = v1.z; al[6] = v0.w; al[7] = v1.w;
-        } else {
-            const float *ap = a.alpha + ((size_t)c * TD_HEADS + lo) * TD_K + 8 * g;
-            const float4 v0 = *reinterpret_cast<const float4 *>(ap), v1 = *reinterpret_cast<const float4 *>(ap + 4);
-            al[0] = v0.x; al[1] = v0.y; al[2] = v0.z; al[3] = v0.w; al[4] = v1.x; al[5] = v1.y; al[6] = v1.z; al[7] = v1.w;
-        }
-        const float hres0 = a.h[(size_t)i * TD_H + nout], hres1 = a.h[(size_t)i * TD_H + nout + 4];
+        float al[8], hres0, hres1, ssum;
         Edge2 ed;
-        float offr[8];
-        {
-            int dep = 0;
-            asm volatile("" : "+v"(dep));
-            const float4 *op = reinterpret_cast<const float4 *>(B2 + 2 * TD_H + 4 + 8 * g + dep);
-            const float4 o0 = op[0], o1 = op[1];
-            offr[0] = o0.x; offr[1] = o0.y; offr[2] = o0.z; offr[3] = o0.w; offr[4] = o1.x; offr[5] = o1.y; offr[6] = o1.z; offr[7] = o1.w;
-        }
-        float ssum = ((al[0] + al[1]) + (al[2] + al[3])) + ((al[4] + al[5]) + (al[6] + al[7]));
-        ssum = td_sum_groups(ssum);
+        auto side_loads = [&]() {
+            if constexpr (L2 != 0) {
+                const float *ap = a.alpha + ((size_t)c * TD_HEADS + lo) * TD_K + 4 * g;
+                const float4 v0 = *reinterpret_cast<const float4 *>(ap), v1 = *reinterpret_cast<const float4 *>(ap + 16);
+                al[0] = v0.x; al[1] = v1.x; al[2] = v0.y; al[3] = v1.y; al[4] = v0.z; al[5] = v1.z; al[6] = v0.w; al[7] = v1.w;
+            } else {
+                const float *ap = a.alpha + ((size_t)c * TD_HEADS + lo) * TD_K + 8 * g;
+                const float4 v0 = *reinterpret_cast<const float4 *>(ap), v1 = *reinterpret_cast<const float4 *>(ap + 4);
+                al[0] = v0.x; al[1] = v0.y; al[2] = v0.z; al[3] = v0.w; al[4] = v1.x; al[5] = v1.y; al[6] = v1.z; al[7] = v1.w;
+            }
+            hres0 = a.h[(size_t)i * TD_H + nout]; hres1 = a.h[(size_t)i * TD_H + nout + 4];
+        };
+        auto sum_alpha = [&]() {
+            ssum = ((al[0] + al[1]) + (al[2] + al[3])) + ((al[4] + al[5]) + (al[6] + al[7]));
+            ssum = td_sum_groups(ssum);
+        };
+        auto live_row = [&]() {
+            td_row_gather16<false>(a, i, c, lane, rin, acc);
+            side_loads();
+            float offr[8];
+            {
+                int dep = 0;
+                asm volatile("" : "+v"(dep));
+                const float4 *op = reinterpret_cast<const float4 *>(B2 + 2 * TD_H + 4 + 8 * g + dep);
+                const float4 o0 = op[0], o1 = op[1];
+                offr[0] = o0.x; offr[1] = o0.y; offr[2] = o0.z; offr[3] = o0.w; offr[4] = o1.x; offr[5] = o1.y; offr[6] = o1.z; offr[7] = o1.w;
+            }
+            sum_alpha();
+            td_first_layer_split16<false, true, false, 2, false, VPK, V16T_AH, TdNoHook, L2 != 0>(a, reinterpret_cast<const uint4 *>(lds), KB, offr, rin, i, lane, acc, ed);
+        };
+        if constexpr (SOPS) {
+            const int sr = a.otab ? __builtin_amdgcn_readfirstlane(a.srow[i]) : -1;
+            if (sr >= 0) {
+                uint4 tq[2][2];
+                td_row_gather_static16<false>(a, i, c, sr, lane, rin, acc, tq);
+                side_loads();
+                sum_alpha();
+                td_first_layer_static16<false, V16T_AH != 0, TdNoHook, L2 != 0>(a, reinterpret_cast<const uint4 *>(lds) + e16q_cs_u4<5>() + lane, KB, rin, tq, i, lane, acc, ed);
+            } else live_row();
+        } else live_row();
         floatx4_t zb[8];
         constexpr float OUT_SCALE = L2 == 0 ? 1.0f : (ZPLAIN ? 1.0f / 1024.0f : 1.0f / (1024.0f * TD_Z_SCALE));
         if constexpr (L2 != 0) {
-        td_first_layer_split16<false, true, false, 2, false, VPK, V16T_AH, TdNoHook, true>(a, reinterpret_cast<const uint4 *>(lds), KB, offr, rin, i, lane, acc, ed);
         uint4 z1[8], z2[8];
         td_ln_relu16_pairs_eb<!ZPLAIN>(KB, g, acc, TdLn{a.mlp.ln_c1, a.mlp.ln_c2}, z1, z2);
         uint4 aq1, aq2;
@@ -1972,7 +2068,6 @@
             zb[hb] = td_mfma16h(zqb[hb & 1][0], aq1, zb[hb]);
         }
         } else {
-        td_first_layer_split16<false, true, false, 2, false, VPK, V16T_AH>(a, reinterpret_cast<const uint4 *>(lds), KB, offr, rin, i, lane, acc, ed);
         auto flip_store = [&](int hb) {
 #pragma unroll
             for (int eb = 0; eb < 2; ++eb)
@@ -2120,9 +2215,11 @@
 
 int td_launch_edge_key16(const TdEdgeMlp &mlp, const TdLayer &L, const float4 *x4, const int32_t *nbr, const float *ew,
                          const float *P, const float *q, const int32_t *rows, const int32_t *count_ptr, int64_t count,
-                         float *alpha, hipStream_t s, bool h2x_stage, const int32_t *cptr, const int32_t *lig_rows, int64_t lig_count, int cpn_p) {
+                         float *alpha, hipStream_t s, bool h2x_stage, const int32_t *cptr, const int32_t *lig_rows, int64_t lig_count, int cpn_p,
+                         const int32_t *srow, const void *otab) {
     if (count == 0) return TD_OK;
     Args16 a = {};
+    if (srow && otab && !cptr && !h2x_stage) { a.srow = srow; a.otab = static_cast<const uint4 *>(otab); }
     a.x4 = x4; a.nbr = nbr; a.ew = ew; a.P = P; a.q = q; a.rows = rows; a.count_ptr = count_ptr; a.h = nullptr;
     a.alpha = alpha; a.x4_out = nullptr; a.count = count; a.mlp = mlp; a.offsets = L.offsets; a.coeff = L.coeff; a.p_off = 0;
     a.cptr = cptr;
@@ -2231,9 +2328,11 @@
 int td_launch_edge_value16(const TdEdgeMlp &mlp, const TdLayer &L, const float4 *x4, const int32_t *nbr, const float *P,
                            const int32_t *rows, const int32_t *count_ptr, int64_t count, float *h, const float *alpha,
                            const int32_t *lig_rows, int64_t lig_count, hipStream_t s, const int32_t *cptr, int cpn_p,
-                           int64_t lig_chunks, const int32_t *mixed_count, float *out, const float *gate_m) {
+                           int64_t lig_chunks, const int32_t *mixed_count, float *out, const float *gate_m, const int32_t *srow,
+                           const void *otab) {
     if (count == 0) return TD_OK;
     Args16 a = {};
+    if (srow && otab && !cptr) { a.srow = srow; a.otab = static_cast<const uint4 *>(otab); }
     a.x4 = x4; a.nbr = nbr; a.ew = nullptr; a.P = P; a.q = nullptr; a.rows = rows; a.count_ptr = count_ptr; a.h = h;
     a.alpha = const_cast<float *>(alpha); a.x4_out = nullptr; a.count = count; a.mlp = mlp; a.offsets = L.offsets;
     a.coeff = L.coeff; a.p_off = 2 * TD_H; a.cptr = cptr; a.cpn_p = cpn_p > 0 ? cpn_p : 1; a.lig_chunks = lig_chunks;
@@ -2358,6 +2457,39 @@
     return TD_OK;
 }
 
+__global__ __launch_bounds__(256) void static_operands_kernel(const float4 *__restrict__ x4, const int32_t *__restrict__ snbr,
+                                                              const int32_t *__restrict__ rows, int64_t count,
+                                                              const float *__restrict__ offsets, float coeff, uint4 *__restrict__ otab) {
+    const int lane = threadIdx.x & 63, lo = lane & 15, g = lane >> 4;
+    const int64_t c = (int64_t)blockIdx.x * 4 + (threadIdx.x >> 6);
+    if (c >= count) return;
+    const int64_t i = rows[c];
+    float offj[8];
+#pragma unroll
+    for (int s8 = 0; s8 < 8; ++s8) offj[s8] = s8 < 5 ? offsets[5 * g + s8] : TD_FAR_CENTRE;
+    const float c2 = coeff * TD_LOG2E;
+    const float4 xi = x4[i];
+    float4 xj[2];
+#pragma unroll
+    for (int eb = 0; eb < 2; ++eb) {
+        const int j = snbr[i * TD_K + 16 * eb + lo];
+        xj[eb] = x4[j >= 0 ? j : (int)i];
+    }
+    uint4 bq[2][2];
+    td_static_bquads16(xi, xj, offj, c2, bq);
+    uint4 *tp = otab + (size_t)c * TD_OTAB_ROW_U4 + lane;
+    tp[0] = bq[0][0]; tp[64] = bq[1][0]; tp[128] = bq[0][1]; tp[192] = bq[1][1];
+}
+
+int td_launch_static_operands(const float4 *x4, const int32_t *snbr, const int32_t *rows, int64_t count, const TdLayer &L, void *otab,
+                              hipStream_t s) {
+    if (count == 0) return TD_OK;
+    static_operands_kernel<<<dim3((unsigned)((count + 3) / 4)), dim3(256), 0, s>>>(x4, snbr, rows, count, L.offsets, L.coeff,
+                                                                                 static_cast<uint4 *>(otab));
+    TD_CHECK_HIP(hipGetLastError());
+    return TD_OK;
+}
+
 int td_launch_gate16(const TdGate &g, const float4 *x4, const int32_t *nbr, int64_t N, const int32_t *rows,
                      const int32_t *count_ptr, float *ew, hipStream_t s, const int32_t *chunk_node) {
     if (N == 0) return TD_OK;
diff --git a/targetdiff_amd/csrc/graph.hip b/targetdiff_amd/csrc/graph.hip
--- a/targetdiff_amd/csrc/graph.hip
+++ b/targetdiff_amd/csrc/graph.hip
@@ -194,6 +194,7 @@
     const unsigned long long *skeys; const int32_t *snbr; const float *h0, *h1s, *ews; int32_t *nbr; float *h, *ew;
     uint8_t *clean, *flags2; int k;
     const int32_t *cgraph, *cbase;
+    int32_t *srow;
 };
 __device__ __forceinline__ void knn_merge_body(unsigned bid, const TdMergeArgs &ma) {
     const float4 *__restrict__ x4 = ma.x4;
@@ -236,6 +237,7 @@
         }
     }
     bool is_clean = !overflow && __ballot(closer) == 0ull;
+    const bool kept = is_clean;
     if (!is_clean && !overflow) {
         const bool c0 = kl[0] < thr, c1 = kl[1] < thr;
         const unsigned long long m0 = __ballot(c0), m1 = __ballot(c1);
@@ -310,6 +312,7 @@
     if (lane == 0) {
         clean[i] = is_clean ? 1 : 0;
         if (flags2) flags2[i] = 0;
+        if (ma.srow) ma.srow[i] = kept ? (int32_t)c : -1;
     }
 }
 
@@ -326,8 +329,8 @@
                         const int32_t *prot_rows, int64_t Np, const unsigned long long *skeys, const int32_t *snbr,
                         const float *h0, const float *h1s, const float *ews, int32_t *nbr, float *h, float *ew,
                         uint8_t *clean, uint8_t *flags2, hipStream_t s, int k, const int32_t *lig_rows, int64_t Nl,
-                        int max_graph_nodes, const int32_t *cgraph, const int32_t *cbase) {
-    const TdMergeArgs ma{x4, node_ptr, pptr, gid, prot_rows, Np, skeys, snbr, h0, h1s, ews, nbr, h, ew, clean, flags2, k, cgraph, cbase};
+                        int max_graph_nodes, const int32_t *cgraph, const int32_t *cbase, int32_t *srow) {
+    const TdMergeArgs ma{x4, node_ptr, pptr, gid, prot_rows, Np, skeys, snbr, h0, h1s, ews, nbr, h, ew, clean, flags2, k, cgraph, cbase, srow};
     const unsigned GA = (unsigned)((Np + 3) / 4), GB = lig_rows ? (unsigned)((Nl + 3) / 4) : 0u;
     if (GA + GB == 0) return TD_OK;
     if (GB == 0) {
diff --git a/targetdiff_amd/csrc/pack.cpp b/targetdiff_amd/csrc/pack.cpp
--- a/targetdiff_amd/csrc/pack.cpp
+++ b/targetdiff_amd/csrc/pack.cpp
@@ -487,9 +487,13 @@
         if (src) memcpy(pk.data.data() + dst, src, (4 * TD_NG + 1) * sizeof(float));
         else pk.data[dst + 4 * TD_NG] = 40.f;
     };
+    const float *off0 = nullptr;
+    bool offsets_uniform = true;
     for (int l = 0; l < L && cur.ok; ++l) {
         const float *off = cur.take(TD_NG);
         if (!cur.ok) break;
+        if (l == 0) off0 = off;
+        else if (memcmp(off, off0, TD_NG * sizeof(float)) != 0) offsets_uniform = false;
         const size_t ooff = pack_vec(pk, off, TD_NG);
         for (int i = 0; i < M; ++i) { lo[(size_t)l * M + i].off = ooff; lo[(size_t)l * M + i].coeff = gaussian_coeff(off); }
         for (int i = 0; i < NX; ++i) {
@@ -568,6 +572,7 @@
     m->cfg = c;
     m->blob_floats = pk.data.size();
     m->fold_dead_units = fold_dead;
+    m->offsets_uniform = offsets_uniform;
     m->layers = new (std::nothrow) TdLayer[(size_t)L * stage_rows(c)]();
     hipError_t e = hipMalloc(reinterpret_cast<void **>(&m->blob), m->blob_floats * sizeof(float));
     if (e == hipSuccess) e = hipMemcpy(m->blob, pk.data.data(), m->blob_floats * sizeof(float), hipMemcpyHostToDevice);
@@ -654,6 +659,8 @@
         m->opt.edge_first_layer_f16 = value != 0;
         for (int l = 0; l < m->cfg.num_layers * stage_rows(m->cfg); ++l)
             for (TdEdgeMlp *e : {&m->layers[l].hk, &m->layers[l].hv, &m->layers[l].xk, &m->layers[l].xv}) e->l1_f16 = e->R16h && e->f16_safe && value != 0;
+    } else if (strcmp(name, "edge_static_operands") == 0) {
+        m->opt.edge_static_operands = value != 0;
     } else if (strcmp(name, "edge_second_layer_f16") == 0) {
         m->opt.edge_second_layer_f16 = value != 0;
         for (int l = 0; l < m->cfg.num_layers * stage_rows(m->cfg); ++l)
@@ -682,6 +689,7 @@
     else if (strcmp(name, "edge_key_split") == 0) *value = m->opt.edge_key_split;
     else if (strcmp(name, "edge_second_layer_f16") == 0) *value = m->opt.edge_second_layer_f16;
     else if (strcmp(name, "edge_first_layer_f16") == 0) *value = m->opt.edge_first_layer_f16;
+    else if (strcmp(name, "edge_static_operands") == 0) *value = m->opt.edge_static_operands;
     else if (strcmp(name, "session_hop_levels") == 0) *value = m->opt.session_hop_levels;
     else if (strcmp(name, "session_forward_reach") == 0) *value = m->opt.session_forward_reach;
     else if (strcmp(name, "session_step_lists") == 0) *value = m->opt.session_step_lists;
diff --git a/targetdiff_amd/csrc/plan.cpp b/targetdiff_amd/csrc/plan.cpp
--- a/targetdiff_amd/csrc/plan.cpp
+++ b/targetdiff_amd/csrc/plan.cpp
@@ -42,13 +42,14 @@
 int key_pass(const TdEdgeMlp &mlp, const TdLayer &L, const float4 *x4, const GraphTab &gt, const float *ew, const int32_t *nbr,
              const float *P, const float *q, const int32_t *rows, const int32_t *count_ptr, int64_t count, float *alpha, hipStream_t s,
              const int32_t *lig, int64_t Nl, bool h2x_stage) {
-    return td_launch_edge_key16(mlp, L, x4, nbr, ew, P, q, rows, count_ptr, count, alpha, s, h2x_stage, gt.cptr, lig, Nl, gt.cpn_p);
+    return td_launch_edge_key16(mlp, L, x4, nbr, ew, P, q, rows, count_ptr, count, alpha, s, h2x_stage, gt.cptr, lig, Nl, gt.cpn_p, gt.srow,
+                                gt.otab);
 }
 int value_pass(const TdEdgeMlp &mlp, const TdLayer &L, const float4 *x4, const GraphTab &gt, const int32_t *nbr, const float *P,
                const int32_t *rows, const int32_t *count_ptr, int64_t count, float *h, const float *alpha, const int32_t *lig,
                int64_t Nl, hipStream_t s, float *out) {
     return td_launch_edge_value16(mlp, L, x4, nbr, P, rows, count_ptr, count, h, alpha, lig, Nl, s, gt.cptr, gt.cpn_p,
-                                  lig ? gt.NCl : 0, gt.mixed, out, L.gate_m);
+                                  lig ? gt.NCl : 0, gt.mixed, out, L.gate_m, gt.srow, gt.otab);
 }
 
 int h2x_project(const TdLayer &L, Workspace &w, float *h, int64_t N, int64_t Nl, float *P, float *q,
diff --git a/targetdiff_amd/csrc/session.cpp b/targetdiff_amd/csrc/session.cpp
--- a/targetdiff_amd/csrc/session.cpp
+++ b/targetdiff_amd/csrc/session.cpp
@@ -34,6 +34,8 @@
     int32_t *cgraph = nullptr, *cbase = nullptr;
     int64_t static_rows = 0;
     int pocket_groups = 0;
+    void *otab = nullptr;
+    int32_t *srow = nullptr;
     bool caching;
     bool chunked;
     GraphPlan plan;
@@ -50,11 +52,13 @@
 };
 
 namespace tdapi {
+constexpr size_t TD_OTAB_MAX_BYTES = (size_t)64 << 20;
 constexpr int TD_STEP_LISTS_MAX_NODES = 12288;
 
 GraphTab session_tab(td_session *S) {
     GraphTab gt = S->chunked ? plan_tab(S->plan) : default_tab(S->w);
     if (S->caching) gt.mixed = S->dirty_count;
+    if (S->otab && S->m->opt.edge_static_operands) { gt.srow = S->srow; gt.otab = S->otab; }
     return gt;
 }
 
@@ -173,6 +177,8 @@
                  o_hcnt = reserve(256), o_dchunks = reserve(C && S->chunked ? nc * 4 : 0),
                  o_ppos = reserve((size_t)N_l * 3 * 4), o_pv = reserve((size_t)N_l * TD_MAXC * 4),
                  o_cg = reserve(share ? (size_t)B * 4 : 0), o_cb = reserve(share ? (size_t)B * 4 : 0), o_crows = reserve(share ? (size_t)Nc * 4 : 0);
+    const bool static_ops = share && m->offsets_uniform && (size_t)Nc * TD_OTAB_ROW_BYTES <= TD_OTAB_MAX_BYTES;
+    const size_t o_srow = reserve(static_ops ? n * 4 : 0), o_otab = reserve(static_ops ? (size_t)Nc * TD_OTAB_ROW_BYTES : 0);
     hipError_t e = td_malloc_async(reinterpret_cast<void **>(&S->block), off, s);
     if (e != hipSuccess) {
         td_set_error("td_session_create: hipMallocAsync(%zu) failed: %s", off, hipGetErrorString(e));
@@ -212,6 +218,7 @@
         S->cbase = reinterpret_cast<int32_t *>(b + o_cb);
         canon_rows = reinterpret_cast<int32_t *>(b + o_crows);
     }
+    if (static_ops) S->srow = reinterpret_cast<int32_t *>(b + o_srow);
     {
         int lv = m->opt.session_hop_levels;
         if (lv < 1) lv = 1;
@@ -299,6 +306,11 @@
         TD_TRY_HIP(hipMemcpyAsync(h2_f, h1_f, n * TD_H * 4, hipMemcpyDeviceToDevice, s));
         TD_TRY(value_pass(L1.hv, L1, w.x4a, st, st.nbr, w.P, set_rows, nullptr, set_count, h2_f, gt.alpha, nullptr, 0, s));
     }
+    if (static_ops) {
+        TD_TRY(td_launch_static_operands(w.x4a, snbr_f, canon_rows, Nc, L0, b + o_otab, s));
+        TD_TRY_HIP(hipMemsetAsync(S->srow, 0xff, n * 4, s));
+        S->otab = b + o_otab;
+    }
     if (share) {
         TD_TRY(td_launch_compact_rows(skeys_f, canon_rows, Nc, TD_K * 8, S->skeys, s));
         TD_TRY(td_launch_compact_rows(snbr_f, canon_rows, Nc, TD_K * 4, S->snbr, s));
@@ -385,7 +397,7 @@
         } else {
             if ((rc = td_launch_knn_merge(w.x4a, w.node_ptr, S->pptr, w.gid, S->prot_node, Np, S->skeys, S->snbr, S->h0,
                                           S->h1s, S->ews, w.nbr, w.h, w.ew, S->clean, S->use_fwd ? S->flags2 : nullptr, s, m->cfg.knn,
-                                          w.lig_node, Nl, S->max_graph_nodes, S->cgraph, S->cbase)) != TD_OK) return rc;
+                                          w.lig_node, Nl, S->max_graph_nodes, S->cgraph, S->cbase, S->srow)) != TD_OK) return rc;
             rc = (m->opt.session_step_lists && S->graph_nodes_max > 0) ? td_launch_step_lists(S->clean, w.x4a, w.nbr, w.node_ptr, N, S->B, S->graph_nodes_max, lists, s)
                                         : TD_EINVAL;
             lists_done = rc == TD_OK;
@@ -537,6 +549,7 @@
         TD_CHECK_HIP(hipMemcpyAsync(host_counts + 2 + TD_HOP_LEVELS, S->fwd_counts, sizeof(int32_t), hipMemcpyDeviceToHost, s));
     if (n_counts > 3 + TD_HOP_LEVELS) host_counts[3 + TD_HOP_LEVELS] = S->cgraph ? (int32_t)S->static_rows : -1;
     if (n_counts > 4 + TD_HOP_LEVELS) host_counts[4 + TD_HOP_LEVELS] = S->cgraph ? (int32_t)S->pocket_groups : -1;
+    if (n_counts > 5 + TD_HOP_LEVELS) host_counts[5 + TD_HOP_LEVELS] = S->otab ? (int32_t)S->static_rows : -1;
     TD_CHECK_HIP(hipStreamSynchronize(s));
     return TD_OK;
 }
diff --git a/targetdiff_amd/csrc/td_api.h b/targetdiff_amd/csrc/td_api.h
--- a/targetdiff_amd/csrc/td_api.h
+++ b/targetdiff_amd/csrc/td_api.h
@@ -119,6 +119,8 @@
     int cpn_p;
     int64_t NCl;
     const int32_t *mixed;
+    const int32_t *srow = nullptr;
+    const void *otab = nullptr;
 };
 
 struct FwdReach {
diff --git a/targetdiff_amd/csrc/td_internal.h b/targetdiff_amd/csrc/td_internal.h
--- a/targetdiff_amd/csrc/td_internal.h
+++ b/targetdiff_amd/csrc/td_internal.h
@@ -157,6 +157,7 @@
     int node_proj_bpipe = 0;
     int node_proj_async = 1;
     int session_share_pockets = 1;
+    int edge_static_operands = 1;
     int session_step_lists = 1;
 };
 
@@ -171,6 +172,7 @@
     TdHead head;
     TdSchedules sched;
     unsigned option_epoch = 0;
+    bool offsets_uniform = true;
     int fold_dead_units = 0;
     int fold_fp32_mlps = 0;
 };
@@ -193,7 +195,7 @@
                         const int32_t *prot_rows, int64_t Np, const unsigned long long *skeys, const int32_t *snbr,
                         const float *h0, const float *h1s, const float *ews, int32_t *nbr, float *h, float *ew,
                         uint8_t *clean, uint8_t *flags2, hipStream_t s, int k = TD_K, const int32_t *lig_rows = nullptr, int64_t Nl = 0,
-                        int max_graph_nodes = 0, const int32_t *cgraph = nullptr, const int32_t *cbase = nullptr);
+                        int max_graph_nodes = 0, const int32_t *cgraph = nullptr, const int32_t *cbase = nullptr, int32_t *srow = nullptr);
 int td_launch_pocket_hash(const float *ppos, const float *pv, const int32_t *pptr, int64_t B, int F, unsigned long long *out, hipStream_t s);
 int td_launch_pocket_verify(const float *ppos, const float *pv, const int32_t *pptr, int64_t B, int F, const int32_t *cand, int32_t *flags,
                             hipStream_t s);
@@ -243,7 +245,7 @@
 int td_launch_edge_key16(const TdEdgeMlp &mlp, const TdLayer &L, const float4 *x4, const int32_t *nbr, const float *ew,
                          const float *P, const float *q, const int32_t *rows, const int32_t *count_ptr, int64_t count,
                          float *alpha, hipStream_t s, bool h2x_stage, const int32_t *cptr = nullptr, const int32_t *lig_rows = nullptr,
-                         int64_t lig_count = 0, int cpn_p = 0);
+                         int64_t lig_count = 0, int cpn_p = 0, const int32_t *srow = nullptr, const void *otab = nullptr);
 int td_launch_edge_h2x16(const TdEdgeMlp &mlp_k, const TdEdgeMlp &mlp_v, const TdLayer &L, const float4 *x4_in, float4 *x4_out,
                          const int32_t *nbr, const float *ew, const float *P, const float *q, const int32_t *rows,
                          int64_t count, hipStream_t s, const int32_t *cptr = nullptr, float *alpha = nullptr);
@@ -253,7 +255,11 @@
 int td_launch_edge_value16(const TdEdgeMlp &mlp, const TdLayer &L, const float4 *x4, const int32_t *nbr, const float *P,
                            const int32_t *rows, const int32_t *count_ptr, int64_t count, float *h, const float *alpha, const int32_t *lig_rows, int64_t lig_count,
                            hipStream_t s, const int32_t *cptr = nullptr, int cpn_p = 1, int64_t lig_chunks = 0,
-                           const int32_t *mixed_count = nullptr, float *out = nullptr, const float *gate_m = nullptr);
+                           const int32_t *mixed_count = nullptr, float *out = nullptr, const float *gate_m = nullptr,
+                           const int32_t *srow = nullptr, const void *otab = nullptr);
+constexpr size_t TD_OTAB_ROW_BYTES = 4096;
+int td_launch_static_operands(const float4 *x4, const int32_t *snbr, const int32_t *rows, int64_t count, const TdLayer &L, void *otab,
+                              hipStream_t s);
 int td_set_wg_trace(unsigned long long *buf, int slots);
 bool td_wg_trace_armed();
 int td_launch_layout(const int32_t *node_ptr, const int32_t *pptr, const int32_t *gid, const int32_t *g_cbase,
```
